# PaddlePaddle/Anakin

Measured on AMD Instinct MI355X. Metric: ResNet50 INT8 images/sec + p50 latency @ batch 1/8, 1×MI355X, higher is better.
Workload: dtype int8

## Files before the change

### anakin_amd/csrc/api_chain.hip

```cpp
#include "api_internal.h"

enum : unsigned { CK_1X1 = 1, CK_3X3 = 2, CK_HEAD = 4, CK_PAIR = 8, CK_LED = CK_3X3 | CK_HEAD, CK_ANY = 15 };
static unsigned chain_kind(const saber_hip_chain* ch) { return !ch->c3 ? CK_1X1 : (ch->b2 ? CK_PAIR : (ch->b ? CK_3X3 : CK_HEAD)); }
static const struct { int c1; unsigned kinds; ChainForm f; } chain_forms[] = {
    {64, CK_ANY,            {4, 4, 4, 1, 1, CS_BASE, false}},
    {64, CK_ANY,            {2, 2, 4, 1, 1, CS_BASE, false}},
    {128, CK_1X1 | CK_LED,  {2, 2, 4, 1, 1, CS_BASE, false}},
    {128, CK_1X1 | CK_LED,  {1, 1, 4, 1, 1, CS_BASE, false}},
    {128, CK_1X1 | CK_LED,  {6, 2, 8, 1, 1, CS_W8, false}},
    {128, CK_1X1 | CK_LED,  {5, 1, 8, 1, 1, CS_W8, false}},
    {256, CK_1X1 | CK_LED,  {1, 1, 4, 1, 1, CS_BASE, false}},
    {256, CK_1X1,           {9, 1, 4, 2, 1, CS_SPLIT, false}},
    {256, CK_1X1,           {11, 1, 8, 2, 1, CS_SPLIT8, false}},
    {256, CK_LED,           {3, 1, 8, 1, 1, CS_W8, false}},
    {256, CK_3X3,           {7, 1, 8, 1, 2, CS_COOP2, true}},
    {256, CK_3X3,           {15, 2, 8, 1, 4, CS_COOP4, true}},
    {512, CK_1X1,           {1, 1, 4, 1, 1, CS_BASE, false}},
    {512, CK_1X1,           {9, 1, 4, 2, 1, CS_SPLIT, false}},
};
static void for_each_chain_form(const saber_hip_chain* ch, const std::function<void(const ChainForm&)>& fn) {
    for (const auto& r : chain_forms)
        if (r.c1 == ch->c1 && (r.kinds & chain_kind(ch))) fn(r.f);
}
static ChainForm chain_form_where(const saber_hip_chain* ch, const std::function<bool(const ChainForm& row, const ChainForm& found)>& take) {
    ChainForm f;
    for_each_chain_form(ch, [&](const ChainForm& c) { if (take(c, f)) f = c; });
    return f;
}
ChainForm chain_form(const saber_hip_chain* ch, int code) { return chain_form_where(ch, [&](const ChainForm& c, const ChainForm&) { return c.code == code; }); }
ChainForm chain_form_default(const saber_hip_chain* ch) { return chain_form_where(ch, [](const ChainForm&, const ChainForm& f) { return !f.code; }); }
ChainForm chain_form_plain(const saber_hip_chain* ch) { return chain_form_where(ch, [](const ChainForm& c, const ChainForm&) { return !c.placement; }); }
bool chain_form_valid(const saber_hip_chain* ch, int code) {
    const ChainForm f = chain_form(ch, code);
    return f.code && ch->d_stream[f.stream].p && (f.coop != 4 || ch->stage1);
}
std::string chain_form_name(const saber_hip_chain* ch) {
    const ChainForm& f = ch->form;
    const std::string c = std::to_string(ch->c1), w8 = f.waves == 8 && f.coop == 1 ? "_w8" : "";
    if (!ch->c3) return "chain1x1_c" + c + "_px" + std::to_string(16 * f.rows) + (f.split == 2 ? "_split2" : "") + w8;
    return std::string("conv3x3+") + (ch->b2 ? "conv1x1+pair1x1_c" : (ch->b ? "chain1x1_c" : "conv1x1_c")) + c + "_" + std::to_string(f.rows) + "x16" + w8 +
           (f.coop == 2 ? "_coop2" : "") + (f.coop == 4 ? "_coop4" : "");
}
void for_each_chain_candidate(const saber_hip_chain* ch, bool shared_device, const std::function<void(const ChainForm&)>& fn) {
    for_each_chain_form(ch, [&](const ChainForm& c) { if (!(shared_device && c.placement) && chain_form_valid(ch, c.code)) fn(c); });
}

static bool chain_1x1(const saber_hip_conv* o, bool sub_res_ok = false) {
    const saber_hip_conv_desc& d = o->d;
    return o->is_i8 && o->weights_set && !o->gpool && o->algo == ALGO_IGEMM_I8 && o->epi == EPI_I8_CONV && d.kh == 1 && d.kw == 1 &&
           d.stride_h == 1 && d.stride_w == 1 && d.pad_h == 0 && d.pad_w == 0 && d.group == 1 && !o->pair_k2 &&
           !o->pool_fused && !o->pool2 && !o->pre_quant && !o->pre_pad && o->c_eff == d.c && d.act_negative_slope == 0.f &&
           d.in_layout == SABER_HIP_NHWC && d.out_layout == SABER_HIP_NHWC && (d.res_stride <= 1 || sub_res_ok);
}
static void pack_chain_params(const saber_hip_conv* o, size_t chunks_pad, std::vector<uint8_t>& out) {
    const int K = o->d.k;
    out.assign(chunks_pad * 16, 0);
    for (int k4 = 0; k4 < K / 4; ++k4) {
        float* f = (float*)(out.data() + (size_t)k4 * 48);
        int* ip = (int*)(out.data() + (size_t)k4 * 48 + 32);
        for (int r = 0; r < 4; ++r) {
            const int k = k4 * 4 + r;
            f[r] = o->scale_host.empty() ? 1.f : o->scale_host[k];
            f[4 + r] = (o->has_bias && !o->bias_p_host.empty()) ? o->bias_p_host[k] : 0.f;
            ip[r] = o->comp_host.empty() ? 0 : o->comp_host[k];
        }
    }
}
static void pack_chain_weights(const int8_t* w, int K, int C, int mfg, int wave, std::vector<uint8_t>& out, int kbase = 0,
                               int nw = 4, int ks0 = 0) {
    const int kw = K / nw, groups = kw / (16 * mfg), ksn = C / 64;
    for (int g = 0; g < groups; ++g)
        for (int ksi = 0; ksi < ksn; ++ksi)
            for (int mf = 0; mf < mfg; ++mf) {
                const int ks = (ks0 + ksi) % ksn;
                for (int lane = 0; lane < 64; ++lane) {
                    const int rho = lane & 15, kq = lane >> 4;
                    const int ch = kbase + wave * kw + g * 16 * mfg + (rho >> 2) * 4 * mfg + mf * 4 + (rho & 3);
                    const int8_t* src = w + (size_t)ch * C + ks * 64 + kq * 16;
                    out.insert(out.end(), (const uint8_t*)src, (const uint8_t*)src + 16);
                }
            }
}
static void pack_chain_weights3(const int8_t* w, int C, int wave, std::vector<uint8_t>& out, int nw = 4, int kbase = 0, int kcount = 0) {
    const int kw = (kcount ? kcount : C) / nw, mf0 = kw / 16, ksn = C / 64;
    for (int tap = 0; tap < 9; ++tap)
        for (int ks = 0; ks < ksn; ++ks)
            for (int mf = 0; mf < mf0; ++mf)
                for (int lane = 0; lane < 64; ++lane) {
                    const int rho = lane & 15, kq = lane >> 4;
                    const int ch = kbase + wave * kw + (rho >> 2) * 4 * mf0 + mf * 4 + (rho & 3);
                    for (int t = 0; t < 16; ++t) {
                        const int c = ks * 64 + kq * 16 + t;
// ... 279 lines not shown
    if (!xcd_round_robin()) return fail(SABER_HIP_UNIMPL, "stage: this device does not place workgroup b on XCD b % 8");
    return stage_build(chains, n, true, nullptr, out);
}
int saber_hip_conv2d_stage_create_tail(saber_hip_chain_t* const* chains, int n, saber_hip_chain_t* tail, saber_hip_chain_stage_t** out) {
    if (!tail) return fail(SABER_HIP_INVALID_VALUE, "null argument");
    if (!xcd_round_robin()) return fail(SABER_HIP_UNIMPL, "stage: this device does not place workgroup b on XCD b % 8");
    return stage_build(chains, n, true, tail, out);
}
int saber_hip_conv2d_stage_create_head(saber_hip_chain_t* const* chains, int n, saber_hip_chain_t* tail, const saber_hip_conv_t* head_a,
                                       const saber_hip_conv_t* head_b, saber_hip_chain_stage_t** out) {
    if (!head_a || !head_b) return fail(SABER_HIP_INVALID_VALUE, "null argument");
    if (!xcd_round_robin()) return fail(SABER_HIP_UNIMPL, "stage: this device does not place workgroup b on XCD b % 8");
    return stage_build(chains, n, true, tail, out, head_a, head_b);
}
void saber_hip_conv2d_stage_destroy(saber_hip_chain_stage_t* st) { delete st; }
int saber_hip_conv2d_stage_run(saber_hip_chain_stage_t* st, const void* x, const void* res, void* const* y1, void* const* y2, saber_hip_stream_t stream) {
    if (g_capture) return capture_unsupported("saber_hip_conv2d_stage_run (saber_hip_net_optimize forms stages itself)");
    if (!st || !x || !res || !y1 || !y2) return fail(SABER_HIP_INVALID_VALUE, "null argument");
    for (size_t i = 0; i < st->chains.size(); ++i)
        if ((!y1[i] && !(st->c1 == 64 && i + 1 < st->chains.size())) || !y2[i]) return fail(SABER_HIP_INVALID_VALUE, "stage: an output pointer per block");
    return stage_run(st, x, res, y1, y2, (hipStream_t)stream);
}
int saber_hip_conv2d_stage_run_tail(saber_hip_chain_stage_t* st, const void* x, const void* res, void* const* y1, void* const* y2, void* y_tail,
                                    saber_hip_stream_t stream) {
    if (g_capture) return capture_unsupported("saber_hip_conv2d_stage_run_tail (saber_hip_net_optimize forms stages itself)");
    if (!st || !x || !res || !y1 || !y2 || !y_tail) return fail(SABER_HIP_INVALID_VALUE, "null argument");
    for (size_t i = 0; i < st->chains.size(); ++i)
        if (!y1[i] || !y2[i]) return fail(SABER_HIP_INVALID_VALUE, "stage: an output pointer per block");
    return stage_run(st, x, res, y1, y2, (hipStream_t)stream, y_tail);
}
int saber_hip_conv2d_stage_run_head(saber_hip_chain_stage_t* st, const void* x_head, void* y_head_b, void* const* y1, void* const* y2, void* y_tail,
                                    saber_hip_stream_t stream) {
    if (g_capture) return capture_unsupported("saber_hip_conv2d_stage_run_head (saber_hip_net_optimize forms stages itself)");
    if (!st || !x_head || !y_head_b || !y1 || !y2) return fail(SABER_HIP_INVALID_VALUE, "null argument");
    for (size_t i = 0; i < st->chains.size(); ++i)
        if (!y1[i] || !y2[i]) return fail(SABER_HIP_INVALID_VALUE, "stage: an output pointer per block");
    return stage_run(st, x_head, nullptr, y1, y2, (hipStream_t)stream, y_tail, y_head_b);
}
static void pack_chain_stream(const saber_hip_chain* ch, ChainStream layout, std::vector<uint8_t>& out) {
    const saber_hip_conv *c3 = ch->c3, *a = ch->a, *b = ch->b;
    const int c = ch->c1, k1 = ch->k1, k2 = ch->k2, c2 = b ? b->d.c : 0, k2w = k2 / 2;
    const int nw = layout == CS_BASE || layout == CS_SPLIT ? 4 : 8;
    const int8_t *w3 = c3 ? c3->wq_oihw.data() : nullptr, *wa = a->wq_oihw.data(), *wb = b ? b->wq_oihw.data() : nullptr;
    std::vector<int8_t> wcat;
    if (ch->b2) {
        wcat.assign(b->wq_oihw.begin(), b->wq_oihw.end());
        wcat.insert(wcat.end(), ch->b2->wq_oihw.begin(), ch->b2->wq_oihw.end());
        wb = wcat.data();
    }
    auto mfg = [&](int k) { return ch->b2 ? 2 : std::min(4, k / nw / 16); };
    switch (layout) {
    case CS_BASE: case CS_W8:
        for (int w = 0; w < nw; ++w) {
            if (c3) pack_chain_weights3(w3, c, w, out, nw);
            pack_chain_weights(wa, k1, c, 4, w, out, 0, nw);
            if (b) pack_chain_weights(wb, k2, c2, mfg(k2), w, out, 0, nw);
        }
        break;
    case CS_SPLIT: case CS_SPLIT8:
        for (int half = 0; half < 2; ++half)
            for (int w = 0; w < nw; ++w) {
                pack_chain_weights(wa, k1, c, 4, w, out, 0, nw);
                pack_chain_weights(wb, k2w, c2, mfg(k2w), w, out, half * k2w, nw);
            }
        break;
    case CS_COOP2:
        for (int half = 0; half < 2; ++half)
            for (int w = 0; w < nw; ++w) {
                pack_chain_weights3(w3, c, w, out, nw, half * (c / 2), c / 2);
                pack_chain_weights(wa, k1 / 2, c, 4, w, out, half * (k1 / 2), nw, half * (c / 128));
                pack_chain_weights(wb, k2w, c2, 1, w, out, half * k2w, nw, half * (c2 / 128));
            }
        break;
    default: pack_coop4_stream(w3, wa, wb, out);
    }
}
static int chain_build(saber_hip_conv* c3, saber_hip_conv* a, saber_hip_conv* b, saber_hip_chain_t** out, saber_hip_conv* b2 = nullptr) {
    if (!a || !out || (!b && !c3) || (b2 && (!b || !c3))) return fail(SABER_HIP_INVALID_VALUE, "null argument");
    const bool pair2 = b2 != nullptr;
    const bool strided = c3 && (!b || pair2) && c3->d.stride_h == 2 && c3->d.stride_w == 2;
    if (pair2 && !strided) return fail(SABER_HIP_INVALID_VALUE, "chain: a sibling pair follows the strided head (conv3x3 / stride 2 + conv1x1 + eltwise) only");
    if (!chain_1x1(a, strided) || (b && !chain_1x1(b)) || (b2 && !chain_1x1(b2)))
        return fail(SABER_HIP_INVALID_VALUE, "chain: both ops must be plain 1x1 stride-1 INT8 NHWC convs with weights set");
    if (strided != (a->d.res_stride > 1) || (strided && a->d.res_stride != 2))
        return fail(SABER_HIP_INVALID_VALUE, "chain: a stride-2 head goes with a shortcut sub-sampled by 2 (and only with one)");
    const saber_hip_conv_desc& da = a->d;
    if (da.res_mode != SABER_HIP_RES_ELTWISE || da.out_dtype != SABER_HIP_S8 || (da.res_has_dtype && da.res_dtype != SABER_HIP_S8))
        return fail(SABER_HIP_INVALID_VALUE, "chain: the first conv must carry the fused eltwise epilogue with s8 residual and output");
    if (b) {
        const saber_hip_conv_desc& db = b->d;
        if (db.res_mode != SABER_HIP_RES_NONE || b->x_dtype != DT_S8 || (db.out_dtype != SABER_HIP_S8 && db.out_dtype != SABER_HIP_U8))
            return fail(SABER_HIP_INVALID_VALUE, "chain: the second conv must be a plain s8-input conv with an 8-bit output");
        if (db.n != da.n || db.h != a->oh || db.w != a->ow || db.c != da.k || (!pair2 && db.k != da.c))
            return fail(SABER_HIP_INVALID_VALUE, "chain: shapes must be C -> 4C -> C with C in {64,128,256,512} on the same pixels");
    }
    if (pair2) {
        const saber_hip_conv_desc &db = b->d, &d2 = b2->d;
        if (d2.res_mode != SABER_HIP_RES_NONE || b2->x_dtype != DT_S8 || (d2.out_dtype != SABER_HIP_S8 && d2.out_dtype != SABER_HIP_U8) || d2.n != da.n ||
            d2.h != a->oh || d2.w != a->ow || d2.c != da.k || da.c != 64 || db.k % 32 || db.k + d2.k != 640 || d2.k <= 0)
            return fail(SABER_HIP_INVALID_VALUE, "chain: the sibling pair after a strided head: 64 -> 256 (+ eltwise) -> k_b | k_b2 with k_b + k_b2 = 640, k_b % 32 == 0, 8-bit outputs");
    }
    if (!conv1x1_chain_ok(da.c, da.k, da.c))
        return fail(SABER_HIP_INVALID_VALUE, "chain: shapes must be C -> 4C -> C with C in {64,128,256,512} on the same pixels");
    if (c3) {
        const saber_hip_conv_desc& d3 = c3->d;
        const bool ok = c3->is_i8 && c3->weights_set && c3->algo == ALGO_IGEMM_I8 && c3->epi == EPI_I8_CONV && d3.kh == 3 && d3.kw == 3 &&
                        d3.stride_h == (strided ? 2 : 1) && d3.stride_w == d3.stride_h && d3.pad_h == 1 && d3.pad_w == 1 && d3.dil_h == 1 && d3.dil_w == 1 &&
                        d3.group == 1 && !c3->pair_k2 && !c3->pool_fused && !c3->pool2 && !c3->pre_quant && !c3->pre_pad &&
                        c3->c_eff == d3.c && d3.act_negative_slope == 0.f && d3.in_layout == SABER_HIP_NHWC &&
                        d3.out_layout == SABER_HIP_NHWC && d3.res_mode == SABER_HIP_RES_NONE && d3.c == da.c && d3.k == da.c &&
                        d3.n == da.n && c3->oh == da.h && c3->ow == da.w && da.c <= 256 &&
                        (d3.out_dtype == SABER_HIP_S8 || d3.out_dtype == SABER_HIP_U8) &&
                        (d3.out_dtype == SABER_HIP_U8) == (a->x_dtype == DT_U8);
        if (!ok) return fail(SABER_HIP_INVALID_VALUE, "chain: the head must be the 3x3 pad-1 INT8 conv (C -> C, C <= 256; stride 1, or 2 in front of a lone 1x1 conv) whose 8-bit output the first 1x1 conv reads");
    }
    saber_hip_chain* ch = new saber_hip_chain();
    const int k2 = b ? b->d.k + (pair2 ? b2->d.k : 0) : 0;
    ch->c3 = c3; ch->a = a; ch->b = b; ch->b2 = b2; ch->c1 = da.c; ch->k1 = da.k; ch->k2 = k2;
    ch->scale_conv = a->out_scale;
    if (c3 && !b && da.c == 256 && strided) {
        ch->tail_w3 = c3->wq_oihw;
        ch->tail_wa = a->wq_oihw;
    }
    ch->form = chain_form_default(ch);
    std::vector<uint8_t> p0, p1, p2;
    hipError_t e = hipSuccess;
    for (int l = 0; l < CS_COUNT && e == hipSuccess; ++l) {
        bool needed = false;
        for_each_chain_form(ch, [&](const ChainForm& f) { needed = needed || (f.stream == l && (!f.placement || xcd_round_robin())); });
        if (!needed) continue;
        std::vector<uint8_t> stream;
        pack_chain_stream(ch, (ChainStream)l, stream);
        e = ch->d_stream[l].upload(stream);
    }
    pack_chain_params(a, (size_t)da.k / 4 * 3, p1);
    if (b) pack_chain_params(b, ((size_t)k2 / 4 * 3 + 63) / 64 * 64 + 64, p2);
    if (pair2) {
        std::vector<uint8_t> pb2;
        pack_chain_params(b2, (size_t)b2->d.k / 4 * 3, pb2);
        std::memcpy(p2.data() + (size_t)b->d.k / 4 * 48, pb2.data(), pb2.size());
    }
    if (e == hipSuccess && ch->d_stream[CS_COOP2].p) {
        ch->coop_tiles = da.n * da.h * ((da.w + 15) / 16);
        e = ch->d_coop_ctr.alloc_zero((size_t)ch->coop_tiles * 32);
        if (e == hipSuccess) e = ch->d_coop_xcc.alloc_zero((size_t)ch->coop_tiles * 32);
        if (e == hipSuccess) e = ch->d_coop_xch.alloc_zero((size_t)ch->coop_tiles * 16 * da.c);
        if (e == hipSuccess) e = hipHostMalloc((void**)&ch->h_coop_err, sizeof(unsigned), hipHostMallocMapped);
        if (e == hipSuccess) *ch->h_coop_err = 0u;
    }
    if (e == hipSuccess && (da.c == 128 || da.c == 64) && c3 && b && !pair2 && c3->d.stride_h == 1 && xcd_round_robin()) {
        std::vector<uint8_t> s1;
        if (da.c == 128) pack_stage1_c128_stream(c3, a, b, s1);
        else pack_stage1_c64_stream(c3->wq_oihw.data(), a->wq_oihw.data(), b->wq_oihw.data(), s1);
        e = ch->d_stream_stage1.upload(s1);
    }
    if (e == hipSuccess) e = ch->d_prm1.upload(p1);
    if (e == hipSuccess && b) e = ch->d_prm2.upload(p2);
    if (e == hipSuccess && c3) {
        pack_chain_params(c3, ((size_t)da.c / 4 * 3 + 63) / 64 * 64 + 64, p0);
        e = ch->d_prm0.upload(p0);
    }
    if (e != hipSuccess) {
        delete ch;
        return hip_fail(e, "chain: device copies");
    }
    if (ch->d_stream[CS_COOP4].p) {
        const int rc = stage_build(&ch, 1, false, nullptr, &ch->stage1);
        if (rc != SABER_HIP_OK) {
            delete ch;
            return rc;
        }
    }
    *out = ch;
    return SABER_HIP_OK;
}
int saber_hip_conv2d_chain_create(saber_hip_conv_t* a, saber_hip_conv_t* b, saber_hip_chain_t** out) {
    if (!b) return fail(SABER_HIP_INVALID_VALUE, "null argument");
    return chain_build(nullptr, a, b, out);
}
int saber_hip_conv2d_chain_create3(saber_hip_conv_t* conv3x3, saber_hip_conv_t* a, saber_hip_conv_t* b, saber_hip_chain_t** out) {
    if (!conv3x3) return fail(SABER_HIP_INVALID_VALUE, "null argument");
    return chain_build(conv3x3, a, b, out);
}
int saber_hip_conv2d_chain_create3_pair(saber_hip_conv_t* conv3x3, saber_hip_conv_t* a, saber_hip_conv_t* pair_a, saber_hip_conv_t* pair_b,
                                        saber_hip_chain_t** out) {
    if (!conv3x3 || !pair_a || !pair_b) return fail(SABER_HIP_INVALID_VALUE, "null argument");
    return chain_build(conv3x3, a, pair_a, out, pair_b);
}
void saber_hip_conv2d_chain_destroy(saber_hip_chain_t* ch) { delete ch; }
int saber_hip_conv2d_chain_set_tile(saber_hip_chain_t* ch, int tn) {
    if (!ch) return fail(SABER_HIP_INVALID_VALUE, "null argument");
    if (!chain_form_valid(ch, tn)) return fail(SABER_HIP_INVALID_VALUE, "chain: no kernel form with that code for this chain");
    ch->form = chain_form(ch, tn);
    return SABER_HIP_OK;
}
int saber_hip_conv2d_chain_get_tile(const saber_hip_chain_t* ch) { return ch ? ch->form.code : 0; }
int saber_hip_conv2d_chain_run(saber_hip_chain_t* ch, const void* x, const void* res, void* y_a, void* y_b,
                               saber_hip_stream_t stream) {
    return saber_hip_conv2d_chain_run3(ch, x, res, y_a, y_b, nullptr, stream);
}
int saber_hip_conv2d_chain_run3(saber_hip_chain_t* ch, const void* x, const void* res, void* y_a, void* y_b, void* y_c,
                                saber_hip_stream_t stream) {
    if (g_capture) return capture_unsupported("saber_hip_conv2d_chain_run (saber_hip_net_optimize forms chains itself)");
    if (!ch || !x || !res || !y_a || (ch->b && !y_b) || (ch->b2 && !y_c)) return fail(SABER_HIP_INVALID_VALUE, "null argument");
    const saber_hip_conv *a = ch->a, *b = ch->b;
    ChainKArgs k;
    std::memset(&k, 0, sizeof k);
    k.x = x; k.res = res;
    const ChainForm f = ch->form;
    k.wstream = ch->d_stream[f.stream].p;
    k.prm1 = ch->d_prm1.p;
    k.prm2 = ch->d_prm2.p;
    k.y1 = y_a; k.y2 = y_b;
    k.M = a->d.n * a->oh * a->ow;
    k.in_u8 = a->x_dtype == DT_U8;
    k.relu1 = a->d.act == SABER_HIP_ACT_RELU;
    k.res_relu = a->d.res_act == SABER_HIP_ACT_RELU;
    k.coeff_conv = a->d.coeff_conv; k.scale_conv = ch->scale_conv; k.coeff_res = a->d.coeff_res; k.scale_res = a->d.scale_res;
    if (b) {
        k.relu2 = b->d.act == SABER_HIP_ACT_RELU;
        k.out_u8_2 = b->d.out_dtype == SABER_HIP_U8;
    }
    if (ch->b2) {
        k.y2b = y_c;
        k.k2_split = b->d.k;
        k.relu2b = ch->b2->d.act == SABER_HIP_ACT_RELU;
        k.out_u8_2b = ch->b2->d.out_dtype == SABER_HIP_U8;
    }
    if (ch->c3) {
        k.prm0 = ch->d_prm0.p;
        k.zero = zero_page();
        if (!k.zero) return fail(SABER_HIP_RUNTIME_ERROR, "chain: zero page");
        k.N = a->d.n; k.H = a->d.h; k.W = a->d.w;
        k.tiles_x = (k.W + 15) / 16;
        k.tiles_per_img = k.tiles_x * ((k.H + f.rows - 1) / f.rows);
        k.mg_tiles_x = div_magic(k.tiles_x);
        k.mg_tpi = div_magic(k.tiles_per_img);
        k.in0_u8 = ch->c3->x_dtype == DT_U8;
        k.relu0 = ch->c3->d.act == SABER_HIP_ACT_RELU;
        k.s0 = ch->c3->d.stride_h;
        k.H0 = ch->c3->d.h; k.W0 = ch->c3->d.w;
        if (a->d.res_stride > 1) { k.res_sub = a->d.res_stride; k.res_H = a->d.res_h; k.res_W = a->d.res_w; }
    }
    if (f.coop == 4) {
        const int rc = stage_run(ch->stage1, x, res, &y_a, &y_b, (hipStream_t)stream);
        if (rc != SABER_HIP_OK) ch->form = chain_form_plain(ch);
        return rc;
    }
    if (f.coop == 2) {
        if (*(volatile unsigned*)ch->h_coop_err) {
            *(volatile unsigned*)ch->h_coop_err = 0u;
            ch->form = chain_form_plain(ch);
            return fail(SABER_HIP_RUNTIME_ERROR, "cooperative chain: an earlier launch's workgroup pairs did not share an XCD or timed out at their "
                        "barrier (its outputs are not valid); the chain now runs the single-workgroup form");
        }
        const CoopKArgs ck{k, ch->d_coop_ctr.p, ch->d_coop_xch.p, ch->d_coop_xcc.p, ch->h_coop_err, ch->coop_tiles};
        HIP_TRY(launch_conv_chain_coop(ck, (hipStream_t)stream));
        return SABER_HIP_OK;
    }
    HIP_TRY(launch_conv1x1_chain(k, ch->c1, ch->k1, ch->k2, f.rows, f.waves, f.split, ch->c3 ? 1 : 0, (hipStream_t)stream));
    return SABER_HIP_OK;
}
```

### anakin_amd/csrc/api_internal.h

```cpp
#pragma once
#include "../../include/saber_hip.h"
#include "kernels.h"

#include <cmath>
#include <cstdio>
#include <algorithm>
#include <cstdlib>
#include <cstring>
#include <functional>
#include <memory>
#include <mutex>
#include <string>
#include <utility>
#include <type_traits>
#include <vector>

using namespace saber_mi355x;

namespace saber_api {

extern thread_local std::string g_err;
inline int fail(int code, const std::string& msg) {
    g_err = msg;
    return code;
// ... 124 lines not shown
    bool is_i8 = false;
    int x_dtype = DT_S8;
    int c_eff = 0;
    bool pre_quant = false;
    bool pre_pad = false;
    bool pre_transpose = false;
    size_t ws_bytes = 0;
    int Kg = 0, Kg_pad = 0, kw_pad = 0;
    float in_scale = 1.f, out_scale = 1.f;
    bool weights_set = false;
    std::vector<int8_t> wq_oihw;
    std::vector<float> w_scale;
    std::vector<float> bias_host;
    std::vector<float> bias_p_host, scale_host;
    std::vector<int> comp_host;
    DevBuf<uint8_t> d_w;
    DevBuf<float> d_part;
    DevBuf<unsigned> d_part_ctr;
    unsigned* h_part_err = nullptr;
    DevBuf<uint8_t> d_w3;
    DevBuf<float> d_bias, d_scale;
    DevBuf<int> d_comp;
    DevBuf<unsigned> d_sm_ctr;
    bool has_bias = false, has_comp = false;
    std::string algo_name;
    int pair_k1 = 0, pair_k2 = 0, pair_relu2 = 0, pair_dtype2 = 0;
    const saber_hip_conv* pair_src_a = nullptr;
    const saber_hip_conv* pair_src_b = nullptr;
};

struct saber_hip_stem_pair {
    saber_hip_conv* stem = nullptr;
    const saber_hip_conv* a = nullptr;
    const saber_hip_conv* b = nullptr;
    DevBuf<uint8_t> d_w, d_prm;
};

enum ChainStream { CS_BASE, CS_SPLIT, CS_SPLIT8, CS_W8, CS_COOP2, CS_COOP4, CS_COUNT };
struct ChainForm {
    int code = 0;
    int rows = 0;
    int waves = 4;
    int split = 1;
    int coop = 1;
    ChainStream stream = CS_BASE;
    bool placement = false;
};

struct saber_hip_chain {
    saber_hip_conv* c3 = nullptr;
    saber_hip_conv* a = nullptr;
    saber_hip_conv* b = nullptr;
    saber_hip_conv* b2 = nullptr;
    int c1 = 0, k1 = 0, k2 = 0;
    float scale_conv = 1.f;
    std::vector<int8_t> tail_w3, tail_wa;
    ChainForm form;
    DevBuf<uint8_t> d_stream[CS_COUNT];
    DevBuf<uint8_t> d_prm0, d_prm1, d_prm2;
    DevBuf<uint8_t> d_coop_xch;
    DevBuf<uint8_t> d_stream_stage1;
    DevBuf<unsigned long long> d_coop_ctr;
    DevBuf<unsigned> d_coop_xcc;
    unsigned* h_coop_err = nullptr;
    int coop_tiles = 0;
    struct saber_hip_chain_stage* stage1 = nullptr;
    ~saber_hip_chain();
};

struct saber_hip_chain_stage {
    std::vector<saber_hip_chain*> chains;
    saber_hip_chain* tail = nullptr;
    DevBuf<uint8_t> d_tail_stream;
    const saber_hip_conv* head_a = nullptr;
    const saber_hip_conv* head_b = nullptr;
    DevBuf<uint8_t> d_head_stream, d_head_prm1, d_head_prm2;
    DevBuf<saber_mi355x::StageBlk> d_blk;
    DevBuf<unsigned long long> d_grp_ctr, d_img_ctr;
    DevBuf<uint8_t> d_xch;
    DevBuf<unsigned> d_xcc;
    unsigned* h_err = nullptr;
    int c1 = 0, n = 0, h = 0, w = 0, tiles_x = 0, tiles_per_img = 0;
    bool per_image = false;
    ~saber_hip_chain_stage() {
        if (h_err) (void)hipHostFree(h_err);
    }
};

struct saber_hip_sep {
    saber_hip_conv* dw = nullptr;
    saber_hip_conv* pw = nullptr;
    int form = 0;
    DevBuf<uint8_t> d_wdw, d_wpw, d_prm;
    DevBuf<float> d_dw_bias, d_dw_scale;
    std::string name;
};

struct saber_hip_ir {
    saber_hip_conv* expand = nullptr;
    saber_hip_conv* dw = nullptr;
    saber_hip_conv* project = nullptr;
    int form = 0;
    float scale_conv = 1.f;
    DevBuf<uint8_t> d_we, d_eprm, d_wdw, d_wp, d_pprm;
    DevBuf<float> d_dw_bias, d_dw_scale;
    std::string name;
// ... 54 lines not shown
        ev.assign(2 * (size_t)reps, nullptr);
        for (hipEvent_t& x : ev)
            if ((e = hipEventCreate(&x)) != hipSuccess) return e;
        return hipStreamSynchronize(nullptr);
    }
    ~ColdBench() {
        for (hipEvent_t x : ev)
            if (x) (void)hipEventDestroy(x);
        if (buf) (void)hipFree(buf);
    }
    float run(hipStream_t s, const std::function<int()>& fn) {
        if (fn() != 0) return -1.f;
        for (int r = 0; r < reps; ++r) {
            if (launch_l2_flush(buf, kBytes, (unsigned*)((char*)buf + kBytes), s) != hipSuccess) return -1.f;
            if (hipEventRecord(ev[2 * r], s) != hipSuccess) return -1.f;
            if (fn() != 0) return -1.f;
            if (hipEventRecord(ev[2 * r + 1], s) != hipSuccess) return -1.f;
        }
        if (hipEventSynchronize(ev[2 * reps - 1]) != hipSuccess) return -1.f;
        std::vector<float> t(reps);
        for (int r = 0; r < reps; ++r)
            if (hipEventElapsedTime(&t[r], ev[2 * r], ev[2 * r + 1]) != hipSuccess) return -1.f;
        std::sort(t.begin(), t.end());
        return t[reps / 2] * 1000.f;
    }
};

extern thread_local ColdBench* g_cold;
int time_enqueued(hipStream_t s, const std::function<int()>& fn, int warm_iters, float* t);
extern thread_local std::vector<unsigned long long>* g_used_kernels;
constexpr float g_reuse_tol = 0.03f;
struct ColdScope {
    ColdBench local;
    bool owner = false;
    hipError_t enter(int reps, size_t flush_bytes = 0) {
        const char* w = std::getenv("SABER_HIP_AUTOTUNE_WARM");
        if (w && w[0] == '1') return hipSuccess;
        if (g_cold) return hipSuccess;
        hipError_t e = local.init(reps, flush_bytes);
        if (e != hipSuccess) return e;
        g_cold = &local;
        owner = true;
        return hipSuccess;
    }
    ~ColdScope() {
        if (owner) g_cold = nullptr;
    }
};

}

namespace saber_api {
enum OpKind { OP_CONV, OP_CONV_PAIR, OP_FC, OP_QUANT, OP_DEQUANT, OP_TRANSPOSE_IN, OP_ELT_I8, OP_ELT_F32, OP_POOL_I8, OP_POOL_F32, OP_POOL_F32_I8, OP_FC_Q, OP_SOFTMAX, OP_RELU_F32, OP_ACT_F32, OP_CONCAT, OP_DECONV };
enum Launch { LAUNCH_NONE, LAUNCH_OWN, LAUNCH_CHAIN, LAUNCH_CHAIN3, LAUNCH_STAGE, LAUNCH_STEM_PAIR, LAUNCH_SEP, LAUNCH_IR, LAUNCH_FIRE };
struct NetOp {
    OpKind kind;
    std::string name;
    saber_hip_conv* conv = nullptr;
    saber_hip_fc* fc = nullptr;
    saber_hip_deconv* deconv = nullptr;
    int in = -1, in2 = -1, out = -1, out2 = -1;
    std::vector<int> ins, cat_c;
    std::vector<float> cat_m;
    Launch launch = LAUNCH_OWN;
    int absorbed_by = -1;
    bool skip = false;
    std::string res_note;
    saber_hip_chain* chain = nullptr;
    int chain_out = -1;
    bool chain_on = false;
    saber_hip_chain* chain3 = nullptr;
    int chain3_res = -1, chain3_y1 = -1, chain3_y2 = -1;
    int chain3_y3 = -1;
    bool led_on = false;
    saber_hip_chain_stage* stage = nullptr;
    int stage_n = 0;
    bool stage_on = false;
    bool stage_name_kept = false;
    bool tail_on = false;
    int tail_of = -1;
    bool head_on = false;
    int head_of = -1;
    bool stage_y1_private = false;
    saber_hip_stem_pair* stem_pair = nullptr;
    int stem_y1 = -1, stem_y2 = -1;
    saber_hip_sep* sep = nullptr;
    int sep_out = -1;
    bool sep_on = false;
    saber_hip_ir* ir = nullptr;
    int ir_out = -1;
    bool ir_on = false;
    saber_hip_fire* fire = nullptr;
    int fire_out = -1;
    bool fire_on = false;
    int lane = 0;
    bool record = false;
    int p[16] = {0};
    float f[6] = {0};
    size_t count = 0;
};
template <typename F>
inline void op_for_each_input(const NetOp& o, F&& f) {
    if (o.kind == OP_CONCAT) {
        for (int t : o.ins) f(t);
        return;
    }
    if (o.in >= 0) f(o.in);
    if (o.in2 >= 0) f(o.in2);
}
inline int op_reads(const NetOp& o, int t) {
    int n = 0;
    op_for_each_input(o, [&](int u) { n += u == t; });
    return n;
}
inline bool op_touches(const NetOp& o, int t) { return op_reads(o, t) || o.out == t || o.out2 == t; }
}

struct saber_hip_net {
    std::vector<size_t> tensor_bytes;
    std::vector<size_t> tensor_off;
    std::vector<void*> tensor_ext;
    std::vector<std::pair<const void*, int>> captured_ptr;
    void* ptr(int id) const {
        if (id < 0) return nullptr;
        if ((size_t)id < tensor_ext.size() && tensor_ext[id]) return tensor_ext[id];
        return (void*)(arena + tensor_off[id]);
    }
    std::vector<NetOp> ops;
    char* arena = nullptr;
    size_t arena_bytes = 0, ws_off = 0, ws_bytes = 0;
    hipGraph_t graph = nullptr;
    hipGraphExec_t exec = nullptr;
    bool finalized = false;
    bool compacted = false;
    bool shared_device = false;
    bool reproducible_fp32 = false;
    bool inplace_external = false;
    int coop_fallbacks = 0;
    hipStream_t side = nullptr;
    hipEvent_t ev_start = nullptr, ev_join = nullptr;
    std::vector<hipEvent_t> ev_op;
    std::vector<int> writer;
    bool lanes_ready = false, has_side = false;
    std::vector<saber_hip_conv*> owned;
    std::vector<saber_hip_chain*> owned_chains;
    std::vector<saber_hip_chain_stage*> owned_stages;
    std::vector<saber_hip_stem_pair*> owned_stem_pairs;
    std::vector<saber_hip_sep*> owned_seps;
    std::vector<saber_hip_ir*> owned_irs;
    std::vector<saber_hip_fire*> owned_fires;
};

namespace saber_api {
struct Capture;
extern thread_local Capture* g_capture;
int capture_conv(saber_hip_conv* op, const void* x, void* y, const void* res);
int capture_fc(saber_hip_fc* fc, const void* x, float* y, bool quantised_input);
int capture_unsupported(const char* what);
int capture_deconv(saber_hip_deconv* op, const void* x, void* y);
int capture_concat(size_t pixels, int n_inputs, const void* const* xs, const int* channels, const float* mult, int dtype, void* y);
int capture_stream_op(OpKind kind, const char* name, const int* p, int np, const float* f, int nf, size_t count, const void* in,
                      size_t in_bytes, const void* in2, size_t in2_bytes, void* out, size_t out_bytes, void* out2, size_t out2_bytes);
}

bool sel_valid(const saber_hip_conv* op, const saber_api::ConvSel& s);
int sel_set(saber_hip_conv* op, const saber_api::ConvSel& s);
void sel_release_unused(saber_hip_conv* op);
void sel_name(saber_hip_conv* op);
unsigned long long sel_kernel_key(const saber_hip_conv* op, const saber_api::ConvSel& s);
int sel_launch(saber_hip_conv* op, saber_mi355x::ConvKArgs& a, hipStream_t s);
void for_each_candidate(const saber_hip_conv* op, const saber_api::ConvSel* best, const std::function<void(const saber_api::ConvSel&)>& fn);
bool dw_ok(const saber_hip_conv* op);
bool group_ok(const saber_hip_conv* op);
bool stem_ok(const saber_hip_conv* op);
bool fc_small_ok(const saber_hip_conv* op);
bool b3_tile_ok(const saber_hip_conv* op, int tile, int ks);
int dw_static_form(const saber_hip_conv* op);
int group_static_form(const saber_hip_conv* op);
constexpr long DW_STRIP_MIN_LANES = 150000;
void conv_fill_args(const saber_hip_conv* op, saber_mi355x::ConvKArgs& a, const void* x, void* y, const void* res);
int stem_pool_args(const saber_hip_conv* op, const void* x, void* y, void* workspace, hipStream_t s, saber_mi355x::ConvKArgs* a);
bool xcd_round_robin();
int split_prepare(saber_hip_conv* op);
bool img_conv_ok(const saber_hip_conv* op);
int img_conv_prepare(saber_hip_conv* op);
int pw_prepare(saber_hip_conv* op);
bool pw_eligible(const saber_hip_conv* op);
int img_conv_run(saber_hip_conv* op, const void* x, void* y, const void* res, void* y_pool, hipStream_t stream);
void img_conv_release(saber_hip_conv* op);
int net_launch(saber_hip_net* net, const NetOp& o, hipStream_t s);
bool fc_softmax_ok(const saber_hip_fc* fc, bool quantised_input = false);
int fc_run_softmax(saber_hip_fc* fc, const void* x, float* y, float* prob, void* workspace, hipStream_t s, bool quantised_input);
int fc_softmax_prepare(saber_hip_fc* fc);
int concat_check(int n_inputs, const int* channels, const float* mult, int dtype, int* row_bytes);
void net_resolve(saber_hip_net* net);
void net_drop_graph(saber_hip_net* net);
void net_set_chain_mode(saber_hip_net* net, int ia, int mode);
int net_chain_mode(const saber_hip_net* net, int ia);
void net_set_stage(saber_hip_net* net, int i0, bool on);
void net_set_head(saber_hip_net* net, int i0, bool on);
void net_set_tail(saber_hip_net* net, int i0, bool on);
ChainForm chain_form(const saber_hip_chain* ch, int code);
bool chain_form_valid(const saber_hip_chain* ch, int code);
ChainForm chain_form_default(const saber_hip_chain* ch);
ChainForm chain_form_plain(const saber_hip_chain* ch);
std::string chain_form_name(const saber_hip_chain* ch);
void for_each_chain_candidate(const saber_hip_chain* ch, bool shared_device, const std::function<void(const ChainForm&)>& fn);
bool conv_sep_ok(const saber_hip_conv* dw, const saber_hip_conv* pw, std::string* why);
bool sep_form_valid(const saber_hip_sep* sp, int code);
void for_each_sep_form(const saber_hip_sep* sp, const std::function<void(int code)>& fn);
int sep_static_form(const saber_hip_sep* sp);
void net_set_sep(saber_hip_net* net, int i, int code);
bool conv_ir_ok(const saber_hip_conv* expand, const saber_hip_conv* dw, const saber_hip_conv* project, std::string* why);
bool ir_form_valid(const saber_hip_ir* ir, int code);
void for_each_ir_form(const saber_hip_ir* ir, const std::function<void(int code)>& fn);
int ir_static_form(const saber_hip_ir* ir);
void net_set_ir(saber_hip_net* net, int i, int code);
bool conv_fire_ok(const saber_hip_conv* squeeze, const saber_hip_conv* e1, const saber_hip_conv* e3, std::string* why);
bool fire_form_valid(const saber_hip_fire* fr, int code);
void for_each_fire_form(const saber_hip_fire* fr, const std::function<void(int code)>& fn);
int fire_static_form(const saber_hip_fire* fr);
void net_set_fire(saber_hip_net* net, int i, int code);
bool deconv_form_valid(const saber_hip_deconv* op, int form);
int deconv_static_form(const saber_hip_deconv* op);
void for_each_deconv_form(const saber_hip_deconv* op, const std::function<void(int form)>& fn);
int stage_run(saber_hip_chain_stage* st, const void* x, const void* res, void* const* y1, void* const* y2, hipStream_t s, void* y_tail = nullptr,
              void* y_head = nullptr);
```

### anakin_amd/csrc/api_net.hip

```cpp
#include "api_internal.h"

#include <atomic>
static std::atomic<int> g_coop_fallbacks_total{0};

void net_drop_graph(saber_hip_net* net) {
    if (net->exec) (void)hipGraphExecDestroy(net->exec);
    if (net->graph) (void)hipGraphDestroy(net->graph);
    net->exec = nullptr;
    net->graph = nullptr;
}
int net_launch(saber_hip_net* net, const NetOp& o, hipStream_t s) {
    auto T = [&](int id) -> void* { return net->ptr(id); };
    void* ws = net->arena + net->ws_off;
    switch (o.kind) {
    case OP_CONV:
        switch (o.launch) {
        case LAUNCH_NONE: return SABER_HIP_OK;
        case LAUNCH_STAGE: {
            void* y1[saber_mi355x::STAGE4_LONG];
            void* y2[saber_mi355x::STAGE4_LONG];
            const NetOp* ops = &o;
            for (int k = 0; k < o.stage_n; ++k) {
                y1[k] = ops[3 * k].stage_y1_private ? nullptr : T(ops[3 * k].chain3_y1);
                y2[k] = T(ops[3 * k].chain3_y2);
            }
            void* const y_tail = o.tail_on ? T(ops[3 * o.stage_n].chain3_y1) : nullptr;
            const int rc = o.head_on ? stage_run(o.stage, T(ops[-1].in), nullptr, y1, y2, s, y_tail, T(o.in))
                                     : stage_run(o.stage, T(o.in), T(o.chain3_res), y1, y2, s, y_tail);
            if (rc == SABER_HIP_RUNTIME_ERROR) {
                ++net->coop_fallbacks;
                ++g_coop_fallbacks_total;
                net_set_stage(net, (int)(&o - net->ops.data()), false);
                net_drop_graph(net);
            }
            return rc;
        }
        case LAUNCH_STEM_PAIR: return saber_hip_conv2d_stem_pair_run(o.stem_pair, T(o.in), nullptr, T(o.stem_y1), T(o.stem_y2), ws, s);
        case LAUNCH_CHAIN3: {
            const int rc = saber_hip_conv2d_chain_run3(o.chain3, T(o.in), T(o.chain3_res), T(o.chain3_y1), T(o.chain3_y2), T(o.chain3_y3), s);
            if (rc == SABER_HIP_RUNTIME_ERROR) {
                ++net->coop_fallbacks;
                ++g_coop_fallbacks_total;
            }
            return rc;
        }
        case LAUNCH_CHAIN: return saber_hip_conv2d_chain_run(o.chain, T(o.in), T(o.in2), T(o.out), T(o.chain_out), s);
        case LAUNCH_SEP: return saber_hip_conv2d_sep_run(o.sep, T(o.in), nullptr, T(o.sep_out), s);
        case LAUNCH_IR: return saber_hip_conv2d_ir_run(o.ir, T(o.in), nullptr, nullptr, T(o.ir_out), s);
        case LAUNCH_FIRE: return saber_hip_conv2d_fire_run(o.fire, T(o.in), nullptr, T(o.fire_out), s);
        case LAUNCH_OWN: break;
        }
        if (o.conv->gpool) return saber_hip_conv2d_run_gpool(o.conv, T(o.in), T(o.out), T(o.in2), T(o.out2), s);
        return saber_hip_conv2d_run(o.conv, T(o.in), T(o.out), T(o.in2), ws, s);
    case OP_CONV_PAIR:
        if (o.skip) return SABER_HIP_OK;
        return saber_hip_conv2d_run_pair(o.conv, T(o.in), T(o.out), T(o.out2), s);
    case OP_FC:
        if (o.out2 >= 0) return fc_run_softmax(o.fc, T(o.in), (float*)T(o.out), (float*)T(o.out2), ws, s, false);
        return saber_hip_fc_run(o.fc, T(o.in), (float*)T(o.out), ws, s);
    case OP_QUANT:
        return saber_hip_quantize_nchw_to_nhwc(o.p[0], o.p[1], o.p[2], o.p[3], o.p[4], o.p[5], o.f[0],
                                               (const float*)T(o.in), T(o.out), s);
    case OP_DEQUANT:
        return saber_hip_dequantize_nhwc_to_nchw(o.p[0], o.p[1], o.p[2], o.p[3], o.p[4], o.f[0], T(o.in),
                                                 (float*)T(o.out), s);
    case OP_TRANSPOSE_IN:
        return saber_hip_transpose_nchw_to_nhwc_f32(o.p[0], o.p[1], o.p[2], o.p[3], o.p[4], (const float*)T(o.in),
                                                    (float*)T(o.out), s);
    case OP_ELT_I8:
        return saber_hip_eltwise_sum_i8(o.count, (const int8_t*)T(o.in), (const int8_t*)T(o.in2), o.f[0], o.f[1],
                                        o.f[2], o.f[3], o.p[0], (int8_t*)T(o.out), s);
    case OP_ELT_F32:
        return saber_hip_eltwise_sum_f32(o.count, (const float*)T(o.in), (const float*)T(o.in2), o.f[0], o.f[1],
                                         o.p[0], (float*)T(o.out), s);
    case OP_POOL_I8:
        return saber_hip_pool2d_i8_nhwc(o.p[0], o.p[1], o.p[2], o.p[3], o.p[4], o.p[5], o.p[6], o.p[7], o.p[8],
                                        o.p[9], o.p[10], o.p[11], o.p[12], o.p[13], o.p[14], T(o.in), T(o.out), s);
    case OP_POOL_F32:
        return saber_hip_pool2d_f32(o.p[0], o.p[1], o.p[2], o.p[3], o.p[4], o.p[5], o.p[6], o.p[7], o.p[8], o.p[9],
                                    o.p[10], o.p[11], o.p[12], o.p[13], (const float*)T(o.in), (float*)T(o.out), s);
    case OP_POOL_F32_I8:
        return saber_hip_pool2d_f32_from_i8_q(o.p[0], o.p[1], o.p[2], o.p[3], o.p[4], o.p[5], o.p[6], o.p[7], o.p[8],
                                              o.p[9], o.p[10], o.p[11], o.p[12], o.p[13], o.f[0], T(o.in),
                                              (float*)T(o.out), o.f[1], (int8_t*)T(o.out2), s);
    case OP_FC_Q:
        if (o.out2 >= 0) return fc_run_softmax(o.fc, T(o.in), (float*)T(o.out), (float*)T(o.out2), ws, s, true);
        return saber_hip_fc_run_q(o.fc, (const int8_t*)T(o.in), (float*)T(o.out), s);
    case OP_SOFTMAX:
        if (o.skip) return SABER_HIP_OK;
        return saber_hip_softmax_f32(o.p[0], o.p[1], (const float*)T(o.in), (float*)T(o.out), s);
    case OP_RELU_F32: return saber_hip_relu_f32(o.count, (const float*)T(o.in), (float*)T(o.out), s);
    case OP_ACT_F32: return saber_hip_activation_f32(o.p[0], o.count, o.f[0], o.f[1], (const float*)T(o.in), (float*)T(o.out), s);
    case OP_CONCAT: {
        if (o.skip) return SABER_HIP_OK;
        const void* xs[CONCAT_MAX_INPUTS];
        for (size_t k = 0; k < o.ins.size(); ++k) xs[k] = T(o.ins[k]);
        return saber_hip_concat_nhwc(o.count, (int)o.ins.size(), xs, o.cat_c.data(), o.cat_m.empty() ? nullptr : o.cat_m.data(), o.p[0], T(o.out), s);
    }
// ... 184 lines not shown
    o.kind = OP_DECONV; o.deconv = op; o.in = in_id; o.out = out_id;
    o.name = std::string("deconv:") + op->algo_name;
    return push(net, std::move(o));
}
int saber_hip_net_add_softmax(saber_hip_net_t* net, int rows, int cols, int in_id, int out_id) {
    NetOp o;
    o.kind = OP_SOFTMAX; o.in = in_id; o.out = out_id; o.name = "softmax_f32";
    o.p[0] = rows; o.p[1] = cols;
    return push(net, std::move(o));
}

int saber_hip_net_finalize(saber_hip_net_t* net) {
    if (net->finalized) return SABER_HIP_OK;
    size_t off = 0;
    net->tensor_off.resize(net->tensor_bytes.size());
    for (size_t i = 0; i < net->tensor_bytes.size(); ++i) {
        net->tensor_off[i] = off;
        if (net->tensor_ext[i]) continue;
        off += (net->tensor_bytes[i] + 255) / 256 * 256;
    }
    net->ws_off = off;
    off += (net->ws_bytes + 255) / 256 * 256;
    net->arena_bytes = off ? off : 256;
    HIP_TRY(hipMalloc((void**)&net->arena, net->arena_bytes));
    HIP_TRY(hipMemset(net->arena, 0, net->arena_bytes));
    HIP_TRY(hipStreamSynchronize(nullptr));
    net->finalized = true;
    return SABER_HIP_OK;
}
int saber_hip_net_compact_arena(saber_hip_net_t* net, const int* keep, int n_keep) {
    if (!net || !net->finalized) return fail(SABER_HIP_INVALID_VALUE, "compact_arena: net not finalized");
    const int nt = (int)net->tensor_bytes.size(), nops = (int)net->ops.size();
    for (const NetOp& o : net->ops)
        if (o.lane) return SABER_HIP_OK;
    std::vector<int> first(nt, nops), last(nt, -1), writes(nt, 0), reads(nt, 0);
    std::vector<char> pinned(nt, 0);
    for (int i = 0; i < n_keep; ++i)
        if (keep && keep[i] >= 0 && keep[i] < nt) pinned[keep[i]] = 1;
    std::vector<int> g_lo(nops), g_hi(nops);
    for (int i = 0; i < nops; ++i) g_lo[i] = g_hi[i] = i;
    auto span = [&](int i, int n) {
        const int hi = std::min(nops - 1, i + n - 1);
        int lo = i;
        for (int j = i; j <= hi; ++j) lo = std::min(lo, g_lo[j]);
        int h2 = hi;
        for (int j = i; j <= hi; ++j) h2 = std::max(h2, g_hi[j]);
        for (int j = lo; j <= h2; ++j) { g_lo[j] = std::min(g_lo[j], lo); g_hi[j] = std::max(g_hi[j], h2); }
    };
    for (int i = 0; i < nops; ++i) {
        const NetOp& o = net->ops[i];
        if (o.stage) span(i, 3 * o.stage_n + (o.stage->tail ? 2 : 0));
        if (o.stage && o.stage->head_a && i > 0) span(i - 1, 2);
        if (o.chain3) span(i, 3);
        if (o.chain) span(i, 2);
        if (o.stem_pair) span(i, 2);
        if (o.sep) span(i, 2);
        if (o.fire) span(i, 4);
        if (o.ir) span(i, 3);
        if ((o.kind == OP_FC || o.kind == OP_FC_Q) && o.out2 >= 0) span(i, 2);
    }
    for (int i = 0; i < nops; ++i) {
        const NetOp& o = net->ops[i];
        const int rd[] = {o.in, o.in2, o.chain3_res};
        const int wr[] = {o.out, o.out2, o.chain_out, o.chain3_y1, o.chain3_y2, o.chain3_y3, o.stem_y1, o.stem_y2, o.sep_out, o.ir_out, o.fire_out};
        auto touch = [&](int t) {
            if (t < 0 || t >= nt) return;
            first[t] = std::min(first[t], g_lo[i]);
            last[t] = std::max(last[t], g_hi[i]);
        };
        for (int t : rd) { touch(t); if (t >= 0 && t < nt) ++reads[t]; }
        for (size_t k = 1; k < o.ins.size(); ++k) { touch(o.ins[k]); if (o.ins[k] >= 0 && o.ins[k] < nt) ++reads[o.ins[k]]; }
        for (int t : wr) { touch(t); if (t >= 0 && t < nt) ++writes[t]; }
    }
    for (int t = 0; t < nt; ++t)
        if (net->tensor_ext[t] || !writes[t] || !reads[t] || last[t] < 0) pinned[t] = 1;
    for (int t = 0; t < nt; ++t)
        if (pinned[t]) { first[t] = -1; last[t] = nops; }
    std::vector<int> order;
    for (int t = 0; t < nt; ++t)
        if (!net->tensor_ext[t]) order.push_back(t);
    auto slot = [&](int t) { return (net->tensor_bytes[t] + 255) / 256 * 256; };
    std::stable_sort(order.begin(), order.end(), [&](int a, int b) { return slot(a) > slot(b); });
    std::vector<size_t> off(nt, 0);
    std::vector<int> placed;
    size_t top = 0;
    for (int t : order) {
        const size_t sz = slot(t);
        if (!sz) { off[t] = 0; continue; }
        std::vector<std::pair<size_t, size_t>> busy;
        for (int u : placed)
            if (first[u] <= last[t] && first[t] <= last[u]) busy.push_back({off[u], off[u] + slot(u)});
        std::sort(busy.begin(), busy.end());
        size_t at = 0;
        for (const auto& b : busy) {
            if (at + sz <= b.first) break;
            at = std::max(at, b.second);
        }
        off[t] = at;
        top = std::max(top, at + sz);
        placed.push_back(t);
    }
    const size_t ws_off = top, total = std::max<size_t>(256, top + (net->ws_bytes + 255) / 256 * 256);
    if (total >= net->arena_bytes) return SABER_HIP_OK;
    char* fresh = nullptr;
    HIP_TRY(hipMalloc((void**)&fresh, total));
    HIP_TRY(hipMemset(fresh, 0, total));
    HIP_TRY(hipDeviceSynchronize());
    for (int t = 0; t < nt; ++t)
        if (!net->tensor_ext[t] && !writes[t] && net->tensor_bytes[t])
            HIP_TRY(hipMemcpy(fresh + off[t], net->arena + net->tensor_off[t], net->tensor_bytes[t], hipMemcpyDeviceToDevice));
    HIP_TRY(hipDeviceSynchronize());
    (void)hipFree(net->arena);
    net->arena = fresh;
    net->arena_bytes = total;
    net->ws_off = ws_off;
    for (int t = 0; t < nt; ++t)
        if (!net->tensor_ext[t]) net->tensor_off[t] = off[t];
// ... 52 lines not shown
int saber_hip_net_run(saber_hip_net_t* net, saber_hip_stream_t stream) {
    if (!net->finalized) return fail(SABER_HIP_INVALID_VALUE, "net not finalized");
    int rc = net_prepare_lanes(net);
    if (rc) return rc;
    hipStream_t main_s = (hipStream_t)stream;
    if (!net->has_side) {
        for (const NetOp& o : net->ops) {
            rc = net_launch(net, o, main_s);
            if (rc) return rc;
        }
        return SABER_HIP_OK;
    }
    HIP_TRY(hipEventRecord(net->ev_start, main_s));
    HIP_TRY(hipStreamWaitEvent(net->side, net->ev_start, 0));
    std::fill(net->writer.begin(), net->writer.end(), -1);
    std::vector<std::vector<int>> readers(net->tensor_bytes.size());
    bool side_dirty = false;
    for (size_t i = 0; i < net->ops.size(); ++i) {
        const NetOp& o = net->ops[i];
        hipStream_t s = o.lane ? net->side : main_s;
        int ins[1 + CONCAT_MAX_INPUTS] = {o.out}, n_ins = 1;
        op_for_each_input(o, [&](int t) { ins[n_ins++] = t; });
        for (int k = 0; k < n_ins; ++k) {
            const int t = ins[k];
            if (t < 0) continue;
            const int wi = net->writer[t];
            if (wi >= 0 && net->ops[wi].lane != o.lane) HIP_TRY(hipStreamWaitEvent(s, net->ev_op[wi], 0));
        }
        const int outs[2] = {o.out, o.out2};
        for (int t : outs) {
            if (t < 0) continue;
            for (int r : readers[t])
                if (net->ops[r].lane != o.lane) HIP_TRY(hipStreamWaitEvent(s, net->ev_op[r], 0));
            readers[t].clear();
        }
        rc = net_launch(net, o, s);
        if (rc) return rc;
        if (o.record) HIP_TRY(hipEventRecord(net->ev_op[i], s));
        if (o.lane) side_dirty = true;
        net->writer[o.out] = (int)i;
        if (o.out2 >= 0) net->writer[o.out2] = (int)i;
        op_for_each_input(o, [&](int t) { readers[t].push_back((int)i); });
    }
    if (side_dirty) {
        HIP_TRY(hipEventRecord(net->ev_join, net->side));
        HIP_TRY(hipStreamWaitEvent(main_s, net->ev_join, 0));
    }
    return SABER_HIP_OK;
}
int saber_hip_net_set_lane(saber_hip_net_t* net, int index, int lane) {
    if (index < 0 || index >= (int)net->ops.size() || lane < 0 || lane > 1) return fail(SABER_HIP_INVALID_VALUE, "bad op index / lane");
    if (net->lanes_ready) return fail(SABER_HIP_INVALID_VALUE, "lanes are fixed after the first run");
    for (const NetOp& o : net->ops)
        if (lane && (o.chain || o.chain3 || o.stem_pair || o.sep || o.ir || o.fire))
            return fail(SABER_HIP_INVALID_VALUE, "the net has launches that span several ops' tensors (conv1x1 chains, the stem pair, separable sites): lanes must be assigned before saber_hip_net_optimize");
    if (lane) {
        const NetOp& o = net->ops[index];
        const size_t ws = o.kind == OP_CONV && o.conv ? o.conv->ws_bytes : (o.kind == OP_FC && o.fc ? saber_hip_fc_workspace_bytes(o.fc) : 0);
        if (ws) return fail(SABER_HIP_INVALID_VALUE, "an op that needs the shared workspace cannot run on the side lane");
    }
    net->ops[index].lane = lane;
    return SABER_HIP_OK;
}
int saber_hip_net_run_op(saber_hip_net_t* net, int index, saber_hip_stream_t stream) {
    if (!net->finalized || index < 0 || index >= (int)net->ops.size()) return fail(SABER_HIP_INVALID_VALUE, "bad op index");
    return net_launch(net, net->ops[index], (hipStream_t)stream);
}
static bool net_coop_error_pending(const saber_hip_net* net) {
    for (const NetOp& o : net->ops) {
        if (o.stage && o.stage->h_err && *(volatile unsigned*)o.stage->h_err) return true;
        if (const saber_hip_chain* ch = o.chain3)
            if ((ch->h_coop_err && *(volatile unsigned*)ch->h_coop_err) || (ch->stage1 && ch->stage1->h_err && *(volatile unsigned*)ch->stage1->h_err))
                return true;
    }
    return false;
}
int saber_hip_net_capture(saber_hip_net_t* net, saber_hip_stream_t stream) {
    hipStream_t s = (hipStream_t)stream;
    net_drop_graph(net);
    if (net_coop_error_pending(net)) return saber_hip_net_status(net);
    HIP_TRY(hipStreamBeginCapture(s, hipStreamCaptureModeThreadLocal));
    int rc = saber_hip_net_run(net, stream);
    hipError_t e = hipStreamEndCapture(s, &net->graph);
    if (rc == SABER_HIP_OK && e != hipSuccess) rc = hip_fail(e, "hipStreamEndCapture");
    if (rc == SABER_HIP_OK && (e = hipGraphInstantiate(&net->exec, net->graph, nullptr, nullptr, 0)) != hipSuccess) rc = hip_fail(e, "hipGraphInstantiate");
    if (rc != SABER_HIP_OK) net_drop_graph(net);
    return rc;
}
int saber_hip_net_replay(saber_hip_net_t* net, saber_hip_stream_t stream) {
    if (!net->exec) return fail(SABER_HIP_INVALID_VALUE, "net not captured");
    if (net_coop_error_pending(net)) return saber_hip_net_status(net);
    HIP_TRY(hipGraphLaunch(net->exec, (hipStream_t)stream));
    return SABER_HIP_OK;
}
int saber_hip_net_coop_fallbacks(const saber_hip_net_t* net) { return net ? net->coop_fallbacks : 0; }
int saber_hip_coop_fallbacks_total(void) { return g_coop_fallbacks_total.load(); }
static void conv_work(const saber_hip_conv* c, double& bytes, double& flops) {
    const saber_hip_conv_desc& d = c->d;
    const double esz_in = d.in_dtype == SABER_HIP_F32 ? 4 : 1, esz_out = d.out_dtype == SABER_HIP_F32 ? 4 : 1;
    const double esz_w = c->is_i8 ? 1 : 4;
    const double in_el = (double)d.n * d.h * d.w * d.c;
    const int oh = c->oh, ow = c->ow;
    const double out_el = (double)d.n * ((c->pool_fused || c->pool2) ? c->pool_oh * c->pool_ow : oh * ow) * d.k;
    bytes += in_el * esz_in + out_el * esz_out + (double)d.k * (d.c / d.group) * d.kh * d.kw * esz_w;
    if (d.res_mode != SABER_HIP_RES_NONE) bytes += (double)d.n * oh * ow * d.k * esz_out;
    flops += 2.0 * d.n * oh * ow * (double)d.k * (d.c / d.group) * d.kh * d.kw;
}
// ... 71 lines not shown
            float ms = 0;
            HIP_TRY(hipEventElapsedTime(&ms, ev[prev[i]], ev[i + 1]));
            acc[i] += ms;
        }
    }
    for (size_t i = 0; i < n; ++i) out_us[i] = (float)(acc[i] * 1000.0 / iters);
    return SABER_HIP_OK;
}
int saber_hip_net_time_op_in_pass(saber_hip_net_t* net, saber_hip_stream_t stream, int index, int iters, float* out_us) {
    if (!net || !net->finalized || iters <= 0 || !out_us || index < 0 || index >= (int)net->ops.size())
        return fail(SABER_HIP_INVALID_VALUE, "bad argument");
    hipStream_t s = (hipStream_t)stream;
    EventPair evp;
    HIP_TRY(evp.init());
    double acc = 0.0;
    for (int it = 0; it < iters + 1; ++it) {
        for (size_t i = 0; i < net->ops.size(); ++i) {
            if ((int)i == index) HIP_TRY(hipEventRecord(evp.e0, s));
            int rc = net_launch(net, net->ops[i], s);
            if (rc) return rc;
            if ((int)i == index) HIP_TRY(hipEventRecord(evp.e1, s));
        }
        HIP_TRY(hipStreamSynchronize(s));
        float ms = 0;
        HIP_TRY(hipEventElapsedTime(&ms, evp.e0, evp.e1));
        if (it) acc += ms;
    }
    *out_us = (float)(acc * 1000.0 / iters);
    return SABER_HIP_OK;
}
int saber_hip_net_time_ops(saber_hip_net_t* net, saber_hip_stream_t stream, int iters, float* out_us) {
    hipStream_t s = (hipStream_t)stream;
    EventPair evp;
    HIP_TRY(evp.init());
    hipEvent_t e0 = evp.e0, e1 = evp.e1;
    for (size_t i = 0; i < net->ops.size(); ++i) {
        int rc = net_launch(net, net->ops[i], s);
        if (rc) return rc;
        HIP_TRY(hipEventRecord(e0, s));
        for (int it = 0; it < iters; ++it) net_launch(net, net->ops[i], s);
        HIP_TRY(hipEventRecord(e1, s));
        HIP_TRY(hipEventSynchronize(e1));
        float ms = 0;
        HIP_TRY(hipEventElapsedTime(&ms, e0, e1));
        out_us[i] = ms * 1000.f / iters;
    }
    return SABER_HIP_OK;
}
int saber_hip_net_tensor_unwritten(const saber_hip_net_t* net, int id) {
    if (id < 0 || id >= (int)net->tensor_bytes.size()) return 0;
    if (net->tensor_bytes[id] == 0) return 1;
    for (const NetOp& o : net->ops) {
        const Launch by = o.skip ? net->ops[o.absorbed_by].launch : o.launch;
        if (o.out == id && (o.launch == LAUNCH_CHAIN3 || o.launch == LAUNCH_STEM_PAIR || o.launch == LAUNCH_SEP || (o.chain3 && by == LAUNCH_STAGE))) return 1;
        if (o.out == id && (o.launch == LAUNCH_IR || (o.skip && by == LAUNCH_IR && (int)(&o - net->ops.data()) == o.absorbed_by + 1))) return 1;
        if (o.out == id && o.kind == OP_CONV && (o.launch == LAUNCH_FIRE || (o.skip && by == LAUNCH_FIRE))) return 1;
        if (o.launch == LAUNCH_STAGE && o.head_on && o.chain3_res == id) return 1;
        if (o.chain3 && o.stage_y1_private && o.chain3_y1 == id && (o.launch == LAUNCH_STAGE || (o.skip && by == LAUNCH_STAGE))) return 1;
    }
    return 0;
}
int saber_hip_net_status(saber_hip_net_t* net) {
    if (!net || !net->finalized) return fail(SABER_HIP_INVALID_VALUE, "net not finalized");
    int bad = 0;
    for (size_t i = 0; i < net->ops.size(); ++i) {
        NetOp& o = net->ops[i];
        if (o.stage && o.stage->h_err && *(volatile unsigned*)o.stage->h_err) {
            *(volatile unsigned*)o.stage->h_err = 0u;
            if (o.stage_on) net_set_stage(net, (int)i, false);
            ++bad;
        }
        saber_hip_chain* ch = o.chain3;
        if (ch) {
            unsigned* words[2] = {ch->h_coop_err, ch->stage1 ? ch->stage1->h_err : nullptr};
            for (unsigned* w : words)
                if (w && *(volatile unsigned*)w) {
                    *(volatile unsigned*)w = 0u;
                    if (ch->form.placement) ch->form = chain_form_plain(ch);
                    ++bad;
                }
        }
    }
    if (!bad) return SABER_HIP_OK;
    net->coop_fallbacks += bad;
    g_coop_fallbacks_total += bad;
    net_resolve(net);
    net_drop_graph(net);
    return fail(SABER_HIP_RUNTIME_ERROR, "a cooperative launch of the last pass did not complete (workgroups on different XCDs, or a hand-off "
                "timed out: another kernel held the CUs); its outputs are not valid - those sites now launch block by block: run the pass again");
}
int saber_hip_net_inject_coop_error(saber_hip_net_t* net) {
    if (!net) return fail(SABER_HIP_INVALID_VALUE, "null argument");
    auto res2 = [](const NetOp& o) { return o.stage && o.stage->c1 == 64; };
    for (NetOp& o : net->ops)
        if (o.stage && !res2(o) && o.stage_on && o.stage->h_err) { *(volatile unsigned*)o.stage->h_err = 1u; return SABER_HIP_OK; }
    for (NetOp& o : net->ops)
        if (res2(o) && o.stage_on && o.stage->h_err) { *(volatile unsigned*)o.stage->h_err = 1u; return SABER_HIP_OK; }
    for (NetOp& o : net->ops) {
        if (o.stage && !res2(o) && o.stage->h_err) { *(volatile unsigned*)o.stage->h_err = 1u; return SABER_HIP_OK; }
        if (o.chain3 && o.chain3->h_coop_err) { *(volatile unsigned*)o.chain3->h_coop_err = 1u; return SABER_HIP_OK; }
    }
    for (NetOp& o : net->ops)
        if (res2(o) && o.stage->h_err) { *(volatile unsigned*)o.stage->h_err = 1u; return SABER_HIP_OK; }
    return fail(SABER_HIP_INVALID_VALUE, "the net has no cooperative launch site");
}
int saber_hip_net_num_launches(const saber_hip_net_t* net) {
    int n = 0;
// ... 23 lines not shown
```

### anakin_amd/csrc/api_net_autotune.hip

```cpp
#include "api_internal.h"

static saber_hip_conv* net_op_conv(saber_hip_net* net, int index) {
    if (index < 0 || index >= (int)net->ops.size()) return nullptr;
    NetOp& o = net->ops[index];
    if (o.kind == OP_CONV || o.kind == OP_CONV_PAIR) return o.conv;
    if (o.kind == OP_FC || o.kind == OP_FC_Q) return o.fc ? o.fc->conv : nullptr;
    return nullptr;
}
int saber_hip_net_get_choice(saber_hip_net_t* net, int index) {
    if (net && index >= 0 && index < (int)net->ops.size() && net->ops[index].kind == OP_DECONV)
        return (18 << 16) | saber_hip_deconv2d_get_tile(net->ops[index].deconv);
    saber_hip_conv* c = net_op_conv(net, index);
    int choice = (c && !c->pool_fused && (c->algo <= ALGO_IGEMM_F32 || dw_ok(c) || group_ok(c))) ? saber_hip_conv2d_get_tile(c) : 0;
    if (!c) return choice;
    const NetOp& o = net->ops[index];
    if (o.chain) choice |= (1 << 28) | ((o.chain_on ? o.chain->form.code : 0) << 24);
    if (o.chain3) choice |= (1 << 29) | ((o.led_on ? o.chain3->form.code : 0) << 24);
    if (o.sep) choice |= (3 << 28) | ((o.sep_on ? o.sep->form : 0) << 24);
    if (o.ir) choice |= (int)0x80000000u | ((o.ir_on ? o.ir->form : 0) << 24);
    if (o.fire) choice |= (int)0x80000000u | ((o.fire_on ? o.fire->form : 0) << 24);
    if (o.stage && o.stage_on) choice |= 1 << 30;
    if (o.stage && o.stage_on && o.tail_on) choice |= (int)0x80000000u;
    if (o.head_of >= 0 && net->ops[o.head_of].stage_on && net->ops[o.head_of].head_on) choice |= 1 << 29;
    return choice;
}
int saber_hip_net_stage_blocks(const saber_hip_net_t* net, int index) {
    if (!net || index < 0 || index >= (int)net->ops.size()) return 0;
    const NetOp& o = net->ops[index];
    return o.stage ? (o.stage->c1 == 64 ? -o.stage_n : o.stage_n) : 0;
}
int saber_hip_net_stage_head(const saber_hip_net_t* net, int index) {
    if (!net || index < 1 || index >= (int)net->ops.size() || !net->ops[index].stage) return -1;
    return net->ops[index - 1].head_of == index ? index - 1 : -1;
}
int saber_hip_net_set_choice(saber_hip_net_t* net, int index, int choice) {
    if (net && index >= 0 && index < (int)net->ops.size() && net->ops[index].kind == OP_DECONV) {
        if (net->reproducible_fp32 || ((choice >> 16) & 0xff) != 18) return SABER_HIP_OK;
        const int rc = saber_hip_deconv2d_set_tile(net->ops[index].deconv, choice & 0xffff);
        if (rc) return rc;
        net_resolve(net);
        net_drop_graph(net);
        return SABER_HIP_OK;
    }
    saber_hip_conv* c = net_op_conv(net, index);
    const bool ir_bits = c && net->ops[index].ir && ((unsigned)choice >> 30) == 2u;
    const int ir_tn = (choice >> 24) & 15;
    if (ir_bits && ir_tn && !ir_form_valid(net->ops[index].ir, ir_tn)) return saber_hip_conv2d_ir_set_tile(net->ops[index].ir, ir_tn);
    const bool fire_bits = c && net->ops[index].fire && ((unsigned)choice >> 30) == 2u;
    if (fire_bits && ir_tn && !fire_form_valid(net->ops[index].fire, ir_tn)) return saber_hip_conv2d_fire_set_tile(net->ops[index].fire, ir_tn);
    if (fire_bits && !(choice & 0xffffff)) {
        net_set_fire(net, index, ir_tn);
        net_drop_graph(net);
        return SABER_HIP_OK;
    }
    if (ir_bits && !(choice & 0xffffff)) {
        net_set_ir(net, index, ir_tn);
        net_drop_graph(net);
        return SABER_HIP_OK;
    }
    if (!c || !choice || c->pool_fused || (c->algo > ALGO_IGEMM_F32 && !dw_ok(c) && !group_ok(c))) return SABER_HIP_OK;
    if (net->reproducible_fp32 && !c->is_i8) return SABER_HIP_OK;
    if (net->ops[index].kind == OP_CONV_PAIR && index > 0 && net->ops[index - 1].stem_pair) return SABER_HIP_OK;
    const int chain_bits = (choice >> 24) & 63;
    const bool stage_on = ((choice >> 30) & 1) && !net->shared_device;
    const bool tail_on = stage_on && (((unsigned)choice >> 31) & 1u);
    choice &= 0xffffff;
    if (net->shared_device && ((choice >> 16) & 0xff) == 11) choice &= ~(0xf << 12);
    NetOp& o = net->ops[index];
    saber_hip_chain* ch = index + 1 >= (int)net->ops.size() ? nullptr : ((o.chain3 && (chain_bits & 32)) ? o.chain3 : ((o.chain && (chain_bits & 16)) ? o.chain : nullptr));
    int tn = chain_bits & 15;
    if (ch && net->shared_device && chain_form(ch, tn).placement) tn = chain_form_plain(ch).code;
    if (ch && tn && !chain_form_valid(ch, tn)) return saber_hip_conv2d_chain_set_tile(ch, tn);
    const bool sep_bits = o.sep && (chain_bits & 48) == 48;
    if (sep_bits && tn && !sep_form_valid(o.sep, tn)) return saber_hip_conv2d_sep_set_tile(o.sep, tn);
    int rc = choice ? saber_hip_conv2d_set_tile(c, choice) : SABER_HIP_OK;
    if (rc) return rc;
    o.res_note.clear();
    o.stage_name_kept = false;
    if (ch && tn) (void)saber_hip_conv2d_chain_set_tile(ch, tn);
    const bool in_stage = o.chain3 && o.skip && !o.stage && o.tail_of < 0;
    const int mode = ch ? net_chain_mode(net, ch == o.chain3 ? index + 1 : index) : 0;
    if (ch && ch == o.chain3) net_set_chain_mode(net, index + 1, (tn || in_stage) ? 2 : std::min(mode, 1));
    else if (ch) net_set_chain_mode(net, index, mode == 2 ? 2 : (tn ? 1 : 0));
    if (o.stage) net_set_stage(net, index, stage_on);
    if (o.stage) net_set_tail(net, index, tail_on);
    if (o.head_of >= 0) net_set_head(net, o.head_of, (chain_bits & 32) && !net->shared_device);
    if (sep_bits) net_set_sep(net, index, tn);
    if (ir_bits) net_set_ir(net, index, ir_tn);
    if (fire_bits) net_set_fire(net, index, ir_tn);
    net_resolve(net);
    net_drop_graph(net);
    return SABER_HIP_OK;
}

static int net_consolidate_kernels(saber_hip_net* net, hipStream_t s) {
    if (net->has_side) return SABER_HIP_OK;
    if (const char* e = std::getenv("SABER_HIP_NO_CONSOLIDATE"))
        if (e[0] == '1') return SABER_HIP_OK;
    struct Site { int op; unsigned long long key; ConvSel choice; };
    auto conv_of = [&](const NetOp& o) -> saber_hip_conv* {
        if (o.launch != LAUNCH_OWN) return nullptr;
        if (o.kind != OP_CONV && o.kind != OP_CONV_PAIR) return nullptr;
        if (net->reproducible_fp32 && o.conv && !o.conv->is_i8) return nullptr;
        return (o.conv && !o.conv->pool_fused && o.conv->algo <= ALGO_IGEMM_F32) ? o.conv : nullptr;
    };
    auto collect = [&]() {
        std::vector<Site> v;
        for (int i = 0; i < (int)net->ops.size(); ++i)
            if (saber_hip_conv* c = conv_of(net->ops[i])) v.push_back({i, sel_kernel_key(c, c->sel), c->sel});
        return v;
    };
    EventPair ev;
    HIP_TRY(ev.init());
    auto forward_ms = [&](float* ms) -> int {
        int rc = 0;
        for (int i = 0; i < 3 && !rc; ++i) rc = saber_hip_net_run(net, s);
        if (rc) return rc;
        HIP_TRY(hipEventRecord(ev.e0, s));
        for (int i = 0; i < 30 && !rc; ++i) rc = saber_hip_net_run(net, s);
        HIP_TRY(hipEventRecord(ev.e1, s));
        HIP_TRY(hipEventSynchronize(ev.e1));
        HIP_TRY(hipEventElapsedTime(ms, ev.e0, ev.e1));
        return rc;
    };
    std::vector<Site> sites = collect();
    for (size_t si = 0; si < sites.size(); ++si) {
        const Site cur = sites[si];
        if ((cur.key >> 8 & 0xff) != 5) continue;
        int uses = 0;
        for (const Site& t : sites) uses += t.key == cur.key;
        if (uses != 1) continue;
        saber_hip_conv* c = conv_of(net->ops[cur.op]);
        std::vector<Site> alts;
        for (const Site& t : sites) {
            if (t.op == cur.op || (t.key & 0xff) != (cur.key & 0xff) || (t.key >> 8 & 0xff) != 5 || t.key == cur.key) continue;
            if ((net->ops[t.op].kind == OP_CONV_PAIR) != (net->ops[cur.op].kind == OP_CONV_PAIR)) continue;
            bool dup = false;
            for (const Site& a : alts) dup |= a.key == t.key;
            if (!dup) alts.push_back(t);
// ... 34 lines not shown
    ColdScope scope;
    HIP_TRY(scope.enter(iters < 7 ? 7 : (iters > 15 ? 15 : iters), net->arena_bytes > ((size_t)256 << 20) ? net->arena_bytes : 0));
    std::vector<unsigned long long> used_kernels;
    struct UsedScope {
        UsedScope(std::vector<unsigned long long>* v) { g_used_kernels = g_cold ? v : nullptr; }
        ~UsedScope() { g_used_kernels = nullptr; }
    } used_scope(&used_kernels);
    for (NetOp& o : net->ops) {
        if (o.kind == OP_CONV_PAIR && o.skip && &o != net->ops.data() && (&o)[-1].stem_pair) continue;
        if (net->reproducible_fp32 && o.conv && !o.conv->is_i8) continue;
        if (net->reproducible_fp32 && o.fc && o.fc->conv && !o.fc->conv->is_i8) continue;
        if (o.kind == OP_CONV_PAIR) {
            int rc = saber_hip_conv2d_autotune_pair(o.conv, T(o.in), T(o.out), T(o.out2), stream, iters);
            if (rc) return rc;
            continue;
        }
        saber_hip_conv* c = o.kind == OP_CONV ? o.conv : ((o.kind == OP_FC || o.kind == OP_FC_Q) ? o.fc->conv : nullptr);
        if (!c) continue;
        const void* xin = T(o.in);
        if (o.kind == OP_FC && o.fc->pre_quant) {
            int rq = net_launch(net, o, (hipStream_t)stream);
            if (rq) return rq;
            xin = net->arena + net->ws_off;
        }
        int rc = saber_hip_conv2d_autotune(c, xin, T(o.out), T(o.in2), net->arena + net->ws_off, stream, iters);
        if (rc) return rc;
        o.res_note.clear();
    }
    for (NetOp& o : net->ops) {
        if (o.kind != OP_DECONV || net->reproducible_fp32) continue;
        hipStream_t s = (hipStream_t)stream;
        auto run = [&]() -> int { return net_launch(net, o, s); };
        float best = 0.f;
        int best_form = -1;
        for_each_deconv_form(o.deconv, [&](int form) {
            float us = -1.f;
            if (saber_hip_deconv2d_set_tile(o.deconv, form) != SABER_HIP_OK) return;
            if (time_enqueued(s, run, 20, &us) != SABER_HIP_OK) return;
            if (best_form < 0 || us < best) { best = us; best_form = form; }
        });
        if (best_form < 0) return fail(SABER_HIP_RUNTIME_ERROR, "autotune: no form of a deconv op could be timed");
        int rc = saber_hip_deconv2d_set_tile(o.deconv, best_form);
        if (!rc) rc = run();
        if (rc) return rc;
    }
    net_resolve(net);
    const char* log_env = std::getenv("SABER_HIP_AUTOTUNE_LOG");
    const bool log_cands = g_cold && log_env && log_env[0] == '1';
    auto log_cand = [&](const saber_hip_conv* c, const std::string& name, float t) {
        if (log_cands) std::fprintf(stderr, "autotune [%dx%dx%d c%d k%d %dx%d] %-40s %8.2f us\n", c->d.n, c->d.h, c->d.w, c->d.c, c->d.k, c->d.kh, c->d.kw, name.c_str(), t);
    };
    for (size_t i = 0; i < net->ops.size(); ++i)
        if (net->ops[i].stage) net_set_stage(net, (int)i, false);
    for (size_t i = 0; i < net->ops.size(); ++i) {
        NetOp& A = net->ops[i];
        const int ia = (int)i;
        NetOp* H = (ia > 0 && net->ops[ia - 1].chain3) ? &net->ops[ia - 1] : nullptr;
        if (!A.chain && !H) continue;
        const int first = H ? ia - 1 : ia;
        const int last = (A.chain || (H && H->chain3->b2)) ? ia + 1 : ia;
        hipStream_t s = (hipStream_t)stream;
        auto run_all = [&]() -> int {
            int rc = 0;
            for (int k = first; k <= last; ++k) rc |= net_launch(net, net->ops[k], s);
            return rc;
        };
        auto timed = [&](float* t) { return time_enqueued(s, run_all, 20, t); };
        float best = 0.f;
        int best_mode = 0, best_tn = 0;
        net_set_chain_mode(net, ia, 0);
        int rc = timed(&best);
        if (rc) return rc;
        log_cand(A.conv, "separate", best);
        for (int mode = A.chain ? 1 : 2; mode <= (H ? 2 : 1); ++mode) {
            saber_hip_chain* ch = mode == 2 ? H->chain3 : A.chain;
            for_each_chain_candidate(ch, net->shared_device, [&](const ChainForm& f) {
                float ms = -1.f;
                if (saber_hip_conv2d_chain_set_tile(ch, f.code) != SABER_HIP_OK) return;
                net_set_chain_mode(net, ia, mode);
                const int rt = timed(&ms);
                log_cand(A.conv, (mode == 2 ? H->name : A.name).substr(5), ms);
                if (rt == SABER_HIP_OK && ms < best) { best = ms; best_mode = mode; best_tn = f.code; }
            });
        }
        if (best_mode) (void)saber_hip_conv2d_chain_set_tile(best_mode == 2 ? H->chain3 : A.chain, best_tn);
        net_set_chain_mode(net, ia, best_mode);
        rc = run_all();
        if (rc) return rc;
    }
    for (size_t i = 0; i < net->ops.size(); ++i) {
        NetOp& H0 = net->ops[i];
        if (!H0.stage || net->shared_device) continue;
        const bool has_tail = H0.stage->tail != nullptr;
        const bool has_head = saber_hip_net_stage_head(net, (int)i) >= 0;
        const int first = (int)i, last = first + 3 * H0.stage_n - 1 + (has_tail ? 2 : 0);
        hipStream_t s = (hipStream_t)stream;
        auto run_all = [&]() -> int {
            int rc = 0;
            for (int k = first - (has_head ? 1 : 0); k <= last; ++k) rc |= net_launch(net, net->ops[k], s);
            return rc;
        };
        auto timed = [&](float* t) { return time_enqueued(s, run_all, 20, t); };
        std::vector<int> modes(H0.stage_n), tns(H0.stage_n);
        for (int k = 0; k < H0.stage_n; ++k) {
            modes[k] = net_chain_mode(net, first + 3 * k + 1);
            tns[k] = net->ops[first + 3 * k].chain3->form.code;
        }
        float sep = 0.f, one = 0.f;
        int rc = timed(&sep);
        if (rc) return rc;
        log_cand(H0.conv, "separate", sep);
        net_set_stage(net, first, true);
        net_set_tail(net, first, false);
        bool ok = timed(&one) == SABER_HIP_OK && hipStreamSynchronize(s) == hipSuccess && !*(volatile unsigned*)H0.stage->h_err;
        log_cand(H0.conv, H0.name.substr(5), ok ? one : -1.f);
        if (ok && has_tail) {
            float wt = 0.f;
            net_set_tail(net, first, true);
            const bool ok_t = timed(&wt) == SABER_HIP_OK && hipStreamSynchronize(s) == hipSuccess && !*(volatile unsigned*)H0.stage->h_err;
            log_cand(H0.conv, H0.name.substr(5), ok_t ? wt : -1.f);
            if (*(volatile unsigned*)H0.stage->h_err) ok = false;
            else if (ok_t && wt < one) one = wt;
            else net_set_tail(net, first, false);
        }
        if (ok && one < sep && has_head) {
            float wh = 0.f;
            net_set_head(net, first, true);
            const bool ok_h = timed(&wh) == SABER_HIP_OK && hipStreamSynchronize(s) == hipSuccess && !*(volatile unsigned*)H0.stage->h_err;
            log_cand(H0.conv, H0.name.substr(5), ok_h ? wh : -1.f);
            if (*(volatile unsigned*)H0.stage->h_err) ok = false;
            else if (ok_h && wh < one * 0.99f) one = wh;
            else net_set_head(net, first, false);
        }
        if (!ok || one >= sep * (H0.stage->c1 == 64 ? 0.99f : 1.f)) {
            *(volatile unsigned*)H0.stage->h_err = 0u;
            net_set_stage(net, first, false);
            for (int k = 0; k < H0.stage_n; ++k) {
                (void)saber_hip_conv2d_chain_set_tile(net->ops[first + 3 * k].chain3, tns[k]);
                net_set_chain_mode(net, first + 3 * k + 1, modes[k]);
            }
        }
        rc = run_all();
        if (rc) return rc;
    }
    for (size_t i = 0; i + 1 < net->ops.size(); ++i) {
        NetOp& D = net->ops[i];
        if (!D.sep) continue;
        hipStream_t s = (hipStream_t)stream;
        auto run_all = [&]() -> int { return net_launch(net, net->ops[i], s) | net_launch(net, net->ops[i + 1], s); };
        auto timed = [&](float* t) { return time_enqueued(s, run_all, 20, t); };
        float best = 0.f;
        int best_code = 0;
        net_set_sep(net, (int)i, 0);
        int rc = timed(&best);
        if (rc) return rc;
        log_cand(D.conv, "separate", best);
        for_each_sep_form(D.sep, [&](int code) {
            float us = -1.f;
            net_set_sep(net, (int)i, code);
            const int rt = timed(&us);
            log_cand(D.conv, D.name.substr(5), us);
            if (rt == SABER_HIP_OK && us < best) { best = us; best_code = code; }
        });
        net_set_sep(net, (int)i, best_code);
        rc = run_all();
        if (rc) return rc;
    }
    for (size_t i = 0; i + 2 < net->ops.size(); ++i) {
        NetOp& E = net->ops[i];
        if (!E.ir) continue;
        hipStream_t s = (hipStream_t)stream;
        auto run_all = [&]() -> int { return net_launch(net, net->ops[i], s) | net_launch(net, net->ops[i + 1], s) | net_launch(net, net->ops[i + 2], s); };
        auto timed = [&](float* t) { return time_enqueued(s, run_all, 20, t); };
        float best = 0.f;
        int best_code = 0;
        net_set_ir(net, (int)i, 0);
        int rc = timed(&best);
        if (rc) return rc;
        log_cand(E.conv, "separate", best);
        for_each_ir_form(E.ir, [&](int code) {
            float us = -1.f;
            net_set_ir(net, (int)i, code);
            const int rt = timed(&us);
            log_cand(E.conv, E.name.substr(5), us);
            if (rt == SABER_HIP_OK && us < best) { best = us; best_code = code; }
        });
        net_set_ir(net, (int)i, best_code);
        rc = run_all();
        if (rc) return rc;
    }
    for (size_t i = 0; i + 3 < net->ops.size(); ++i) {
        NetOp& Q = net->ops[i];
        if (!Q.fire) continue;
        hipStream_t s = (hipStream_t)stream;
        auto run_all = [&]() -> int {
            int r = 0;
            for (size_t j = i; j <= i + 3; ++j) r |= net_launch(net, net->ops[j], s);
// ... 23 lines not shown
```

### anakin_amd/csrc/api_net_optimize.hip

```cpp
#include "api_internal.h"

void net_resolve(saber_hip_net* net) {
    std::vector<NetOp>& ops = net->ops;
    const int n = (int)ops.size();
    enum { IN_CHAIN, IN_STAGE, IN_STEM, IN_SEP, IN_IR, IN_FIRE };
    static const char* const covered[] = {"conv:(in the chain launch)", "conv:(in the stage launch)", "conv:(in the stem launch)", "conv:(in the separable launch)",
                                          "conv:(in the inverted-residual launch)", "conv:(in the fire launch)"};
    std::vector<int> in(n, IN_CHAIN);
    for (NetOp& o : ops) {
        o.launch = LAUNCH_OWN;
        o.absorbed_by = -1;
    }
    auto absorb = [&](int j, int by, int what) {
        ops[j].launch = LAUNCH_NONE;
        ops[j].absorbed_by = by;
        in[j] = what;
    };
    for (int i = 0; i < n; ++i) {
        NetOp& o = ops[i];
        if (o.launch == LAUNCH_NONE) continue;
        if ((o.kind == OP_FC || o.kind == OP_FC_Q) && o.out2 >= 0) {
            for (int j = i + 1; j < n; ++j)
                if (ops[j].kind == OP_SOFTMAX && ops[j].out == o.out2) { absorb(j, i, IN_CHAIN); break; }
        }
        if (o.kind != OP_CONV || i + 1 >= n) continue;
        if (o.stage && o.stage_on) {
            o.launch = LAUNCH_STAGE;
            for (int k = 0; k < o.stage_n; ++k) {
                if (k) absorb(i + 3 * k, i, IN_STAGE);
                absorb(i + 3 * k + 1, i, IN_CHAIN);
                absorb(i + 3 * k + 2, i, IN_CHAIN);
            }
            if (o.tail_on)
                for (int j = i + 3 * o.stage_n; j < i + 3 * o.stage_n + 2; ++j) absorb(j, i, IN_STAGE);
            if (o.head_on) absorb(i - 1, i, IN_STAGE);
        } else if (o.stem_pair) {
            o.launch = LAUNCH_STEM_PAIR;
            absorb(i + 1, i, IN_STEM);
        } else if (o.chain3 && o.led_on) {
            o.launch = LAUNCH_CHAIN3;
            absorb(i + 1, i, IN_CHAIN);
            if (o.chain3->b || o.chain3->b2) absorb(i + 2, i, IN_CHAIN);
        } else if (o.chain && o.chain_on) {
            o.launch = LAUNCH_CHAIN;
            absorb(i + 1, i, IN_CHAIN);
        } else if (o.sep && o.sep_on) {
            o.launch = LAUNCH_SEP;
            absorb(i + 1, i, IN_SEP);
        } else if (o.ir && o.ir_on && i + 2 < n) {
            o.launch = LAUNCH_IR;
            absorb(i + 1, i, IN_IR);
            absorb(i + 2, i, IN_IR);
        } else if (o.fire && o.fire_on && i + 3 < n) {
            o.launch = LAUNCH_FIRE;
            for (int j = i + 1; j <= i + 3; ++j) absorb(j, i, IN_FIRE);
        }
    }
    for (int i = 0; i < n; ++i) {
        NetOp& o = ops[i];
        o.skip = o.launch == LAUNCH_NONE;
        if (o.kind == OP_CONCAT) {
            o.name = "concat" + std::to_string(o.ins.size()) + (o.skip ? " (in the fire launch)" : "");
        } else if (o.kind == OP_DECONV) {
            o.name = std::string("deconv:") + o.deconv->algo_name;
        } else if (o.kind == OP_SOFTMAX) {
            o.name = o.skip ? "softmax_f32 (in the fc launch)" : "softmax_f32";
        } else if (o.kind == OP_FC || o.kind == OP_FC_Q) {
            o.name = std::string("fc:") + o.fc->conv->algo_name;
            if (o.out2 >= 0) o.name += fc_softmax_ok(o.fc, o.kind == OP_FC_Q) ? "+softmax" : " | softmax_f32";
        } else if (o.kind == OP_CONV || o.kind == OP_CONV_PAIR) {
            const std::string own = o.conv->algo_name;
            const bool kept = o.stage_name_kept && !o.skip;
            switch (kept ? (o.stage ? LAUNCH_STAGE : LAUNCH_NONE) : o.launch) {
            case LAUNCH_NONE: o.name = covered[kept ? IN_STAGE : in[i]]; break;
            case LAUNCH_OWN: o.name = "conv:" + own + o.res_note; break;
            case LAUNCH_CHAIN: o.name = "conv:" + chain_form_name(o.chain); break;
            case LAUNCH_CHAIN3: o.name = "conv:" + chain_form_name(o.chain3); break;
            case LAUNCH_SEP: o.name = std::string("conv:") + saber_hip_conv2d_sep_algo(o.sep); break;
            case LAUNCH_IR: o.name = std::string("conv:") + saber_hip_conv2d_ir_algo(o.ir); break;
            case LAUNCH_FIRE: o.name = std::string("conv:") + saber_hip_conv2d_fire_algo(o.fire); break;
            case LAUNCH_STEM_PAIR: o.name = "conv:" + own + "+pair1x1_" + std::to_string(o.stem_pair->a->d.k) + "+" + std::to_string(o.stem_pair->b->d.k); break;
            case LAUNCH_STAGE:
                o.name = std::string(o.head_on && !kept ? "conv:[pair1x1]+stage_c" : "conv:stage_c") + std::to_string(o.stage->c1) + "_" + std::to_string(o.stage_n) + "x[conv3x3+chain1x1]_2x16" +
                         (o.stage->c1 == 256 ? "_coop4" : "") + (o.tail_on && !kept ? "+[conv3x3/2+conv1x1]" : "");
                break;
            }
        }
    }
}
void net_set_chain_mode(saber_hip_net* net, int ia, int mode) {
    NetOp& A = net->ops[ia];
    NetOp* H = (ia > 0 && net->ops[ia - 1].chain3) ? &net->ops[ia - 1] : nullptr;
    if (H) H->led_on = mode == 2;
    if (H) H->stage_name_kept = false;
    A.chain_on = A.chain && mode >= 1;
    A.res_note.clear();
    net_resolve(net);
}
int net_chain_mode(const saber_hip_net* net, int ia) {
    const NetOp& A = net->ops[ia];
    return (ia > 0 && net->ops[ia - 1].chain3 && net->ops[ia - 1].led_on) ? 2 : (A.chain_on ? 1 : 0);
}
void net_set_tail(saber_hip_net* net, int i0, bool on) {
    NetOp& H0 = net->ops[i0];
    if (!H0.stage || !H0.stage->tail) return;
    H0.tail_on = on;
    net_resolve(net);
}
void net_set_head(saber_hip_net* net, int i0, bool on) {
    NetOp& H0 = net->ops[i0];
    if (!H0.stage || !H0.stage->head_a || i0 < 1 || net->ops[i0 - 1].head_of != i0) return;
    H0.head_on = on;
    net_resolve(net);
}
void net_set_stage(saber_hip_net* net, int i0, bool on) {
    NetOp& H0 = net->ops[i0];
    if (!H0.stage) return;
    if (on || H0.stage_on)
        for (int k = 0; k < H0.stage_n; ++k) {
            net->ops[i0 + 3 * k].led_on = true;
            net->ops[i0 + 3 * k].stage_name_kept = !on;
            net->ops[i0 + 3 * k + 1].chain_on = net->ops[i0 + 3 * k + 1].chain != nullptr;
        }
    if (on) H0.tail_on = H0.stage->tail != nullptr;
    if (!on) H0.tail_on = H0.head_on = false;
    H0.stage_on = on;
    net_resolve(net);
}
void net_set_sep(saber_hip_net* net, int i, int code) {
    NetOp& D = net->ops[i];
    if (!D.sep || i + 1 >= (int)net->ops.size()) return;
    if (code && saber_hip_conv2d_sep_set_tile(D.sep, code) != SABER_HIP_OK) code = 0;
    D.sep_on = code != 0;
    net_resolve(net);
}
void net_set_ir(saber_hip_net* net, int i, int code) {
    NetOp& E = net->ops[i];
    if (!E.ir || i + 2 >= (int)net->ops.size()) return;
    if (code && saber_hip_conv2d_ir_set_tile(E.ir, code) != SABER_HIP_OK) code = 0;
    E.ir_on = code != 0;
    net_resolve(net);
}
void net_set_fire(saber_hip_net* net, int i, int code) {
    NetOp& Q = net->ops[i];
    if (!Q.fire || i + 3 >= (int)net->ops.size()) return;
    if (code && saber_hip_conv2d_fire_set_tile(Q.fire, code) != SABER_HIP_OK) code = 0;
    Q.fire_on = code != 0;
    net_resolve(net);
}
static int clone_conv_i8(const saber_hip_conv* src, const saber_hip_conv_desc& d, saber_hip_conv** out) {
    int rc = saber_hip_conv2d_create(&d, out);
    if (rc) return rc;
    rc = saber_hip_conv2d_set_weights(*out, src->wq_oihw.data(), SABER_HIP_S8, src->w_scale.data(),
                                      src->has_bias ? src->bias_host.data() : nullptr, src->in_scale, src->out_scale);
    if (rc) {
        saber_hip_conv2d_destroy(*out);
        *out = nullptr;
    }
    return rc;
}

int saber_hip_net_optimize(saber_hip_net_t* net, int flags) {
    if (!net) return fail(SABER_HIP_INVALID_VALUE, "null argument");
    if (net->finalized) return fail(SABER_HIP_INVALID_VALUE, "optimize must run before finalize");
    if (flags & 2048) {
        net->shared_device = true;
        flags &= ~256;
    }
    if (net->shared_device) flags &= ~256;
    if (flags & SABER_HIP_NET_REPRODUCIBLE_FP32) net->reproducible_fp32 = true;
    std::vector<NetOp>& ops = net->ops;
    const int nt = (int)net->tensor_bytes.size();
    std::vector<char> dead(ops.size(), 0);
    int removed = 0;
    auto consumers = [&](int t) {
        int c = 0;
        for (size_t i = 0; i < ops.size(); ++i)
            if (!dead[i]) c += op_reads(ops[i], t);
// ... 314 lines not shown
                A.chain3 || B.chain3 || in_ir(A) || in_ir(B))
                continue;
            if (A.conv->d.res_mode != SABER_HIP_RES_ELTWISE || B.in != A.out || A.in2 < 0 || B.in2 >= 0) continue;
            saber_hip_chain* ch = nullptr;
            if (saber_hip_conv2d_chain_create(A.conv, B.conv, &ch) != SABER_HIP_OK) continue;
            net->owned_chains.push_back(ch);
            A.chain = ch;
            A.chain_out = B.out;
            net_set_chain_mode(net, (int)i, ch->c1 <= 256 ? 1 : 0);
            if (A.chain_on) ++removed;
        }
    }
    if (flags & 32) {
        for (size_t i = 0; i + 2 < ops.size(); ++i) {
            NetOp& Hd = ops[i];
            NetOp& A = ops[i + 1];
            NetOp& B = ops[i + 2];
            if (!A.chain || Hd.kind != OP_CONV || !Hd.conv || Hd.chain3 || Hd.chain || Hd.skip || Hd.lane || Hd.in2 >= 0 ||
                A.in != Hd.out)
                continue;
            if (readers(Hd.out) != 1) continue;
            saber_hip_chain* ch = nullptr;
            if (saber_hip_conv2d_chain_create3(Hd.conv, A.conv, B.conv, &ch) != SABER_HIP_OK) continue;
            net->owned_chains.push_back(ch);
            Hd.chain3 = ch;
            Hd.chain3_res = A.in2; Hd.chain3_y1 = A.out; Hd.chain3_y2 = B.out;
            const bool was = A.chain_on;
            net_set_chain_mode(net, (int)i + 1, ch->c1 <= 128 ? 2 : (was ? 1 : 0));
            if (Hd.led_on) removed += was ? 1 : 2;
        }
        for (size_t i = 0; i + 1 < ops.size(); ++i) {
            NetOp& Hd = ops[i];
            NetOp& A = ops[i + 1];
            if (A.chain || A.skip || A.kind != OP_CONV || !A.conv || A.conv->d.res_mode != SABER_HIP_RES_ELTWISE || A.in2 < 0 || A.lane ||
                Hd.kind != OP_CONV || !Hd.conv || Hd.chain3 || Hd.chain || Hd.skip || Hd.lane || Hd.in2 >= 0 || A.in != Hd.out || in_ir(Hd) || in_ir(A))
                continue;
            if (readers(Hd.out) != 1) continue;
            saber_hip_chain* ch = nullptr;
            NetOp* P = (flags & 1024) && i + 2 < ops.size() ? &ops[i + 2] : nullptr;
            if (P && (P->kind != OP_CONV_PAIR || P->lane || P->skip || P->in != A.out || !P->conv || !P->conv->pair_src_a || !P->conv->pair_src_b)) P = nullptr;
            if (P) {
                if (readers(A.out) != 1 || saber_hip_conv2d_chain_create3_pair(Hd.conv, A.conv, const_cast<saber_hip_conv*>(P->conv->pair_src_a),
                                                                   const_cast<saber_hip_conv*>(P->conv->pair_src_b), &ch) != SABER_HIP_OK)
                    P = nullptr;
            }
            if (!P && saber_hip_conv2d_chain_create3(Hd.conv, A.conv, nullptr, &ch) != SABER_HIP_OK) continue;
            net->owned_chains.push_back(ch);
            Hd.chain3 = ch;
            Hd.chain3_res = A.in2; Hd.chain3_y1 = A.out; Hd.chain3_y2 = P ? P->out : -1; Hd.chain3_y3 = P ? P->out2 : -1;
            net_set_chain_mode(net, (int)i + 1, ch->c1 <= 128 ? 2 : 0);
            if (Hd.led_on) removed += P ? 2 : 1;
        }
    }
    if ((flags & 256) && (flags & 32) && !two_lanes) {
        for (size_t i = 0; i + 2 < ops.size();) {
            auto block_ok = [&](size_t j) {
                return j + 2 < ops.size() && ops[j].chain3 && ops[j].chain3->b && !ops[j].stage && ops[j].chain3_y2 >= 0 &&
                       ((ops[j].chain3->c1 == 256 && ops[j].chain3->stage1) || ((ops[j].chain3->c1 == 128 || ops[j].chain3->c1 == 64) && ops[j].chain3->d_stream_stage1.p));
            };
            if (!block_ok(i)) { ++i; continue; }
            std::vector<saber_hip_chain*> run{ops[i].chain3};
            while ((int)run.size() < saber_mi355x::STAGE4_LONG) {
                const size_t p = i + 3 * (run.size() - 1), j = p + 3;
                if (!block_ok(j) || ops[j].chain3->c1 != run[0]->c1 || ops[j].in != ops[p].chain3_y2 || ops[j].chain3_res != ops[p].chain3_y1) break;
                run.push_back(ops[j].chain3);
            }
            if (run.size() >= 2) {
                saber_hip_chain_stage* st = nullptr;
                const size_t pl = i + 3 * (run.size() - 1), jt = pl + 3;
                saber_hip_chain* tail = nullptr;
                if (jt + 1 < ops.size() && run[0]->c1 == 256 && ops[jt].chain3 && !ops[jt].chain3->b && !ops[jt].chain3->b2 && !ops[jt].stage &&
                    ops[jt].chain3->c1 == 256 && ops[jt].chain3->c3->d.stride_h == 2 && ops[jt].in == ops[pl].chain3_y2 &&
                    ops[jt].chain3_res == ops[pl].chain3_y1 && ops[jt].chain3_y1 >= 0)
                    tail = ops[jt].chain3;
                const saber_hip_conv *head_a = nullptr, *head_b = nullptr;
                if (i >= 1 && run[0]->c1 == 256 && ops[i - 1].kind == OP_CONV_PAIR && !ops[i - 1].skip && !ops[i - 1].lane && ops[i - 1].conv &&
                    ops[i - 1].conv->pair_src_a && ops[i - 1].conv->pair_src_b && !(i >= 3 && ops[i - 3].chain3 && ops[i - 3].chain3->b2)) {
                    const NetOp& P = ops[i - 1];
                    const int t_res = ops[i].chain3_res, t_x = ops[i].in;
                    const bool fwd = P.out == t_res && P.out2 == t_x, rev = P.out == t_x && P.out2 == t_res;
                    if ((fwd || rev) && t_res != t_x && readers(t_res) == 1 && readers(t_x) == 1) {
                        head_a = fwd ? P.conv->pair_src_a : P.conv->pair_src_b;
                        head_b = fwd ? P.conv->pair_src_b : P.conv->pair_src_a;
                    }
                }
                if (head_a && saber_hip_conv2d_stage_create_head(run.data(), (int)run.size(), tail, head_a, head_b, &st) != SABER_HIP_OK) head_a = head_b = nullptr;
                if (!head_a && tail && saber_hip_conv2d_stage_create_tail(run.data(), (int)run.size(), tail, &st) != SABER_HIP_OK) tail = nullptr;
                if (head_a || tail || saber_hip_conv2d_stage_create(run.data(), (int)run.size(), &st) == SABER_HIP_OK) {
                    net->owned_stages.push_back(st);
                    ops[i].stage = st;
                    ops[i].stage_n = (int)run.size();
                    if (tail) ops[jt].tail_of = (int)i;
                    if (head_a) ops[i - 1].head_of = (int)i;
                    int before = 0;
                    for (size_t k = 0; k < run.size(); ++k) before += 3 - (ops[i + 3 * k].skip + ops[i + 3 * k + 1].skip + ops[i + 3 * k + 2].skip);
                    if (tail) before += 2 - (ops[jt].skip + ops[jt + 1].skip);
                    if (run[0]->c1 == 64)
                        for (size_t k = 0; k + 1 < run.size(); ++k) ops[i + 3 * k].stage_y1_private = readers(ops[i + 3 * k].chain3_y1) == 2;
                    const bool on = run[0]->a->d.n >= 4 && run[0]->c1 == 256;
                    net_set_stage(net, (int)i, on);
                    if (on) removed += before - 1;
                }
            }
            i += 3 * run.size();
        }
    }
// ... 38 lines not shown
```

### anakin_amd/csrc/conv1x1_chain.hip

```cpp
#include "epilogue_pack.h"

namespace saber_mi355x {


template <int KS1, int G1, int MFG2, int G2, int TN, int R, bool C3, int SP, bool HAS2 = true, int NW = 4, int S0 = 1>
__global__ __launch_bounds__(64 * NW) void conv1x1_chain_kernel(const ChainKArgs a) {
    static_assert(NW == 4 || NW == 8, "4 or 8 waves");
    static_assert(S0 == 1 || (C3 && S0 == 2), "a strided head is led by its 3x3 conv");
    constexpr int KS2 = NW * G1;
    constexpr int K1 = 64 * NW * G1, C1 = 64 * KS1, K2W = NW * G2 * 16 * MFG2, K2 = K2W * SP;
    constexpr int NPX = 16 * TN;
    constexpr int MF0 = C3 ? C1 / (16 * NW) : 1;
    static_assert(!C3 || C1 % (16 * NW) == 0, "3x3 conv: at least 16 channels per wave");
    constexpr int T0 = C3 ? MF0 * 9 * KS1 : 0;
    constexpr int SG1 = KS1 * 4, SG2 = KS2 * MFG2;
    constexpr int T1 = G1 * SG1, T2 = HAS2 ? G2 * SG2 : 0;
    constexpr int OFF = T0 % R;
    constexpr int CPR = K1 / 16;
    constexpr int CH1 = C1 / 16;
    constexpr int PCH = CH1 + 1;
    constexpr int HW = 16 * S0 + 3 - S0, HP = ((TN - 1) * S0 + 3) * HW;
    constexpr int HCH = C3 ? (HP * PCH + 63) / 64 * 64 : 1;
    constexpr int P0C = C3 ? (C1 / 4 * 3 + 63) / 64 * 64 : 1;
    constexpr int P1C = K1 / 4 * 3, P2C = (K2 / 4 * 3 + 63) / 64 * 64;
    static_assert(SG1 % R == 0 && SG2 % R == 0, "ring depth must divide the group lengths");
    static_assert(CPR >= 16 && P1C % 64 == 0, "tile rows are swizzled on 16 chunks");
    static_assert(SP == 1 || (!C3 && (NPX * CPR / (64 * NW)) % SP == 0), "split second conv: 1x1 chains only");

    __shared__ v4i tile[NPX * CPR];
    __shared__ v4i prm1[P1C];
    __shared__ v4i prm2[P2C];
    __shared__ v4i halo[HCH];
    __shared__ v4i mid[C3 ? NPX * PCH : 1];
    __shared__ v4i prm0[P0C];
    SABER_TL_DECL;
    SABER_TL(0);
    asm volatile("" ::"s"(a.x), "s"(a.wstream), "s"(a.res), "s"(a.prm1), "s"(a.prm2), "s"(a.M), "s"(a.in_u8));
    const int tid = threadIdx.x, lane = tid & 63;
    const int wave = __builtin_amdgcn_readfirstlane(tid >> 6);
    const int frow = lane & 15, fq = lane >> 4;
    const int half = SP == 1 ? 0 : (int)(blockIdx.x % SP);
    const int p0 = (SP == 1 ? blockIdx.x : blockIdx.x / SP) * NPX;
    const int plast = a.M - 1;
    int n = 0, y0 = 0, x0 = 0;
    if constexpr (C3) {
        asm volatile("" ::"s"(a.prm0), "s"(a.zero), "s"(a.H), "s"(a.W), "s"(a.tiles_x), "s"(a.tiles_per_img), "s"(a.mg_tiles_x),
                     "s"(a.mg_tpi));
        const int t = blockIdx.x;
        n = a.mg_tpi ? (int)__umulhi((unsigned)t, a.mg_tpi) : t;
        const int rem = t - n * a.tiles_per_img;
        const int ty = a.mg_tiles_x ? (int)__umulhi((unsigned)rem, a.mg_tiles_x) : rem;
        y0 = ty * TN;
        x0 = (rem - ty * a.tiles_x) * 16;
    }
    auto pix = [&](int px, bool& ok) -> int {
        if constexpr (!C3) {
            const int p = p0 + px;
            ok = p < a.M;
            return p < plast ? p : plast;
        } else {
            int y = y0 + (px >> 4), x = x0 + (px & 15);
            ok = y < a.H && x < a.W;
            y = y < a.H ? y : a.H - 1;
            x = x < a.W ? x : a.W - 1;
            return (n * a.H + y) * a.W + x;
        }
    };

    v4i bx[KS1][TN];
    if constexpr (!C3) {
#pragma unroll
        for (int j = 0; j < TN; ++j) {
            bool ok;
            const int p = pix(j * 16 + frow, ok);
            const char* xp = (const char*)a.x + (size_t)p * C1 + fq * 16;
#pragma unroll
            for (int ks = 0; ks < KS1; ++ks) bx[ks][j] = *(const v4i*)(xp + ks * 64);
        }
    }

    {
        if constexpr (C3) {
            const char* xg = (const char*)a.x;
            for (int i = wave; i < HCH / 64; i += NW) {
                const int L = i * 64 + lane;
                const int hp = L / PCH, cc = L - hp * PCH;
                const int hy = hp / HW, hx = hp - hy * HW;
                const int gy = y0 * S0 - 1 + hy, gx = x0 * S0 - 1 + hx;
                const int H0 = S0 == 1 ? a.H : a.H0, W0 = S0 == 1 ? a.W : a.W0;
                const bool in = hp < HP && cc < CH1 && (unsigned)gy < (unsigned)H0 && (unsigned)gx < (unsigned)W0;
                const char* src = in ? xg + ((size_t)((n * H0 + gy) * W0 + gx) * C1 + cc * 16) : (const char*)a.zero;
                lds_dma16(src, halo + i * 64);
            }
            for (int i = wave; i < P0C / 64; i += NW) lds_dma16((const v4i*)a.prm0 + i * 64 + lane, prm0 + i * 64);
        }
        const char* rg = (const char*)a.res;
        constexpr int NI = NPX * CPR / 64;
#pragma unroll
        for (int i0 = 0; i0 < NI; i0 += NW) {
            const int i = i0 + wave;
            const int L = i * 64 + lane;
            const int px = L / CPR, c = (L % CPR) ^ (px & 15);
            bool ok;
            int p = pix(px, ok);
            if constexpr (S0 > 1) {
                const int yy = min(y0 + (px >> 4), a.H - 1), xx = min(x0 + (px & 15), a.W - 1);
                p = (n * a.res_H + yy * a.res_sub) * a.res_W + xx * a.res_sub;
            }
            lds_dma16(rg + (size_t)p * K1 + c * 16, tile + i * 64);
        }
        for (int i = wave; i < P1C / 64; i += NW) lds_dma16((const v4i*)a.prm1 + i * 64 + lane, prm1 + i * 64);
        if constexpr (HAS2)
            for (int i = wave; i < P2C / 64; i += NW) lds_dma16((const v4i*)a.prm2 + i * 64 + lane, prm2 + i * 64);
    }
    asm volatile("" ::: "memory");

    const v4i* wsb = (const v4i*)a.wstream + (size_t)(half * NW + wave) * ((T0 + T1 + T2) * 64);
    v4i ring[R];
#pragma unroll
    for (int r = 0; r < R; ++r) ring[r] = wsb[r * 64 + lane];
    wsb += R * 64;

    if constexpr (C3) {
        asm volatile("s_waitcnt vmcnt(%0)" ::"n"(R) : "memory");
        __builtin_amdgcn_s_barrier();
        SABER_TL(1);
        const int xm0 = a.in0_u8 ? (int)0x80808080u : 0;
        const int c0 = wave * (C1 / NW) + fq * (4 * MF0);
        const v4i* pp = prm0 + (c0 / 4) * 3;
        v4i acc[MF0][TN];
#pragma unroll
        for (int mf = 0; mf < MF0; ++mf)
#pragma unroll
            for (int j = 0; j < TN; ++j) acc[mf][j] = pp[mf * 3 + 2];
        const v4i* hb = halo + (frow * S0) * PCH + fq;
#pragma unroll
        for (int s = 0; s < T0; ++s) {
            const int mf = s % MF0, ks = (s / MF0) % KS1, tap = s / (MF0 * KS1);
            const int dy = tap / 3, dx = tap % 3;
#pragma unroll
            for (int j = 0; j < TN; ++j) {
                v4i b = hb[((j * S0 + dy) * HW + dx) * PCH + ks * 4];
                b.x ^= xm0; b.y ^= xm0; b.z ^= xm0; b.w ^= xm0;
                acc[mf][j] = mma_step(ring[s % R], b, acc[mf][j]);
            }
            ring[s % R] = wsb[s * 64 + lane];
        }
        wsb += T0 * 64;
        const float lo0 = a.relu0 ? 0.f : -3.0e38f;
        const float off0 = a.in_u8 ? 0.f : 128.f;
        const unsigned xo0 = a.in_u8 ? 0u : 0x80808080u;
#pragma unroll
        for (int j = 0; j < TN; ++j) {
            unsigned o[MF0];
#pragma unroll
            for (int mf = 0; mf < MF0; ++mf)
                o[mf] = chain_out_pack(acc[mf][j], v4i{0, 0, 0, 0}, __builtin_bit_cast(v4f, pp[mf * 3 + 1]),
                                       __builtin_bit_cast(v4f, pp[mf * 3]), lo0, off0, xo0);
            char* mp = (char*)mid + (j * 16 + frow) * (PCH * 16) + c0;
            if constexpr (MF0 == 1) *(unsigned*)mp = o[0];
            else if constexpr (MF0 == 2) *(uint2*)mp = make_uint2(o[0], o[1]);
            else *(uint4*)mp = make_uint4(o[0], o[1], o[2], o[3]);
        }
        asm volatile("s_waitcnt lgkmcnt(0)" ::: "memory");
        __builtin_amdgcn_s_barrier();
#pragma unroll
        for (int j = 0; j < TN; ++j)
#pragma unroll
            for (int ks = 0; ks < KS1; ++ks) bx[ks][j] = mid[(j * 16 + frow) * PCH + ks * 4 + fq];
    }

    const int xmask = a.in_u8 ? (int)0x80808080u : 0;
#pragma unroll
    for (int ks = 0; ks < KS1; ++ks)
// ... 74 lines not shown
    }
    v4i b2[KS2][TN];
#pragma unroll
    for (int j = 0; j < TN; ++j)
#pragma unroll
        for (int ks = 0; ks < KS2; ++ks) b2[ks][j] = tile[(j * 16 + frow) * CPR + ((ks * 4 + fq) ^ frow)];
    SABER_TL(4);

#pragma unroll 1
    for (int g = 0; g < G2; ++g) {
        v4i acc[MFG2][TN];
        const int cg = half * K2W + wave * (K2W / NW) + g * (16 * MFG2) + fq * (4 * MFG2);
        const bool side_b = a.k2_split > 0 && wave * (K2W / NW) + g * (16 * MFG2) >= a.k2_split;
        const float lo2 = (side_b ? a.relu2b : a.relu2) ? 0.f : -3.0e38f;
        const float off2 = (side_b ? a.out_u8_2b : a.out_u8_2) ? 0.f : 128.f;
        const unsigned xm2 = (side_b ? a.out_u8_2b : a.out_u8_2) ? 0u : 0x80808080u;
        const int kout = a.k2_split > 0 ? (side_b ? K2 - a.k2_split : a.k2_split) : K2;
        char* yout = side_b ? (char*)a.y2b - a.k2_split : (char*)a.y2;
        const v4i* pp = prm2 + (cg / 4) * 3;
#pragma unroll
        for (int mf = 0; mf < MFG2; ++mf)
#pragma unroll
            for (int j = 0; j < TN; ++j) acc[mf][j] = pp[mf * 3 + 2];
#pragma unroll
        for (int s = 0; s < SG2; ++s) {
            const int ri = (OFF + s) % R;
            const int ks = s / MFG2, mf = s % MFG2;
#pragma unroll
            for (int j = 0; j < TN; ++j) acc[mf][j] = mma_step(ring[ri], b2[ks][j], acc[mf][j]);
            if (s + R < SG2 || g + 1 < G2) ring[ri] = wsb[s * 64 + lane];
        }
        wsb += SG2 * 64;
        unsigned o[MFG2];
#pragma unroll
        for (int j = 0; j < TN; ++j) {
#pragma unroll
            for (int mf = 0; mf < MFG2; ++mf)
                o[mf] = chain_out_pack(acc[mf][j], v4i{0, 0, 0, 0}, __builtin_bit_cast(v4f, pp[mf * 3 + 1]),
                                       __builtin_bit_cast(v4f, pp[mf * 3]), lo2, off2, xm2);
            bool ok;
            const int p = pix(j * 16 + frow, ok);
            if (ok) {
                char* y = yout + (size_t)p * kout + cg;
                if constexpr (MFG2 == 1) *(unsigned*)y = o[0];
                else if constexpr (MFG2 == 2) *(uint2*)y = make_uint2(o[0], o[1]);
                else *(uint4*)y = make_uint4(o[0], o[1], o[2], o[3]);
            }
        }
    }
    SABER_TL(5);
    SABER_TL_FLUSH();
}

bool conv1x1_chain_ok(int c1, int k1, int k2) {
    return (c1 == 64 || c1 == 128 || c1 == 256 || c1 == 512) && k1 == 4 * c1 && k2 == c1;
}

hipError_t launch_conv1x1_chain(const ChainKArgs& a, int c1, int k1, int k2, int rows, int waves, int split, int with3x3, hipStream_t s) {
    const bool has2 = k2 != 0;
    const bool pair2 = has2 && a.k2_split > 0;
    if (pair2 && !(a.s0 == 2 && with3x3 && c1 == 64 && k1 == 256 && k2 == 640 && a.k2_split % 32 == 0 && a.k2_split < 640)) return hipErrorInvalidValue;
    if (!conv1x1_chain_ok(c1, k1, (has2 && !pair2) ? k2 : c1) || a.M <= 0 || (!has2 && !with3x3)) return hipErrorInvalidValue;
    const dim3 block(64 * waves);
    const dim3 grid((with3x3 ? a.tiles_per_img * a.N : (a.M + 16 * rows - 1) / (16 * rows)) * split);
    enum { PLAIN, LED, HEAD, SHEAD, PAIR };
    const int kind = pair2 ? PAIR : (!has2 ? (a.s0 == 2 ? SHEAD : HEAD) : (with3x3 ? LED : PLAIN));
#define SABER_CHAIN(KIND, C1, ROWS, NW, SP, KS1, G1, MFG2, G2, R)                                                                   \
    case (((KIND * 1024 + C1) * 8 + ROWS) * 16 + NW) * 4 + SP:                                                                      \
        hipLaunchKernelGGL((conv1x1_chain_kernel<KS1, G1, MFG2, G2, ROWS, R, KIND != PLAIN, SP, KIND == PLAIN || KIND == LED || KIND == PAIR, NW, \
                                                 KIND == SHEAD || KIND == PAIR ? 2 : 1>), grid, block, 0, s, a);                   \
        break;
#define SABER_CHAIN_W4(KIND)                          \
    SABER_CHAIN(KIND, 64, 4, 4, 1, 1, 1, 1, 1, 4)     \
    SABER_CHAIN(KIND, 64, 2, 4, 1, 1, 1, 1, 1, 4)     \
    SABER_CHAIN(KIND, 128, 2, 4, 1, 2, 2, 2, 1, 8)    \
    SABER_CHAIN(KIND, 128, 1, 4, 1, 2, 2, 2, 1, 8)    \
    SABER_CHAIN(KIND, 256, 1, 4, 1, 4, 4, 4, 1, 16)
#define SABER_CHAIN_C128_W8(KIND)                     \
    SABER_CHAIN(KIND, 128, 2, 8, 1, 2, 1, 1, 1, 8)    \
    SABER_CHAIN(KIND, 128, 1, 8, 1, 2, 1, 1, 1, 8)
    switch ((((kind * 1024 + c1) * 8 + rows) * 16 + waves) * 4 + split) {
    SABER_CHAIN(PAIR, 64, 4, 4, 1, 1, 1, 2, 5, 4)
    SABER_CHAIN(PAIR, 64, 2, 4, 1, 1, 1, 2, 5, 4)
    SABER_CHAIN_W4(SHEAD)
    SABER_CHAIN(SHEAD, 256, 1, 8, 1, 4, 2, 2, 1, 16)
    SABER_CHAIN_C128_W8(SHEAD)
    SABER_CHAIN_W4(HEAD)
    SABER_CHAIN(HEAD, 256, 1, 8, 1, 4, 2, 2, 1, 16)
    SABER_CHAIN_C128_W8(HEAD)
    SABER_CHAIN_W4(PLAIN)
    SABER_CHAIN(PLAIN, 256, 1, 4, 2, 4, 4, 2, 1, 16)
    SABER_CHAIN(PLAIN, 256, 1, 8, 2, 4, 2, 1, 1, 16)
    SABER_CHAIN(PLAIN, 512, 1, 4, 1, 8, 8, 4, 2, 16)
    SABER_CHAIN(PLAIN, 512, 1, 4, 2, 8, 8, 4, 1, 16)
    SABER_CHAIN_W4(LED)
    SABER_CHAIN(LED, 256, 1, 8, 1, 4, 2, 2, 1, 16)
    SABER_CHAIN_C128_W8(PLAIN)
    SABER_CHAIN_C128_W8(LED)
    default: return hipErrorInvalidValue;
    }
#undef SABER_CHAIN_C128_W8
#undef SABER_CHAIN_W4
#undef SABER_CHAIN
    return hipGetLastError();
}

}
```

### anakin_amd/csrc/kernels.h

```cpp
#pragma once
#include <hip/hip_runtime.h>
#include <stddef.h>
#include <stdint.h>

#ifdef SABER_TIMELINE
extern __device__ unsigned long long* saber_tl_buf;
#define SABER_TL_DECL unsigned long long tl_[16] = {0, 0, 0, 0, 0, 0, 0, 0, 0, 0, 0, 0, 0, 0, 0, 0}
#define SABER_TL(i) tl_[i] = wall_clock64()
#define SABER_TL_FLUSH()                                                                   \
    do {                                                                                   \
        if (threadIdx.x == 0 && saber_tl_buf)                                              \
            for (int i_ = 0; i_ < 16; ++i_) saber_tl_buf[(size_t)blockIdx.x * 16 + i_] = tl_[i_]; \
    } while (0)
#else
#define SABER_TL_DECL do { } while (0)
#define SABER_TL(i) do { } while (0)
#define SABER_TL_FLUSH() do { } while (0)
#endif

namespace saber_mi355x {

enum { DT_F32 = 0, DT_S8 = 1, DT_U8 = 2 };

enum {
// ... 42 lines not shown
    int K1, K2, relu2, out_dtype2;
    int pool_oh, pool_ow;
    int res_sub, res_H, res_W;
    int w_plane_chunks;
    int ksplit_sh;
    float* part;
    unsigned* part_ctr;
    unsigned* part_err;
};

struct ImgKArgs {
    ConvKArgs c;
    int ib, rb, nw, nrs;
    unsigned mg[6];
};
static_assert(offsetof(ConvKArgs, y) == 128, "hot kernel arguments fill exactly the first two 64-byte lines");

struct StemPairTail {
    const void* w;
    const void* prm;
    void* y1;
    void* y2;
    int K1, K2;
    int relu1, relu2, u8_1, u8_2;
};
struct StemPairKArgs {
    ConvKArgs c;
    StemPairTail t;
};

constexpr int STAGE_MAX_TENSORS = 24;
struct ChainKArgs {
    const void* x;
    const void* wstream;
    const void* res;
    const void* prm1;
    const void* prm2;
    void* y1;
    void* y2;
    int M, in_u8;
    int relu1, res_relu;
    float coeff_conv, scale_conv, coeff_res, scale_res;
    int relu2, out_u8_2;
    const void* prm0;
    const void* zero;
    int N, H, W;
    int tiles_x, tiles_per_img;
    unsigned mg_tiles_x, mg_tpi;
    int in0_u8, relu0;
    int s0, H0, W0;
    int res_sub, res_H, res_W;
    void* y2b;
    int k2_split, relu2b, out_u8_2b;
};
struct CoopKArgs {
    ChainKArgs c;
    unsigned long long* coop_ctr;
    void* coop_xch;
    unsigned* coop_xcc;
    unsigned* coop_err;
    int n_tiles;
};
bool conv1x1_chain_ok(int c1, int k1, int k2);
hipError_t launch_conv1x1_chain(const ChainKArgs& a, int c1, int k1, int k2, int rows, int waves, int split, int with3x3, hipStream_t s);
hipError_t launch_conv_chain_coop(const CoopKArgs& a, hipStream_t s);

struct StageBlk {
    const void* wstream;
    const void* prm0;
    const void* prm1;
    const void* prm2;
    float coeff_conv, scale_conv, coeff_res, scale_res;
    int in0_u8, relu0, in_u8, relu1, res_relu, relu2, out_u8_2, pad_;
};
template <int MAXB>
struct Stage4KArgs {
    const void* x;
    const void* res;
    const void* zero;
    const StageBlk* blk;
    unsigned long long* grp_ctr;
    unsigned long long* img_ctr;
    void* xch;
    unsigned* xcc;
    unsigned* err;
    int nblk, N, H, W;
    int tiles_x, tiles_per_img;
    unsigned mg_tiles_x, mg_tpi, mg_wpi;
    int per_image;
    void* y1[MAXB];
    void* y2[MAXB];
    void* head_y;
};
constexpr int STAGE4_SHORT = 8, STAGE4_LONG = 24;
hipError_t launch_conv_stage4(const Stage4KArgs<STAGE4_SHORT>& a, bool tail, bool head, hipStream_t s);
hipError_t launch_conv_stage4(const Stage4KArgs<STAGE4_LONG>& a, bool tail, bool head, hipStream_t s);
hipError_t launch_conv_stage1_c128(const Stage4KArgs<STAGE4_SHORT>& a, hipStream_t s);
hipError_t launch_conv_stage1_c128(const Stage4KArgs<STAGE4_LONG>& a, hipStream_t s);
hipError_t launch_conv_stage1_c64(const Stage4KArgs<STAGE4_SHORT>& a, hipStream_t s);
hipError_t launch_conv_stage1_c64(const Stage4KArgs<STAGE4_LONG>& a, hipStream_t s);
int conv_stage1_c64_blocks_per_cu();

struct StagePhase {
    int type;
    int cin, cout;
    int in_t, out_t, res_t;
    int in_u8, relu, out_u8;
    int elt, res_relu;
    float coeff_conv, scale_conv, coeff_res, scale_res;
    unsigned w_chunk, prm_chunk;
    int barrier;
    int reload;
    unsigned pch, mg_pch;
    int red_chunk;
    int pool_t;
    float pool_idiv;
// ... 231 lines not shown
```

### anakin_amd/lib.py

```python
import ctypes as C
import os

HERE = os.path.dirname(os.path.abspath(__file__))
LIB_PATH = os.environ.get("SABER_MI355X_LIB") or os.path.join(HERE, "libsaber_mi355x.so")

F32, S8, U8, S32 = 0, 1, 2, 3
NHWC, NCHW = 0, 1
ACT_NONE, ACT_RELU = 0, 1
POOL_MAX, POOL_AVG_INCL, POOL_AVG_EXCL = 0, 1, 2
RES_NONE, RES_SUM_INPLACE, RES_ELTWISE = 0, 1, 2
TILES = ["32x32", "64x32", "64x64", "128x64", "64x128", "128x128"]

SYMBOLS = [
    "saber_hip_last_error", "saber_hip_device_ok",
    "saber_hip_conv2d_create", "saber_hip_conv2d_set_weights", "saber_hip_conv2d_workspace_bytes",
    "saber_hip_conv2d_out_shape", "saber_hip_conv2d_run", "saber_hip_conv2d_destroy",
    "saber_hip_conv2d_get_quantized_weights", "saber_hip_conv2d_algo", "saber_hip_conv2d_set_tile",
    "saber_hip_conv2d_get_tile", "saber_hip_conv2d_autotune", "saber_hip_conv2d_set_pooling",
    "saber_hip_conv2d_create_pair", "saber_hip_conv2d_run_pair", "saber_hip_conv2d_autotune_pair",
    "saber_hip_net_add_conv_pair",
    "saber_hip_conv2d_chain_create", "saber_hip_conv2d_chain_create3", "saber_hip_conv2d_chain_create3_pair", "saber_hip_conv2d_chain_destroy", "saber_hip_conv2d_chain_run",
    "saber_hip_conv2d_chain_run3",
    "saber_hip_conv2d_chain_set_tile", "saber_hip_conv2d_chain_get_tile",
    "saber_hip_conv2d_stage_create", "saber_hip_conv2d_stage_destroy", "saber_hip_conv2d_stage_run", "saber_hip_conv2d_stage_create_tail", "saber_hip_conv2d_stage_run_tail",
    "saber_hip_conv2d_stage_create_head", "saber_hip_conv2d_stage_run_head",
    "saber_hip_conv2d_stem_pair_create", "saber_hip_conv2d_stem_pair_destroy", "saber_hip_conv2d_stem_pair_run",
    "saber_hip_conv2d_sep_create", "saber_hip_conv2d_sep_run", "saber_hip_conv2d_sep_set_tile", "saber_hip_conv2d_sep_get_tile",
    "saber_hip_conv2d_sep_algo", "saber_hip_conv2d_sep_destroy",
    "saber_hip_conv2d_ir_create", "saber_hip_conv2d_ir_run", "saber_hip_conv2d_ir_set_tile", "saber_hip_conv2d_ir_get_tile",
    "saber_hip_conv2d_ir_algo", "saber_hip_conv2d_ir_destroy",
    "saber_hip_conv2d_set_global_pooling", "saber_hip_conv2d_run_gpool",
    "saber_hip_stage_create", "saber_hip_stage_num_tensors", "saber_hip_stage_run", "saber_hip_stage_status", "saber_hip_stage_trace", "saber_hip_stage_destroy",
    "saber_hip_fc_create", "saber_hip_fc_set_weights", "saber_hip_fc_workspace_bytes", "saber_hip_fc_run",
    "saber_hip_fc_destroy", "saber_hip_fc_algo", "saber_hip_fc_set_tile", "saber_hip_gemm_f32", "saber_hip_gemm_f32_release_plans",
    "saber_hip_gemm_i8_create", "saber_hip_gemm_i8_workspace_bytes", "saber_hip_gemm_i8_run", "saber_hip_gemm_i8_destroy",
    "saber_hip_quantize_nchw_to_nhwc", "saber_hip_dequantize_nhwc_to_nchw",
    "saber_hip_transpose_nchw_to_nhwc_f32", "saber_hip_transpose_nhwc_to_nchw_f32",
    "saber_hip_quantize_flat_s8", "saber_hip_eltwise_sum_i8", "saber_hip_eltwise_sum_f32", "saber_hip_relu_f32", "saber_hip_activation_f32", "saber_hip_prelu_f32",
    "saber_hip_pool_out_dim", "saber_hip_pool_out_dim2", "saber_hip_pool2d_i8_nhwc", "saber_hip_pool2d_f32", "saber_hip_pool2d_f32_from_i8", "saber_hip_pool2d_f32_from_i8_q", "saber_hip_fc_run_q", "saber_hip_fc_run_softmax", "saber_hip_softmax_f32",
    "saber_hip_net_add_pool_f32_from_i8_q", "saber_hip_net_add_fc_q", "saber_hip_net_optimize", "saber_hip_net_num_launches", "saber_hip_net_tensor_unwritten", "saber_hip_net_get_choice", "saber_hip_net_set_choice", "saber_hip_net_stage_blocks", "saber_hip_net_stage_head", "saber_hip_net_time_op_in_pass", "saber_hip_net_status", "saber_hip_net_inject_coop_error", "saber_hip_net_coop_fallbacks", "saber_hip_coop_fallbacks_total",
    "saber_hip_net_create", "saber_hip_net_add_tensor", "saber_hip_net_add_conv", "saber_hip_net_add_fc",
    "saber_hip_net_add_quantize", "saber_hip_net_add_dequantize", "saber_hip_net_add_transpose_in_f32", "saber_hip_net_add_eltwise_i8",
    "saber_hip_net_add_eltwise_f32", "saber_hip_net_add_pool_i8", "saber_hip_net_add_pool_f32",
    "saber_hip_net_add_pool_f32_from_i8", "saber_hip_net_add_softmax", "saber_hip_net_set_lane", "saber_hip_net_finalize", "saber_hip_net_tensor_ptr",
    "saber_hip_net_arena_bytes", "saber_hip_net_num_ops", "saber_hip_net_run", "saber_hip_net_run_op",
    "saber_hip_net_capture", "saber_hip_net_replay", "saber_hip_net_time_ops", "saber_hip_net_time_pass", "saber_hip_net_op_work", "saber_hip_net_op_name",
    "saber_hip_net_autotune", "saber_hip_net_destroy",
    "saber_hip_net_add_relu_f32", "saber_hip_net_add_activation_f32", "saber_hip_net_bind_tensor", "saber_hip_net_num_tensors", "saber_hip_net_tensor_bytes",
    "saber_hip_capture_begin", "saber_hip_capture_end", "saber_hip_capture_active", "saber_hip_net_tensor_of_ptr",
    "saber_hip_net_compact_arena", "saber_hip_net_arena_compacted", "saber_hip_serving_streams",
    "saber_hip_concat_nhwc", "saber_hip_net_add_concat",
    "saber_hip_conv2d_fire_create", "saber_hip_conv2d_fire_run", "saber_hip_conv2d_fire_set_tile", "saber_hip_conv2d_fire_get_tile",
    "saber_hip_conv2d_fire_algo", "saber_hip_conv2d_fire_destroy",
    "saber_hip_deconv2d_create", "saber_hip_deconv2d_set_weights", "saber_hip_deconv2d_out_shape", "saber_hip_deconv2d_run",
    "saber_hip_deconv2d_algo", "saber_hip_deconv2d_set_tile", "saber_hip_deconv2d_get_tile", "saber_hip_deconv2d_destroy",
    "saber_hip_net_add_deconv",
]


class StagePhase(C.Structure):
    _fields_ = [("conv", C.c_void_p), ("in_", C.c_int), ("out", C.c_int), ("res", C.c_int)]


class ConvDesc(C.Structure):
    _fields_ = [(n, C.c_int) for n in
                ("n", "h", "w", "c", "k", "kh", "kw", "pad_h", "pad_w", "stride_h", "stride_w", "dil_h", "dil_w",
                 "group", "in_dtype", "out_dtype", "in_layout", "out_layout", "act", "res_mode", "res_act")] + \
               [("sum_scale", C.c_float), ("coeff_conv", C.c_float), ("coeff_res", C.c_float),
                ("scale_res", C.c_float), ("int8_weights", C.c_int), ("act_negative_slope", C.c_float),
                ("res_has_dtype", C.c_int), ("res_dtype", C.c_int), ("res_stride", C.c_int), ("res_h", C.c_int),
                ("res_w", C.c_int)]


class FcDesc(C.Structure):
    _fields_ = [(n, C.c_int) for n in ("m", "n", "k", "in_dtype", "int8_weights", "w_is_kn")]


class SaberHipError(RuntimeError):
    pass


_lib = None


def load():
    global _lib
    if _lib is not None:
        return _lib
    try:
        import torch
    except ImportError:
        pass
    if not os.path.exists(LIB_PATH):
        raise SaberHipError(
            "anakin_amd/libsaber_mi355x.so is missing - build it with `python anakin_amd/build.py` "
            "(there is no CPU fallback for the MI355X Saber target)")
    lib = C.CDLL(LIB_PATH)
    P, I, F, Z = C.c_void_p, C.c_int, C.c_float, C.c_size_t
    lib.saber_hip_last_error.restype = C.c_char_p
    lib.saber_hip_conv2d_create.argtypes = [C.POINTER(ConvDesc), C.POINTER(P)]
    lib.saber_hip_conv2d_set_weights.argtypes = [P, P, I, P, P, F, F]
    lib.saber_hip_conv2d_workspace_bytes.argtypes = [P]
    lib.saber_hip_conv2d_workspace_bytes.restype = Z
    lib.saber_hip_conv2d_out_shape.argtypes = [P, C.POINTER(I), C.POINTER(I)]
    lib.saber_hip_conv2d_out_shape.restype = None
    lib.saber_hip_conv2d_run.argtypes = [P, P, P, P, P, P]
    lib.saber_hip_conv2d_destroy.argtypes = [P]
    lib.saber_hip_conv2d_destroy.restype = None
    lib.saber_hip_conv2d_get_quantized_weights.argtypes = [P, P, P]
    lib.saber_hip_conv2d_algo.argtypes = [P]
    lib.saber_hip_conv2d_algo.restype = C.c_char_p
    lib.saber_hip_conv2d_set_tile.argtypes = [P, I]
    lib.saber_hip_conv2d_get_tile.argtypes = [P]
    lib.saber_hip_conv2d_set_pooling.argtypes = [P] + [I] * 8
    lib.saber_hip_conv2d_autotune.argtypes = [P, P, P, P, P, P, I]
    lib.saber_hip_conv2d_create_pair.argtypes = [P, P, C.POINTER(P)]
    lib.saber_hip_conv2d_run_pair.argtypes = [P, P, P, P, P]
    lib.saber_hip_conv2d_autotune_pair.argtypes = [P, P, P, P, P, I]
    lib.saber_hip_net_add_conv_pair.argtypes = [P, P, I, I, I]
    lib.saber_hip_conv2d_chain_create.argtypes = [P, P, C.POINTER(P)]
    lib.saber_hip_conv2d_chain_create3.argtypes = [P, P, P, C.POINTER(P)]
    lib.saber_hip_net_tensor_unwritten.argtypes = [P, I]
    lib.saber_hip_net_num_launches.argtypes = [P]
    lib.saber_hip_conv2d_chain_destroy.argtypes = [P]
    lib.saber_hip_conv2d_chain_destroy.restype = None
    lib.saber_hip_conv2d_chain_run.argtypes = [P, P, P, P, P, P]
    lib.saber_hip_conv2d_chain_create3_pair.argtypes = [P, P, P, P, C.POINTER(P)]
    lib.saber_hip_conv2d_chain_run3.argtypes = [P, P, P, P, P, P, P]
    lib.saber_hip_conv2d_chain_set_tile.argtypes = [P, I]
    lib.saber_hip_conv2d_chain_get_tile.argtypes = [P]
    lib.saber_hip_conv2d_stage_create.argtypes = [C.POINTER(P), I, C.POINTER(P)]
    lib.saber_hip_conv2d_stage_destroy.argtypes = [P]
    lib.saber_hip_conv2d_stage_destroy.restype = None
    lib.saber_hip_conv2d_stage_run.argtypes = [P, P, P, C.POINTER(P), C.POINTER(P), P]
    lib.saber_hip_conv2d_stage_create_tail.argtypes = [C.POINTER(P), I, P, C.POINTER(P)]
    lib.saber_hip_conv2d_stage_run_tail.argtypes = [P, P, P, C.POINTER(P), C.POINTER(P), P, P]
    lib.saber_hip_conv2d_stage_create_head.argtypes = [C.POINTER(P), I, P, P, P, C.POINTER(P)]
    lib.saber_hip_conv2d_stage_run_head.argtypes = [P, P, P, C.POINTER(P), C.POINTER(P), P, P]
    lib.saber_hip_conv2d_stem_pair_create.argtypes = [P, P, P, C.POINTER(P)]
    lib.saber_hip_conv2d_stem_pair_destroy.argtypes = [P]
    lib.saber_hip_conv2d_stem_pair_destroy.restype = None
    lib.saber_hip_conv2d_stem_pair_run.argtypes = [P, P, P, P, P, P, P]
    lib.saber_hip_conv2d_sep_create.argtypes = [P, P, C.POINTER(P)]
    lib.saber_hip_conv2d_sep_run.argtypes = [P, P, P, P, P]
    lib.saber_hip_conv2d_sep_set_tile.argtypes = [P, I]
    lib.saber_hip_conv2d_sep_get_tile.argtypes = [P]
    lib.saber_hip_conv2d_sep_algo.argtypes = [P]
    lib.saber_hip_conv2d_sep_algo.restype = C.c_char_p
    lib.saber_hip_conv2d_sep_destroy.argtypes = [P]
    lib.saber_hip_conv2d_sep_destroy.restype = None
    lib.saber_hip_conv2d_ir_create.argtypes = [P, P, P, C.POINTER(P)]
    lib.saber_hip_conv2d_ir_run.argtypes = [P, P, P, P, P, P]
    lib.saber_hip_conv2d_ir_set_tile.argtypes = [P, I]
    lib.saber_hip_conv2d_ir_get_tile.argtypes = [P]
    lib.saber_hip_conv2d_ir_algo.argtypes = [P]
    lib.saber_hip_conv2d_ir_algo.restype = C.c_char_p
    lib.saber_hip_conv2d_ir_destroy.argtypes = [P]
    lib.saber_hip_conv2d_ir_destroy.restype = None
    lib.saber_hip_conv2d_set_global_pooling.argtypes = [P]
    lib.saber_hip_conv2d_run_gpool.argtypes = [P, P, P, P, P, P]
    lib.saber_hip_stage_create.argtypes = [C.POINTER(StagePhase), I, C.POINTER(P)]
    lib.saber_hip_stage_num_tensors.argtypes = [P]
    lib.saber_hip_stage_run.argtypes = [P, C.POINTER(P), I, P]
    lib.saber_hip_stage_status.argtypes = [P]
    lib.saber_hip_stage_trace.argtypes = [P, P, C.c_size_t]
    lib.saber_hip_stage_destroy.argtypes = [P]
    lib.saber_hip_stage_destroy.restype = None
    lib.saber_hip_fc_create.argtypes = [C.POINTER(FcDesc), C.POINTER(P)]
    lib.saber_hip_fc_set_weights.argtypes = [P, P, I, P, P, F, F]
    lib.saber_hip_fc_workspace_bytes.argtypes = [P]
    lib.saber_hip_fc_workspace_bytes.restype = Z
    lib.saber_hip_fc_run.argtypes = [P, P, P, P, P]
    lib.saber_hip_fc_destroy.argtypes = [P]
    lib.saber_hip_net_optimize.argtypes = [P, I]
    lib.saber_hip_net_stage_blocks.argtypes = [P, I]
    lib.saber_hip_net_stage_head.argtypes = [P, I]
    lib.saber_hip_net_status.argtypes = [P]
    lib.saber_hip_net_inject_coop_error.argtypes = [P]
    lib.saber_hip_net_coop_fallbacks.argtypes = [P]
    lib.saber_hip_coop_fallbacks_total.argtypes = []
# ... 138 lines not shown
```

### anakin_amd/saber.py

```python
import ctypes as C

import numpy as np
import torch

from . import lib as L

_TORCH_DT = {L.F32: torch.float32, L.S8: torch.int8, L.U8: torch.uint8}


def _stream():
    return C.c_void_p(torch.cuda.current_stream().cuda_stream)


def _p(t):
    return None if t is None else C.c_void_p(t.data_ptr())


def _np_ptr(a):
    return None if a is None else a.ctypes.data_as(C.c_void_p)


def dtype_code(t):
    return {torch.float32: L.F32, torch.int8: L.S8, torch.uint8: L.U8}[t.dtype]

# ... 263 lines not shown
        return y


class SaberConvPair:

    def __init__(self, a, b):
        self.a, self.b = a, b
        self.h = C.c_void_p()
        L.check(L.load().saber_hip_conv2d_create_pair(a.h, b.h, C.byref(self.h)))

    def dispatch(self, x, ya, yb):
        L.check(L.load().saber_hip_conv2d_run_pair(self.h, _p(x), _p(ya), _p(yb), _stream()))
        return ya, yb

    def algo(self):
        return L.load().saber_hip_conv2d_algo(self.h).decode()

    def set_tile(self, tile):
        L.check(L.load().saber_hip_conv2d_set_tile(self.h, tile))

    def autotune(self, x, ya, yb, iters=5):
        L.check(L.load().saber_hip_conv2d_autotune_pair(self.h, _p(x), _p(ya), _p(yb), _stream(), iters))

    def __del__(self):
        try:
            if self.h:
                L.load().saber_hip_conv2d_destroy(self.h)
        except Exception:
            pass


ACTIVE_SIGMOID, ACTIVE_RELU, ACTIVE_TANH, ACTIVE_CLIPPED_RELU, ACTIVE_ELU, ACTIVE_STANH, ACTIVE_PRELU, ACTIVE_GELU, ACTIVE_SWISH = \
    1, 2, 3, 4, 5, 9, 10, 11, 12


def activation(active, x, y=None, negative_slope=0.0, coef=1.0):
    import torch
    if y is None:
        y = torch.empty_like(x)
    L.check(L.load().saber_hip_activation_f32(int(active), x.numel(), float(negative_slope), float(coef), _p(x), _p(y), _stream()))
    return y


def prelu(x, slope, channels, inner, channel_shared=False, y=None):
    import torch
    if y is None:
        y = torch.empty_like(x)
    L.check(L.load().saber_hip_prelu_f32(x.numel(), int(channels), int(inner), int(bool(channel_shared)), _p(slope), _p(x), _p(y), _stream()))
    return y


class SaberConvChain:

    def __init__(self, a, b, conv3x3=None, pair_b=None):
        self.a, self.b, self.c3, self.b2 = a, b, conv3x3, pair_b
        self.h = C.c_void_p()
        if pair_b is not None:
            L.check(L.load().saber_hip_conv2d_chain_create3_pair(conv3x3.h, a.h, b.h, pair_b.h, C.byref(self.h)))
        elif conv3x3 is None:
            L.check(L.load().saber_hip_conv2d_chain_create(a.h, b.h, C.byref(self.h)))
        else:
            L.check(L.load().saber_hip_conv2d_chain_create3(conv3x3.h, a.h, None if b is None else b.h, C.byref(self.h)))

    def dispatch(self, x, res, ya, yb=None, yc=None):
        L.check(L.load().saber_hip_conv2d_chain_run3(self.h, _p(x), _p(res), _p(ya), _p(yb), _p(yc), _stream()))
        return ya, yb

    def set_tile(self, tn):
        L.check(L.load().saber_hip_conv2d_chain_set_tile(self.h, tn))

    def tile(self):
        return L.load().saber_hip_conv2d_chain_get_tile(self.h)

    def __del__(self):
        try:
            if self.h:
                L.load().saber_hip_conv2d_chain_destroy(self.h)
        except Exception:
            pass


class SaberChainStage:

    def __init__(self, chains, tail=None, head=None):
        self.chains = list(chains)
        self.tail = tail
        self.head = head
        arr = (C.c_void_p * len(chains))(*[c.h for c in chains])
        self.h = C.c_void_p()
        if head is not None:
            L.check(L.load().saber_hip_conv2d_stage_create_head(arr, len(chains), tail.h if tail is not None else None, head[0].h, head[1].h,
                                                                C.byref(self.h)))
        elif tail is None:
            L.check(L.load().saber_hip_conv2d_stage_create(arr, len(chains), C.byref(self.h)))
        else:
            L.check(L.load().saber_hip_conv2d_stage_create_tail(arr, len(chains), tail.h, C.byref(self.h)))

    def dispatch(self, x, res, y1s, y2s, y_tail=None):
        n = len(self.chains)
        a = (C.c_void_p * n)(*[t.data_ptr() if t is not None else None for t in y1s])
        b = (C.c_void_p * n)(*[t.data_ptr() for t in y2s])
        if y_tail is None:
            L.check(L.load().saber_hip_conv2d_stage_run(self.h, _p(x), _p(res), a, b, _stream()))
        else:
            L.check(L.load().saber_hip_conv2d_stage_run_tail(self.h, _p(x), _p(res), a, b, _p(y_tail), _stream()))

    def dispatch_head(self, x_head, y_head_b, y1s, y2s, y_tail=None):
        n = len(self.chains)
        a = (C.c_void_p * n)(*[t.data_ptr() for t in y1s])
        b = (C.c_void_p * n)(*[t.data_ptr() for t in y2s])
# ... 712 lines not shown
```

### anakin_amd/workloads.py

```python
import numpy as np

F32, S8, U8 = 0, 1, 2


def resnet_spec(depth=50):
    return _bottleneck_spec({50: [3, 4, 6, 3], 101: [3, 4, 23, 3]}[depth], 64, 4, 1, False)


def resnext_spec():
    return _bottleneck_spec([3, 4, 6, 3], 128, 2, 32, True)


def _bottleneck_spec(blocks, width, expand, group, stride_3x3):
    L = []
    L.append(dict(kind="conv", name="conv1", src="data", cin=3, cout=64, k=7, stride=2, pad=3, relu=True))
    L.append(dict(kind="pool", name="pool1", src="conv1", win=3, stride=2, pad=0, type=0))
    prev, cin, hw = "pool1", 64, 56
    for si, nb in enumerate(blocks):
        mid = width << si
        cout = mid * expand
        for bi in range(nb):
            stride = 2 if (bi == 0 and si > 0) else 1
            tag = "res%d%s" % (si + 2, chr(ord("a") + bi) if nb <= 6 else ("a" if bi == 0 else "b%d" % bi))
            if bi == 0:
# ... 293 lines not shown
            odt = l.get("odt", U8 if l["relu"] else S8)
            p = S.ConvParam(w, b, l.get("group", 1), (l["pad"],) * 2, (l["stride"],) * 2, (1, 1), l["relu"])
            shape[nm], dtype[nm] = (ho, l["cout"]), odt
            conv = S.SaberConv2D(True).init((B, cin, hin, hin), p, dtype[l["src"]], odt, scales[l["src"]], scales[nm],
                                            in_layout=L.NCHW if dtype[l["src"]] == F32 else L.NHWC)
            net.add_tensor(nm, (B, ho, ho, l["cout"]), odt)
            net.add_conv(conv, l["src"], nm)
        elif kd == "pool":
            hin, c = shape[l["src"]]
            ho = S.pool_out_dim(hin, l["pad"], l["win"], l["stride"], l.get("floor", False))
            shape[nm], dtype[nm] = (ho, c), dtype[l["src"]]
            scales[nm] = scales[l["src"]]
            net.add_tensor(nm, (B, ho, ho, c), dtype[nm])
            net.add_pool_i8(B, hin, hin, c, ho, ho, (l["win"],) * 2, (l["stride"],) * 2, (l["pad"],) * 2, l["type"],
                            dtype[l["src"]], dtype[nm], l["src"], nm)
        elif kd == "eltwise":
            ho, c = shape[l["a"]]
            shape[nm], dtype[nm] = (ho, c), S8
            net.add_tensor(nm, (B, ho, ho, c), S8)
            coeff = 1.0 / scales[nm]
            net.add_eltwise_i8(B * ho * ho * c, scales[l["a"]], scales[l["b"]], coeff, coeff, l["relu"], l["a"], l["b"], nm)
        elif kd == "concat":
            ho, dt = shape[l["srcs"][0]][0], dtype[l["srcs"][0]]
            chans = [shape[s][1] for s in l["srcs"]]
            cat = S.SaberConcat().init(chans, dt, [scales[s] for s in l["srcs"]])
            shape[nm], dtype[nm], scales[nm] = (ho, sum(chans)), dt, cat.out_scale
            net.add_tensor(nm, (B, ho, ho, sum(chans)), dt)
            net.add_concat(l["srcs"], nm, cat)
        elif kd == "gpool" and l.get("int8"):
            hin, c = shape[l["src"]]
            shape[nm], dtype[nm] = (1, c), dtype[l["src"]]
            scales[nm] = scales[l["src"]]
            net.add_tensor(nm, (B, 1, 1, c), dtype[nm])
            net.add_pool_i8(B, hin, hin, c, 1, 1, (hin, hin), (hin, hin), (0, 0), 1, dtype[l["src"]], dtype[nm], l["src"], nm)
        elif kd == "gpool":
            hin, c = shape[l["src"]]
            net.add_tensor(nm, (B, c, 1, 1), F32)
            net.add_pool_f32_from_i8(B, hin, hin, c, 1, 1, (hin, hin), (hin, hin), (0, 0), 1, dtype[l["src"]],
                                     scales[l["src"]], l["src"], nm)
            shape[nm], dtype[nm] = (1, c), F32
        elif kd == "fc":
            w, b = model["params"][nm]
            fc = S.SaberFc(True).init(B, l["cout"], l["cin"], w, b, dtype.get(l["src"], F32), scales[l["src"]])
            net.add_tensor(nm, (B, l["cout"]), F32)
            net.add_fc(fc, l["src"], nm)
        elif kd == "softmax":
            classes = next(e.get("cout", shape.get(l["src"], (0, 0))[1]) for e in model["spec"] if e["name"] == l["src"])
            net.add_tensor(nm, (B, classes), F32)
            net.add_softmax(B, classes, l["src"], nm)
    net.unfused_ops = net.num_ops()
    if shared_device:
        net.optimize(2048)
        stage = False
    net.removed = net.absorbed = net.gpooled = net.stem_paired = net.chained = net.fc_softmaxed = net.separated = net.inverted = net.fired = 0
    if fuse:
        net.removed = net.optimize(15)
    if fire:
        net.fired = net.optimize(65536)
    if inverted:
        net.inverted = net.optimize(32768)
    if separable:
        net.separated = net.optimize(16384)
    if fuse:
        net.absorbed = net.optimize(64) if absorb_pool else 0
        net.gpooled = net.optimize(128) if absorb_pool else 0
        net.stem_paired = net.optimize(512) if stem_pair else 0
        net.chained = net.optimize(16 | (32 if int(chain) >= 2 else 0) | (256 if int(chain) >= 2 and stage else 0) |
                                   (1024 if int(chain) >= 2 and head_pair else 0)) if chain else 0
        net.fc_softmaxed = net.optimize(4096) if fc_softmax else 0
    if before_finalize is not None:
        before_finalize(net)
    net.finalize()
    return net


def build_fp32_net(model, batch, hw=224, pair_siblings=True, fuse_pool=True, shared_device=False, reproducible=False, fuse_stem=True,
                   fc_softmax=True):
    from . import lib as L
    from . import saber as S
    net = S.Net()
    B = batch
    net.add_tensor("data", (B, 3, hw, hw), F32)
    spec = model["spec"]
    shape, alias = {}, {}
    fused_away = set()
    done_convs = set()
    produced = []
    l0, l1 = spec[0], (spec[1] if len(spec) > 1 else None)
    if fuse_stem and l0["kind"] == "conv" and l0["src"] == "data" and l1 is not None and l1["kind"] == "pool" and l1["src"] == l0["name"] \
            and l1["type"] == 0 and l0["relu"] and sum(1 for e in spec for k in ("src", "a", "b") if e.get(k) == l0["name"]) == 1:
        w0, b0 = model["params"][l0["name"]]
        p0 = S.ConvParam(w0, b0, 1, (l0["pad"],) * 2, (l0["stride"],) * 2, (1, 1), True)
        cp0 = S.SaberConv2DPooling(int8=False).init((B, 3, hw, hw), p0, l1["type"], (l1["win"],) * 2, (l1["stride"],) * 2, (l1["pad"],) * 2,
                                                     F32, F32, floor_mode=l1.get("floor", False), in_layout=L.NCHW)
        if cp0.fused and cp0.algo().startswith("stem7x7s2_maxpool3x3s2_f32"):
            po = cp0.out_hw[0]
            net.add_tensor(l1["name"], (B, po, po, l0["cout"]), F32)
            shape[l1["name"]] = (po, l0["cout"])
            net.add_conv(cp0.conv, "data", l1["name"])
            net.keep.append(cp0)
            produced.append((net.num_ops() - 1, l1["name"]))
            fused_away.add(l1["name"])
            done_convs.add(l0["name"])
    if not done_convs:
        net.add_tensor("data_nhwc", (B, hw, hw, 4), F32)
        net.add_transpose_in(B, 3, hw, hw, 4, "data", "data_nhwc")
        shape["data_nhwc"] = (hw, 4)
        alias["data"] = "data_nhwc"

    def T(n):
        return alias.get(n, n)
    sib = {}
    consumers = {}
    for e in spec:
        for src in [e[key] for key in ("src", "a", "b") if key in e] + list(e.get("srcs", ())):
            consumers[src] = consumers.get(src, 0) + 1
    def mark(*names):
        for n_ in names:
            produced.append((net.num_ops() - 1, n_))
    for li, l in enumerate(spec):
        kd, nm = l["kind"], l["name"]
# ... 124 lines not shown
```

### include/saber_hip.h

```cpp
#ifndef SABER_HIP_H
#define SABER_HIP_H

#include <stddef.h>
#include <stdint.h>

#ifdef __cplusplus
extern "C" {
#endif

typedef void* saber_hip_stream_t;

typedef enum {
    SABER_HIP_OK = 0,
    SABER_HIP_INVALID_VALUE = -2,
    SABER_HIP_UNIMPL = -3,
    SABER_HIP_OUT_OF_MEM = -4,
    SABER_HIP_RUNTIME_ERROR = -5
} saber_hip_status;

typedef enum { SABER_HIP_F32 = 0, SABER_HIP_S8 = 1, SABER_HIP_U8 = 2, SABER_HIP_S32 = 3 } saber_hip_dtype;
typedef enum { SABER_HIP_NHWC = 0, SABER_HIP_NCHW = 1 } saber_hip_layout;
typedef enum { SABER_HIP_ACT_NONE = 0, SABER_HIP_ACT_RELU = 1 } saber_hip_act;
typedef enum { SABER_HIP_POOL_MAX = 0, SABER_HIP_POOL_AVG_INCL = 1, SABER_HIP_POOL_AVG_EXCL = 2 } saber_hip_pool_type;

// ... 10 lines not shown
    int n, h, w, c;
    int k;
    int kh, kw;
    int pad_h, pad_w, stride_h, stride_w, dil_h, dil_w, group;
    int in_dtype, out_dtype;
    int in_layout, out_layout;
    int act;
    int res_mode;
    int res_act;
    float sum_scale;
    float coeff_conv, coeff_res;
    float scale_res;
    int int8_weights;
    float act_negative_slope;
    int res_has_dtype;
    int res_dtype;
    int res_stride;
    int res_h, res_w;
} saber_hip_conv_desc;

typedef struct saber_hip_conv saber_hip_conv_t;

int saber_hip_conv2d_create(const saber_hip_conv_desc* desc, saber_hip_conv_t** out);
int saber_hip_conv2d_set_weights(saber_hip_conv_t* op, const void* w, int w_dtype, const float* w_scale,
                                 const float* bias, float in_scale, float out_scale);
size_t saber_hip_conv2d_workspace_bytes(const saber_hip_conv_t* op);
void saber_hip_conv2d_out_shape(const saber_hip_conv_t* op, int* oh, int* ow);
int saber_hip_conv2d_run(saber_hip_conv_t* op, const void* x, void* y, const void* res, void* workspace,
                         saber_hip_stream_t stream);
void saber_hip_conv2d_destroy(saber_hip_conv_t* op);
int saber_hip_conv2d_set_pooling(saber_hip_conv_t* op, int pool_type, int kh, int kw, int stride_h, int stride_w,
                                 int pad_h, int pad_w, int floor_mode);
int saber_hip_conv2d_get_quantized_weights(const saber_hip_conv_t* op, int8_t* wq_oihw, float* w_scale);
const char* saber_hip_conv2d_algo(const saber_hip_conv_t* op);
int saber_hip_conv2d_set_tile(saber_hip_conv_t* op, int tile);
int saber_hip_conv2d_get_tile(const saber_hip_conv_t* op);
int saber_hip_conv2d_autotune(saber_hip_conv_t* op, const void* x, void* y, const void* res, void* workspace,
                              saber_hip_stream_t stream, int iters);

int saber_hip_conv2d_set_global_pooling(saber_hip_conv_t* op);
int saber_hip_conv2d_run_gpool(saber_hip_conv_t* op, const void* x, void* y, const void* res, void* y_pool,
                               saber_hip_stream_t stream);

int saber_hip_conv2d_create_pair(const saber_hip_conv_t* a, const saber_hip_conv_t* b, saber_hip_conv_t** out);
int saber_hip_conv2d_run_pair(saber_hip_conv_t* pair, const void* x, void* y_a, void* y_b, saber_hip_stream_t stream);
int saber_hip_conv2d_autotune_pair(saber_hip_conv_t* pair, const void* x, void* y_a, void* y_b,
                                   saber_hip_stream_t stream, int iters);

typedef struct saber_hip_chain saber_hip_chain_t;
int saber_hip_conv2d_chain_create(saber_hip_conv_t* a, saber_hip_conv_t* b, saber_hip_chain_t** out);
int saber_hip_conv2d_chain_create3(saber_hip_conv_t* conv3x3, saber_hip_conv_t* a, saber_hip_conv_t* b, saber_hip_chain_t** out);
int saber_hip_conv2d_chain_create3_pair(saber_hip_conv_t* conv3x3, saber_hip_conv_t* a, saber_hip_conv_t* pair_a, saber_hip_conv_t* pair_b,
                                        saber_hip_chain_t** out);
void saber_hip_conv2d_chain_destroy(saber_hip_chain_t* chain);
int saber_hip_conv2d_chain_run(saber_hip_chain_t* chain, const void* x, const void* res, void* y_a, void* y_b,
                               saber_hip_stream_t stream);
int saber_hip_conv2d_chain_run3(saber_hip_chain_t* chain, const void* x, const void* res, void* y_a, void* y_b, void* y_c,
                                saber_hip_stream_t stream);
int saber_hip_conv2d_chain_set_tile(saber_hip_chain_t* chain, int tn);
int saber_hip_conv2d_chain_get_tile(const saber_hip_chain_t* chain);

typedef struct saber_hip_chain_stage saber_hip_chain_stage_t;
int saber_hip_conv2d_stage_create(saber_hip_chain_t* const* chains, int n, saber_hip_chain_stage_t** out);
void saber_hip_conv2d_stage_destroy(saber_hip_chain_stage_t* stage);
int saber_hip_conv2d_stage_run(saber_hip_chain_stage_t* stage, const void* x, const void* res, void* const* y1, void* const* y2,
                               saber_hip_stream_t stream);
int saber_hip_conv2d_stage_create_tail(saber_hip_chain_t* const* chains, int n, saber_hip_chain_t* tail, saber_hip_chain_stage_t** out);
int saber_hip_conv2d_stage_run_tail(saber_hip_chain_stage_t* stage, const void* x, const void* res, void* const* y1, void* const* y2,
                                    void* y_tail, saber_hip_stream_t stream);

int saber_hip_conv2d_stage_create_head(saber_hip_chain_t* const* chains, int n, saber_hip_chain_t* tail, const saber_hip_conv_t* head_a,
                                       const saber_hip_conv_t* head_b, saber_hip_chain_stage_t** out);
int saber_hip_conv2d_stage_run_head(saber_hip_chain_stage_t* stage, const void* x_head, void* y_head_b, void* const* y1, void* const* y2,
                                    void* y_tail, saber_hip_stream_t stream);

typedef struct saber_hip_stem_pair saber_hip_stem_pair_t;
int saber_hip_conv2d_stem_pair_create(saber_hip_conv_t* stem, const saber_hip_conv_t* a, const saber_hip_conv_t* b, saber_hip_stem_pair_t** out);
void saber_hip_conv2d_stem_pair_destroy(saber_hip_stem_pair_t* sp);
int saber_hip_conv2d_stem_pair_run(saber_hip_stem_pair_t* sp, const void* x, void* y_pool, void* y_a, void* y_b, void* workspace,
                                   saber_hip_stream_t stream);

typedef struct saber_hip_sep saber_hip_sep_t;
int saber_hip_conv2d_sep_create(saber_hip_conv_t* dw, saber_hip_conv_t* pw, saber_hip_sep_t** out);
int saber_hip_conv2d_sep_run(saber_hip_sep_t* sep, const void* x, void* y_dw , void* y_pw, saber_hip_stream_t stream);
int saber_hip_conv2d_sep_set_tile(saber_hip_sep_t* sep, int code);
int saber_hip_conv2d_sep_get_tile(const saber_hip_sep_t* sep);
const char* saber_hip_conv2d_sep_algo(const saber_hip_sep_t* sep);
void saber_hip_conv2d_sep_destroy(saber_hip_sep_t* sep);

typedef struct saber_hip_ir saber_hip_ir_t;
int saber_hip_conv2d_ir_create(saber_hip_conv_t* expand, saber_hip_conv_t* dw, saber_hip_conv_t* project, saber_hip_ir_t** out);
int saber_hip_conv2d_ir_run(saber_hip_ir_t* ir, const void* x, void* y_expand , void* y_dw , void* y,
                            saber_hip_stream_t stream);
int saber_hip_conv2d_ir_set_tile(saber_hip_ir_t* ir, int code);
int saber_hip_conv2d_ir_get_tile(const saber_hip_ir_t* ir);
const char* saber_hip_conv2d_ir_algo(const saber_hip_ir_t* ir);
void saber_hip_conv2d_ir_destroy(saber_hip_ir_t* ir);

typedef struct saber_hip_fire saber_hip_fire_t;
int saber_hip_conv2d_fire_create(saber_hip_conv_t* squeeze, saber_hip_conv_t* e1, saber_hip_conv_t* e3, saber_hip_fire_t** out);
int saber_hip_conv2d_fire_run(saber_hip_fire_t* fire, const void* x, void* y_squeeze , void* y, saber_hip_stream_t stream);
int saber_hip_conv2d_fire_set_tile(saber_hip_fire_t* fire, int code);
int saber_hip_conv2d_fire_get_tile(const saber_hip_fire_t* fire);
const char* saber_hip_conv2d_fire_algo(const saber_hip_fire_t* fire);
void saber_hip_conv2d_fire_destroy(saber_hip_fire_t* fire);

// ... 69 lines not shown
                        saber_hip_stream_t stream);
int saber_hip_concat_nhwc(size_t pixels, int n_inputs, const void* const* xs, const int* channels, const float* mult, int dtype,
                          void* y, saber_hip_stream_t stream);
int saber_hip_pool_out_dim(int in, int pad, int window, int stride, int floor_mode);
int saber_hip_pool_out_dim2(int in, int pad, int window, int stride, int floor_mode, int any_pad);
int saber_hip_pool2d_i8_nhwc(int n, int h, int w, int c, int oh, int ow, int kh, int kw, int stride_h,
                             int stride_w, int pad_h, int pad_w, int pool_type, int in_dtype, int out_dtype,
                             const void* x, void* y, saber_hip_stream_t stream);
int saber_hip_pool2d_f32(int n, int h, int w, int c, int oh, int ow, int kh, int kw, int stride_h,
                         int stride_w, int pad_h, int pad_w, int pool_type, int layout, const float* x,
                         float* y, saber_hip_stream_t stream);
int saber_hip_pool2d_f32_from_i8(int n, int h, int w, int c, int oh, int ow, int kh, int kw, int stride_h,
                                 int stride_w, int pad_h, int pad_w, int pool_type, int in_dtype, float scale,
                                 const void* x, float* y, saber_hip_stream_t stream);
int saber_hip_pool2d_f32_from_i8_q(int n, int h, int w, int c, int oh, int ow, int kh, int kw, int stride_h,
                                   int stride_w, int pad_h, int pad_w, int pool_type, int in_dtype, float scale,
                                   const void* x, float* y, float q_scale, int8_t* yq, saber_hip_stream_t stream);
int saber_hip_softmax_f32(int rows, int cols, const float* x, float* y, saber_hip_stream_t stream);

typedef struct saber_hip_net saber_hip_net_t;
int saber_hip_net_create(saber_hip_net_t** out);
int saber_hip_net_add_tensor(saber_hip_net_t* net, size_t bytes);
int saber_hip_net_add_conv(saber_hip_net_t* net, saber_hip_conv_t* op, int in_id, int out_id, int res_id);
int saber_hip_net_add_conv_pair(saber_hip_net_t* net, saber_hip_conv_t* pair, int in_id, int out_a_id, int out_b_id);
int saber_hip_net_add_fc(saber_hip_net_t* net, saber_hip_fc_t* op, int in_id, int out_id);
int saber_hip_net_add_quantize(saber_hip_net_t* net, int n, int c, int h, int w, int c_pad, int out_dtype,
                               float scale, int in_id, int out_id);
int saber_hip_net_add_dequantize(saber_hip_net_t* net, int n, int c, int h, int w, int in_dtype, float scale,
                                 int in_id, int out_id);
int saber_hip_net_add_transpose_in_f32(saber_hip_net_t* net, int n, int c, int h, int w, int c_pad, int in_id,
                                       int out_id);
int saber_hip_net_add_eltwise_i8(saber_hip_net_t* net, size_t count, float scale_a, float scale_b,
                                 float coeff_a, float coeff_b, int relu, int a_id, int b_id, int out_id);
int saber_hip_net_add_eltwise_f32(saber_hip_net_t* net, size_t count, float coeff_a, float coeff_b, int relu,
                                  int a_id, int b_id, int out_id);
int saber_hip_net_add_pool_i8(saber_hip_net_t* net, int n, int h, int w, int c, int oh, int ow, int kh, int kw,
                              int stride_h, int stride_w, int pad_h, int pad_w, int pool_type, int in_dtype,
                              int out_dtype, int in_id, int out_id);
int saber_hip_net_add_pool_f32(saber_hip_net_t* net, int n, int h, int w, int c, int oh, int ow, int kh, int kw,
                               int stride_h, int stride_w, int pad_h, int pad_w, int pool_type, int layout,
                               int in_id, int out_id);
int saber_hip_net_add_pool_f32_from_i8(saber_hip_net_t* net, int n, int h, int w, int c, int oh, int ow, int kh,
                                       int kw, int stride_h, int stride_w, int pad_h, int pad_w, int pool_type,
                                       int in_dtype, float scale, int in_id, int out_id);
int saber_hip_net_add_pool_f32_from_i8_q(saber_hip_net_t* net, int n, int h, int w, int c, int oh, int ow, int kh, int kw,
                                         int stride_h, int stride_w, int pad_h, int pad_w, int pool_type, int in_dtype,
                                         float scale, int in_id, int out_id, float q_scale, int q_out_id);
int saber_hip_net_add_fc_q(saber_hip_net_t* net, saber_hip_fc_t* op, int in_q_id, int out_id);
#define SABER_HIP_NET_SHARED_DEVICE 2048
#define SABER_HIP_NET_REPRODUCIBLE_FP32 8192
#define SABER_HIP_NET_SEPARABLE 16384
#define SABER_HIP_NET_INVERTED_RESIDUAL 32768
#define SABER_HIP_NET_FIRE 65536
int saber_hip_net_optimize(saber_hip_net_t* net, int flags);
int saber_hip_net_coop_fallbacks(const saber_hip_net_t* net);
int saber_hip_coop_fallbacks_total(void);
int saber_hip_net_status(saber_hip_net_t* net);
int saber_hip_net_inject_coop_error(saber_hip_net_t* net);
int saber_hip_net_stage_blocks(const saber_hip_net_t* net, int index);
int saber_hip_net_stage_head(const saber_hip_net_t* net, int index);
int saber_hip_net_num_launches(const saber_hip_net_t* net);
int saber_hip_net_tensor_unwritten(const saber_hip_net_t* net, int id);
int saber_hip_net_add_softmax(saber_hip_net_t* net, int rows, int cols, int in_id, int out_id);
int saber_hip_net_set_lane(saber_hip_net_t* net, int op_index, int lane);
int saber_hip_net_finalize(saber_hip_net_t* net);
void* saber_hip_net_tensor_ptr(saber_hip_net_t* net, int id);
size_t saber_hip_net_arena_bytes(const saber_hip_net_t* net);
int saber_hip_net_compact_arena(saber_hip_net_t* net, const int* keep, int n_keep);
int saber_hip_net_arena_compacted(const saber_hip_net_t* net);
int saber_hip_net_num_ops(const saber_hip_net_t* net);
int saber_hip_net_run(saber_hip_net_t* net, saber_hip_stream_t stream);
int saber_hip_net_run_op(saber_hip_net_t* net, int index, saber_hip_stream_t stream);
int saber_hip_net_capture(saber_hip_net_t* net, saber_hip_stream_t stream);
int saber_hip_net_replay(saber_hip_net_t* net, saber_hip_stream_t stream);
int saber_hip_net_time_ops(saber_hip_net_t* net, saber_hip_stream_t stream, int iters, float* out_us);
int saber_hip_net_time_pass(saber_hip_net_t* net, saber_hip_stream_t stream, int iters, float* out_us);
int saber_hip_net_time_op_in_pass(saber_hip_net_t* net, saber_hip_stream_t stream, int index, int iters, float* out_us);
int saber_hip_net_op_work(const saber_hip_net_t* net, int index, double* bytes, double* flops);
const char* saber_hip_net_op_name(const saber_hip_net_t* net, int index);
int saber_hip_net_get_choice(saber_hip_net_t* net, int index);
int saber_hip_net_set_choice(saber_hip_net_t* net, int index, int choice);
int saber_hip_net_autotune(saber_hip_net_t* net, saber_hip_stream_t stream, int iters);
void saber_hip_net_destroy(saber_hip_net_t* net);
int saber_hip_net_add_relu_f32(saber_hip_net_t* net, size_t count, int in_id, int out_id);
int saber_hip_net_add_activation_f32(saber_hip_net_t* net, int active, size_t count, float negative_slope, float coef, int in_id,
                                     int out_id);
int saber_hip_net_add_concat(saber_hip_net_t* net, size_t pixels, int n_inputs, const int* in_ids, const int* channels,
                             const float* mult, int dtype, int out_id);
int saber_hip_net_add_deconv(saber_hip_net_t* net, saber_hip_deconv_t* op, int in_id, int out_id);
int saber_hip_net_bind_tensor(saber_hip_net_t* net, int id, void* ptr);
int saber_hip_net_num_tensors(const saber_hip_net_t* net);
size_t saber_hip_net_tensor_bytes(const saber_hip_net_t* net, int id);

int saber_hip_capture_begin(void);
int saber_hip_capture_end(saber_hip_net_t** out);
int saber_hip_capture_active(void);
int saber_hip_net_tensor_of_ptr(const saber_hip_net_t* net, const void* ptr);

int saber_hip_serving_streams(int n, saber_hip_stream_t* out, int* distinct);

#ifdef __cplusplus
}
#endif
#endif
```

Measured before the change: 39690.

## Split the stage-transition sibling pair into trailing-conv and projection-fused chains

```diff
diff --git a/anakin_amd/csrc/api_chain.hip b/anakin_amd/csrc/api_chain.hip
--- a/anakin_amd/csrc/api_chain.hip
+++ b/anakin_amd/csrc/api_chain.hip
@@ -20,7 +20,7 @@
 };
 static void for_each_chain_form(const saber_hip_chain* ch, const std::function<void(const ChainForm&)>& fn) {
     for (const auto& r : chain_forms)
-        if (r.c1 == ch->c1 && (r.kinds & chain_kind(ch))) fn(r.f);
+        if (r.c1 == ch->c1 && (r.kinds & chain_kind(ch)) && (!ch->proj || (r.f.waves == 8 && r.f.coop == 1))) fn(r.f);
 }
 static ChainForm chain_form_where(const saber_hip_chain* ch, const std::function<bool(const ChainForm& row, const ChainForm& found)>& take) {
     ChainForm f;
@@ -38,6 +38,8 @@
     const ChainForm& f = ch->form;
     const std::string c = std::to_string(ch->c1), w8 = f.waves == 8 && f.coop == 1 ? "_w8" : "";
     if (!ch->c3) return "chain1x1_c" + c + "_px" + std::to_string(16 * f.rows) + (f.split == 2 ? "_split2" : "") + w8;
+    if (ch->proj) return "[proj1x1]+conv3x3+chain1x1_c" + c + "_" + std::to_string(f.rows) + "x16" + w8;
+    if (ch->b && !ch->b2 && ch->c3->d.stride_h == 2) return "conv3x3+conv1x1+next1x1_c" + c + "_" + std::to_string(f.rows) + "x16" + w8;
     return std::string("conv3x3+") + (ch->b2 ? "conv1x1+pair1x1_c" : (ch->b ? "chain1x1_c" : "conv1x1_c")) + c + "_" + std::to_string(f.rows) + "x16" + w8 +
            (f.coop == 2 ? "_coop2" : "") + (f.coop == 4 ? "_coop4" : "");
 }
@@ -423,6 +425,7 @@
     switch (layout) {
     case CS_BASE: case CS_W8:
         for (int w = 0; w < nw; ++w) {
+            if (ch->proj) pack_chain_weights(ch->proj->wq_oihw.data(), ch->proj->d.k, ch->proj->d.c, 4, w, out, 0, nw);
             if (c3) pack_chain_weights3(w3, c, w, out, nw);
             pack_chain_weights(wa, k1, c, 4, w, out, 0, nw);
             if (b) pack_chain_weights(wb, k2, c2, mfg(k2), w, out, 0, nw);
@@ -446,10 +449,12 @@
     default: pack_coop4_stream(w3, wa, wb, out);
     }
 }
-static int chain_build(saber_hip_conv* c3, saber_hip_conv* a, saber_hip_conv* b, saber_hip_chain_t** out, saber_hip_conv* b2 = nullptr) {
-    if (!a || !out || (!b && !c3) || (b2 && (!b || !c3))) return fail(SABER_HIP_INVALID_VALUE, "null argument");
+static int chain_build(saber_hip_conv* c3, saber_hip_conv* a, saber_hip_conv* b, saber_hip_chain_t** out, saber_hip_conv* b2 = nullptr, bool trail = false,
+                       saber_hip_conv* proj = nullptr) {
+    if (!a || !out || (!b && !c3) || (b2 && (!b || !c3)) || (trail && (!b || !c3 || b2)) || (proj && (!b || !c3 || b2 || trail))) return fail(SABER_HIP_INVALID_VALUE, "null argument");
     const bool pair2 = b2 != nullptr;
-    const bool strided = c3 && (!b || pair2) && c3->d.stride_h == 2 && c3->d.stride_w == 2;
+    const bool strided = c3 && (!b || pair2 || trail) && c3->d.stride_h == 2 && c3->d.stride_w == 2;
+    if (trail && !strided) return fail(SABER_HIP_INVALID_VALUE, "chain: a trailing conv follows the strided head (conv3x3 / stride 2 + conv1x1 + eltwise) only");
     if (pair2 && !strided) return fail(SABER_HIP_INVALID_VALUE, "chain: a sibling pair follows the strided head (conv3x3 / stride 2 + conv1x1 + eltwise) only");
     if (!chain_1x1(a, strided) || (b && !chain_1x1(b)) || (b2 && !chain_1x1(b2)))
         return fail(SABER_HIP_INVALID_VALUE, "chain: both ops must be plain 1x1 stride-1 INT8 NHWC convs with weights set");
@@ -462,7 +467,9 @@
         const saber_hip_conv_desc& db = b->d;
         if (db.res_mode != SABER_HIP_RES_NONE || b->x_dtype != DT_S8 || (db.out_dtype != SABER_HIP_S8 && db.out_dtype != SABER_HIP_U8))
             return fail(SABER_HIP_INVALID_VALUE, "chain: the second conv must be a plain s8-input conv with an 8-bit output");
-        if (db.n != da.n || db.h != a->oh || db.w != a->ow || db.c != da.k || (!pair2 && db.k != da.c))
+        if (trail && (da.c != 64 || db.k != 128))
+            return fail(SABER_HIP_INVALID_VALUE, "chain: the trailing conv after a strided head: 64 -> 256 (+ eltwise) -> 128");
+        if (db.n != da.n || db.h != a->oh || db.w != a->ow || db.c != da.k || (!pair2 && !trail && db.k != da.c))
             return fail(SABER_HIP_INVALID_VALUE, "chain: shapes must be C -> 4C -> C with C in {64,128,256,512} on the same pixels");
     }
     if (pair2) {
@@ -470,6 +477,14 @@
         if (d2.res_mode != SABER_HIP_RES_NONE || b2->x_dtype != DT_S8 || (d2.out_dtype != SABER_HIP_S8 && d2.out_dtype != SABER_HIP_U8) || d2.n != da.n ||
             d2.h != a->oh || d2.w != a->ow || d2.c != da.k || da.c != 64 || db.k % 32 || db.k + d2.k != 640 || d2.k <= 0)
             return fail(SABER_HIP_INVALID_VALUE, "chain: the sibling pair after a strided head: 64 -> 256 (+ eltwise) -> k_b | k_b2 with k_b + k_b2 = 640, k_b % 32 == 0, 8-bit outputs");
+    }
+    if (proj) {
+        const saber_hip_conv_desc& dp = proj->d;
+        if (!chain_1x1(proj) || dp.res_mode != SABER_HIP_RES_NONE || dp.out_dtype != SABER_HIP_S8 || dp.c != 256 || dp.k != da.k || da.c != 128 || dp.n != da.n ||
+            dp.h != da.h || dp.w != da.w || (proj->x_dtype != DT_S8 && proj->x_dtype != DT_U8) || (int)proj->wq_oihw.size() != dp.k * dp.c || !c3 ||
+            c3->d.stride_h != 1)
+            return fail(SABER_HIP_INVALID_VALUE, "chain: the projection shortcut must be a plain 1x1 / stride-1 INT8 NHWC conv 256 -> 512 (s8 out) on the pixels of a "
+                                                  "3x3-led C = 128 chain");
     }
     if (!conv1x1_chain_ok(da.c, da.k, da.c))
         return fail(SABER_HIP_INVALID_VALUE, "chain: shapes must be C -> 4C -> C with C in {64,128,256,512} on the same pixels");
@@ -487,7 +502,7 @@
     }
     saber_hip_chain* ch = new saber_hip_chain();
     const int k2 = b ? b->d.k + (pair2 ? b2->d.k : 0) : 0;
-    ch->c3 = c3; ch->a = a; ch->b = b; ch->b2 = b2; ch->c1 = da.c; ch->k1 = da.k; ch->k2 = k2;
+    ch->c3 = c3; ch->a = a; ch->b = b; ch->b2 = b2; ch->proj = proj; ch->c1 = da.c; ch->k1 = da.k; ch->k2 = k2;
     ch->scale_conv = a->out_scale;
     if (c3 && !b && da.c == 256 && strided) {
         ch->tail_w3 = c3->wq_oihw;
@@ -519,7 +534,7 @@
         if (e == hipSuccess) e = hipHostMalloc((void**)&ch->h_coop_err, sizeof(unsigned), hipHostMallocMapped);
         if (e == hipSuccess) *ch->h_coop_err = 0u;
     }
-    if (e == hipSuccess && (da.c == 128 || da.c == 64) && c3 && b && !pair2 && c3->d.stride_h == 1 && xcd_round_robin()) {
+    if (e == hipSuccess && (da.c == 128 || da.c == 64) && c3 && b && !pair2 && !proj && c3->d.stride_h == 1 && xcd_round_robin()) {
         std::vector<uint8_t> s1;
         if (da.c == 128) pack_stage1_c128_stream(c3, a, b, s1);
         else pack_stage1_c64_stream(c3->wq_oihw.data(), a->wq_oihw.data(), b->wq_oihw.data(), s1);
@@ -527,6 +542,11 @@
     }
     if (e == hipSuccess) e = ch->d_prm1.upload(p1);
     if (e == hipSuccess && b) e = ch->d_prm2.upload(p2);
+    if (e == hipSuccess && proj) {
+        std::vector<uint8_t> pp;
+        pack_chain_params(proj, (size_t)proj->d.k / 4 * 3, pp);
+        e = ch->d_prmp.upload(pp);
+    }
     if (e == hipSuccess && c3) {
         pack_chain_params(c3, ((size_t)da.c / 4 * 3 + 63) / 64 * 64 + 64, p0);
         e = ch->d_prm0.upload(p0);
@@ -557,6 +577,23 @@
                                         saber_hip_chain_t** out) {
     if (!conv3x3 || !pair_a || !pair_b) return fail(SABER_HIP_INVALID_VALUE, "null argument");
     return chain_build(conv3x3, a, pair_a, out, pair_b);
+}
+int saber_hip_conv2d_chain_create3_trail(saber_hip_conv_t* conv3x3, saber_hip_conv_t* a, saber_hip_conv_t* next, saber_hip_chain_t** out) {
+    if (!conv3x3 || !next) return fail(SABER_HIP_INVALID_VALUE, "null argument");
+    return chain_build(conv3x3, a, next, out, nullptr, true);
+}
+int saber_hip_conv2d_chain_create3_proj(saber_hip_conv_t* proj, saber_hip_conv_t* conv3x3, saber_hip_conv_t* a, saber_hip_conv_t* b, saber_hip_chain_t** out) {
+    if (!proj || !conv3x3 || !b) return fail(SABER_HIP_INVALID_VALUE, "null argument");
+    return chain_build(conv3x3, a, b, out, nullptr, false, proj);
+}
+int saber_hip_conv2d_chain_pack_weights_host(const int8_t* w_oihw, int k, int c, int acc_per_group, int waves, uint8_t* out, size_t out_bytes) {
+    if (!w_oihw || !out || k <= 0 || c <= 0 || c % 64 || (waves != 4 && waves != 8) || acc_per_group < 1 || acc_per_group > 4 || k % (waves * 16 * acc_per_group))
+        return fail(SABER_HIP_INVALID_VALUE, "chain pack: k a multiple of waves x 16 x accumulators, c of 64");
+    std::vector<uint8_t> v;
+    for (int w = 0; w < waves; ++w) pack_chain_weights(w_oihw, k, c, acc_per_group, w, v, 0, waves);
+    if (v.size() != out_bytes) return fail(SABER_HIP_INVALID_VALUE, "chain pack: the stream has k x c bytes");
+    std::memcpy(out, v.data(), v.size());
+    return SABER_HIP_OK;
 }
 void saber_hip_conv2d_chain_destroy(saber_hip_chain_t* ch) { delete ch; }
 int saber_hip_conv2d_chain_set_tile(saber_hip_chain_t* ch, int tn) {
@@ -592,6 +629,11 @@
         k.relu2 = b->d.act == SABER_HIP_ACT_RELU;
         k.out_u8_2 = b->d.out_dtype == SABER_HIP_U8;
     }
+    if (ch->proj) {
+        k.prmp = ch->d_prmp.p;
+        k.proj_in_u8 = ch->proj->x_dtype == DT_U8;
+        k.proj_relu = ch->proj->d.act == SABER_HIP_ACT_RELU;
+    }
     if (ch->b2) {
         k.y2b = y_c;
         k.k2_split = b->d.k;
diff --git a/anakin_amd/csrc/api_internal.h b/anakin_amd/csrc/api_internal.h
--- a/anakin_amd/csrc/api_internal.h
+++ b/anakin_amd/csrc/api_internal.h
@@ -200,6 +200,8 @@
     saber_hip_conv* a = nullptr;
     saber_hip_conv* b = nullptr;
     saber_hip_conv* b2 = nullptr;
+    saber_hip_conv* proj = nullptr;
+    DevBuf<uint8_t> d_prmp;
     int c1 = 0, k1 = 0, k2 = 0;
     float scale_conv = 1.f;
     std::vector<int8_t> tail_w3, tail_wa;
@@ -360,7 +362,7 @@
 
 namespace saber_api {
 enum OpKind { OP_CONV, OP_CONV_PAIR, OP_FC, OP_QUANT, OP_DEQUANT, OP_TRANSPOSE_IN, OP_ELT_I8, OP_ELT_F32, OP_POOL_I8, OP_POOL_F32, OP_POOL_F32_I8, OP_FC_Q, OP_SOFTMAX, OP_RELU_F32, OP_ACT_F32, OP_CONCAT, OP_DECONV };
-enum Launch { LAUNCH_NONE, LAUNCH_OWN, LAUNCH_CHAIN, LAUNCH_CHAIN3, LAUNCH_STAGE, LAUNCH_STEM_PAIR, LAUNCH_SEP, LAUNCH_IR, LAUNCH_FIRE };
+enum Launch { LAUNCH_NONE, LAUNCH_OWN, LAUNCH_CHAIN, LAUNCH_CHAIN3, LAUNCH_STAGE, LAUNCH_STEM_PAIR, LAUNCH_SEP, LAUNCH_IR, LAUNCH_FIRE, LAUNCH_SPLIT };
 struct NetOp {
     OpKind kind;
     std::string name;
@@ -401,6 +403,9 @@
     saber_hip_fire* fire = nullptr;
     int fire_out = -1;
     bool fire_on = false;
+    saber_hip_chain* split = nullptr;
+    int split_res = -1, split_y1 = -1, split_y2 = -1, split_b1 = -1;
+    bool split_site = false, split_on = false;
     int lane = 0;
     bool record = false;
     int p[16] = {0};
@@ -506,6 +511,7 @@
 void net_set_chain_mode(saber_hip_net* net, int ia, int mode);
 int net_chain_mode(const saber_hip_net* net, int ia);
 void net_set_stage(saber_hip_net* net, int i0, bool on);
+void net_set_split(saber_hip_net* net, int ip, bool on, int head_code = 0, int proj_code = 0);
 void net_set_head(saber_hip_net* net, int i0, bool on);
 void net_set_tail(saber_hip_net* net, int i0, bool on);
 ChainForm chain_form(const saber_hip_chain* ch, int code);
diff --git a/anakin_amd/csrc/api_net.hip b/anakin_amd/csrc/api_net.hip
--- a/anakin_amd/csrc/api_net.hip
+++ b/anakin_amd/csrc/api_net.hip
@@ -44,6 +44,7 @@
             }
             return rc;
         }
+        case LAUNCH_SPLIT: return saber_hip_conv2d_chain_run3(o.split, T(o.in), T(o.split_res), T(o.split_y1), T(o.split_y2), nullptr, s);
         case LAUNCH_CHAIN: return saber_hip_conv2d_chain_run(o.chain, T(o.in), T(o.in2), T(o.out), T(o.chain_out), s);
         case LAUNCH_SEP: return saber_hip_conv2d_sep_run(o.sep, T(o.in), nullptr, T(o.sep_out), s);
         case LAUNCH_IR: return saber_hip_conv2d_ir_run(o.ir, T(o.in), nullptr, nullptr, T(o.ir_out), s);
@@ -334,6 +335,7 @@
         if (o.stage) span(i, 3 * o.stage_n + (o.stage->tail ? 2 : 0));
         if (o.stage && o.stage->head_a && i > 0) span(i - 1, 2);
         if (o.chain3) span(i, 3);
+        if (o.split) span(i, 3);
         if (o.chain) span(i, 2);
         if (o.stem_pair) span(i, 2);
         if (o.sep) span(i, 2);
@@ -343,8 +345,8 @@
     }
     for (int i = 0; i < nops; ++i) {
         const NetOp& o = net->ops[i];
-        const int rd[] = {o.in, o.in2, o.chain3_res};
-        const int wr[] = {o.out, o.out2, o.chain_out, o.chain3_y1, o.chain3_y2, o.chain3_y3, o.stem_y1, o.stem_y2, o.sep_out, o.ir_out, o.fire_out};
+        const int rd[] = {o.in, o.in2, o.chain3_res, o.split_res};
+        const int wr[] = {o.out, o.out2, o.chain_out, o.chain3_y1, o.chain3_y2, o.chain3_y3, o.split_y1, o.split_y2, o.stem_y1, o.stem_y2, o.sep_out, o.ir_out, o.fire_out};
         auto touch = [&](int t) {
             if (t < 0 || t >= nt) return;
             first[t] = std::min(first[t], g_lo[i]);
@@ -503,7 +505,7 @@
     if (index < 0 || index >= (int)net->ops.size() || lane < 0 || lane > 1) return fail(SABER_HIP_INVALID_VALUE, "bad op index / lane");
     if (net->lanes_ready) return fail(SABER_HIP_INVALID_VALUE, "lanes are fixed after the first run");
     for (const NetOp& o : net->ops)
-        if (lane && (o.chain || o.chain3 || o.stem_pair || o.sep || o.ir || o.fire))
+        if (lane && (o.chain || o.chain3 || o.split || o.stem_pair || o.sep || o.ir || o.fire))
             return fail(SABER_HIP_INVALID_VALUE, "the net has launches that span several ops' tensors (conv1x1 chains, the stem pair, separable sites): lanes must be assigned before saber_hip_net_optimize");
     if (lane) {
         const NetOp& o = net->ops[index];
@@ -681,7 +683,8 @@
     if (net->tensor_bytes[id] == 0) return 1;
     for (const NetOp& o : net->ops) {
         const Launch by = o.skip ? net->ops[o.absorbed_by].launch : o.launch;
-        if (o.out == id && (o.launch == LAUNCH_CHAIN3 || o.launch == LAUNCH_STEM_PAIR || o.launch == LAUNCH_SEP || (o.chain3 && by == LAUNCH_STAGE))) return 1;
+        if (o.launch == LAUNCH_SPLIT && o.split_b1 == id) return 1;
+        if (o.out == id && (o.launch == LAUNCH_CHAIN3 || o.launch == LAUNCH_SPLIT || o.launch == LAUNCH_STEM_PAIR || o.launch == LAUNCH_SEP || (o.chain3 && by == LAUNCH_STAGE))) return 1;
         if (o.out == id && (o.launch == LAUNCH_IR || (o.skip && by == LAUNCH_IR && (int)(&o - net->ops.data()) == o.absorbed_by + 1))) return 1;
         if (o.out == id && o.kind == OP_CONV && (o.launch == LAUNCH_FIRE || (o.skip && by == LAUNCH_FIRE))) return 1;
         if (o.launch == LAUNCH_STAGE && o.head_on && o.chain3_res == id) return 1;
diff --git a/anakin_amd/csrc/api_net_autotune.hip b/anakin_amd/csrc/api_net_autotune.hip
--- a/anakin_amd/csrc/api_net_autotune.hip
+++ b/anakin_amd/csrc/api_net_autotune.hip
@@ -22,6 +22,8 @@
     if (o.stage && o.stage_on) choice |= 1 << 30;
     if (o.stage && o.stage_on && o.tail_on) choice |= (int)0x80000000u;
     if (o.head_of >= 0 && net->ops[o.head_of].stage_on && net->ops[o.head_of].head_on) choice |= 1 << 29;
+    if (o.split_site && o.split_on)
+        choice |= (1 << 28) | ((net->ops[index - 2].split->form.code == 2 ? 1 : 0) << 24) | ((net->ops[index + 1].split->form.code == 5 ? 1 : 0) << 25);
     return choice;
 }
 int saber_hip_net_stage_blocks(const saber_hip_net_t* net, int index) {
@@ -85,6 +87,7 @@
     if (o.stage) net_set_stage(net, index, stage_on);
     if (o.stage) net_set_tail(net, index, tail_on);
     if (o.head_of >= 0) net_set_head(net, o.head_of, (chain_bits & 32) && !net->shared_device);
+    if (o.split_site) net_set_split(net, index, (chain_bits & 16) != 0, (chain_bits & 1) ? 2 : 4, (chain_bits & 2) ? 5 : 6);
     if (sep_bits) net_set_sep(net, index, tn);
     if (ir_bits) net_set_ir(net, index, ir_tn);
     if (fire_bits) net_set_fire(net, index, ir_tn);
@@ -225,6 +228,8 @@
     };
     for (size_t i = 0; i < net->ops.size(); ++i)
         if (net->ops[i].stage) net_set_stage(net, (int)i, false);
+    for (size_t i = 0; i < net->ops.size(); ++i)
+        if (net->ops[i].split_site) net_set_split(net, (int)i, false);
     for (size_t i = 0; i < net->ops.size(); ++i) {
         NetOp& A = net->ops[i];
         const int ia = (int)i;
@@ -316,6 +321,34 @@
         rc = run_all();
         if (rc) return rc;
     }
+    for (size_t i = 2; i + 3 < net->ops.size(); ++i) {
+        NetOp& P = net->ops[i];
+        if (!P.split_site || net->shared_device || (net->ops[i + 1].stage && net->ops[i + 1].stage_on)) continue;
+        hipStream_t s = (hipStream_t)stream;
+        auto run_all = [&]() -> int {
+            int rc = 0;
+            for (size_t k = i - 2; k <= i + 3; ++k) rc |= net_launch(net, net->ops[k], s);
+            return rc;
+        };
+        auto timed = [&](float* t) { return time_enqueued(s, run_all, 20, t); };
+        float sep = 0.f, best = 0.f;
+        int best_h = 0, best_p = 0;
+        int rc = timed(&sep);
+        if (rc) return rc;
+        log_cand(P.conv, "separate", sep);
+        best = sep * 0.99f;
+        for (int hc : {4, 2})
+            for (int pc : {6, 5}) {
+                float us = -1.f;
+                net_set_split(net, (int)i, true, hc, pc);
+                const int rt = timed(&us);
+                log_cand(P.conv, net->ops[i - 2].name.substr(5) + " | " + net->ops[i + 1].name.substr(5), us);
+                if (rt == SABER_HIP_OK && us > 0.f && us < best) { best = us; best_h = hc; best_p = pc; }
+            }
+        net_set_split(net, (int)i, best_h != 0, best_h, best_p);
+        rc = run_all();
+        if (rc) return rc;
+    }
     for (size_t i = 0; i + 1 < net->ops.size(); ++i) {
         NetOp& D = net->ops[i];
         if (!D.sep) continue;
diff --git a/anakin_amd/csrc/api_net_optimize.hip b/anakin_amd/csrc/api_net_optimize.hip
--- a/anakin_amd/csrc/api_net_optimize.hip
+++ b/anakin_amd/csrc/api_net_optimize.hip
@@ -37,6 +37,14 @@
         } else if (o.stem_pair) {
             o.launch = LAUNCH_STEM_PAIR;
             absorb(i + 1, i, IN_STEM);
+        } else if (o.split && i + 5 < n && ops[i + 2].split_site && ops[i + 2].split_on && !(ops[i + 3].stage && ops[i + 3].stage_on)) {
+            o.launch = LAUNCH_SPLIT;
+            absorb(i + 1, i, IN_CHAIN);
+            absorb(i + 2, i, IN_CHAIN);
+        } else if (o.split && i >= 3 && i + 2 < n && ops[i - 1].split_site && ops[i - 3].launch == LAUNCH_SPLIT) {
+            o.launch = LAUNCH_SPLIT;
+            absorb(i + 1, i, IN_CHAIN);
+            absorb(i + 2, i, IN_CHAIN);
         } else if (o.chain3 && o.led_on) {
             o.launch = LAUNCH_CHAIN3;
             absorb(i + 1, i, IN_CHAIN);
@@ -76,6 +84,7 @@
             case LAUNCH_OWN: o.name = "conv:" + own + o.res_note; break;
             case LAUNCH_CHAIN: o.name = "conv:" + chain_form_name(o.chain); break;
             case LAUNCH_CHAIN3: o.name = "conv:" + chain_form_name(o.chain3); break;
+            case LAUNCH_SPLIT: o.name = "conv:" + chain_form_name(o.split); break;
             case LAUNCH_SEP: o.name = std::string("conv:") + saber_hip_conv2d_sep_algo(o.sep); break;
             case LAUNCH_IR: o.name = std::string("conv:") + saber_hip_conv2d_ir_algo(o.ir); break;
             case LAUNCH_FIRE: o.name = std::string("conv:") + saber_hip_conv2d_fire_algo(o.fire); break;
@@ -107,6 +116,14 @@
     H0.tail_on = on;
     net_resolve(net);
 }
+void net_set_split(saber_hip_net* net, int ip, bool on, int head_code, int proj_code) {
+    if (ip < 2 || ip + 1 >= (int)net->ops.size() || !net->ops[ip].split_site) return;
+    saber_hip_chain *hd = net->ops[ip - 2].split, *pj = net->ops[ip + 1].split;
+    if (head_code && chain_form_valid(hd, head_code)) hd->form = chain_form(hd, head_code);
+    if (proj_code && chain_form_valid(pj, proj_code)) pj->form = chain_form(pj, proj_code);
+    net->ops[ip].split_on = on && !net->shared_device;
+    net_resolve(net);
+}
 void net_set_head(saber_hip_net* net, int i0, bool on) {
     NetOp& H0 = net->ops[i0];
     if (!H0.stage || !H0.stage->head_a || i0 < 1 || net->ops[i0 - 1].head_of != i0) return;
@@ -124,6 +141,7 @@
         }
     if (on) H0.tail_on = H0.stage->tail != nullptr;
     if (!on) H0.tail_on = H0.head_on = false;
+    if (on && i0 >= 1 && net->ops[i0 - 1].split_site) net->ops[i0 - 1].split_on = false;
     H0.stage_on = on;
     net_resolve(net);
 }
@@ -544,6 +562,37 @@
             if (Hd.led_on) removed += P ? 2 : 1;
         }
     }
+    if ((flags & SABER_HIP_NET_PAIR_SPLIT) && !two_lanes && !net->shared_device) {
+        for (size_t i = 0; i + 5 < ops.size(); ++i) {
+            NetOp &Hd = ops[i], &A = ops[i + 1], &P = ops[i + 2], &H2 = ops[i + 3], &A2 = ops[i + 4], &B2 = ops[i + 5];
+            if (Hd.kind != OP_CONV || A.kind != OP_CONV || P.kind != OP_CONV_PAIR || H2.kind != OP_CONV || A2.kind != OP_CONV || B2.kind != OP_CONV) continue;
+            if (!Hd.conv || !A.conv || !P.conv || !H2.conv || !A2.conv || !B2.conv || P.split_site || Hd.split || H2.split) continue;
+            if (!P.conv->pair_src_a || !P.conv->pair_src_b || (Hd.chain3 && Hd.chain3->b2)) continue;
+            bool busy = false;
+            for (size_t j = i; j <= i + 5; ++j) busy = busy || ops[j].lane || ops[j].stem_pair || ops[j].sep || in_ir(ops[j]) || (j > 0 && ops[j - 1].stem_pair);
+            if (busy || Hd.stage || Hd.tail_of >= 0 || P.head_of >= 0) continue;
+            if (Hd.in2 >= 0 || H2.in2 >= 0 || B2.in2 >= 0 || A.in != Hd.out || A.in2 < 0 || P.in != A.out || A2.in != H2.out || B2.in != A2.out) continue;
+            const bool fwd = A2.in2 == P.out && H2.in == P.out2, rev = A2.in2 == P.out2 && H2.in == P.out;
+            if (!(fwd || rev) || P.out == P.out2) continue;
+            const int t_b1 = fwd ? P.out : P.out2, t_b2a = fwd ? P.out2 : P.out;
+            if (readers(Hd.out) != 1 || readers(A.out) != 1 || readers(t_b1) != 1 || readers(t_b2a) != 1 || readers(H2.out) != 1) continue;
+            saber_hip_conv* b1 = const_cast<saber_hip_conv*>(fwd ? P.conv->pair_src_a : P.conv->pair_src_b);
+            saber_hip_conv* b2a = const_cast<saber_hip_conv*>(fwd ? P.conv->pair_src_b : P.conv->pair_src_a);
+            saber_hip_chain *hd = nullptr, *pj = nullptr;
+            if (saber_hip_conv2d_chain_create3_trail(Hd.conv, A.conv, b2a, &hd) != SABER_HIP_OK) continue;
+            if (saber_hip_conv2d_chain_create3_proj(b1, H2.conv, A2.conv, B2.conv, &pj) != SABER_HIP_OK) {
+                saber_hip_conv2d_chain_destroy(hd);
+                continue;
+            }
+            net->owned_chains.push_back(hd);
+            net->owned_chains.push_back(pj);
+            Hd.split = hd; Hd.split_res = A.in2; Hd.split_y1 = A.out; Hd.split_y2 = t_b2a;
+            H2.split = pj; H2.split_res = A.out; H2.split_y1 = A2.out; H2.split_y2 = B2.out; H2.split_b1 = t_b1;
+            P.split_site = true;
+            P.split_on = false;
+            ++removed;
+        }
+    }
     if ((flags & 256) && (flags & 32) && !two_lanes) {
         for (size_t i = 0; i + 2 < ops.size();) {
             auto block_ok = [&](size_t j) {
diff --git a/anakin_amd/csrc/conv1x1_chain.hip b/anakin_amd/csrc/conv1x1_chain.hip
--- a/anakin_amd/csrc/conv1x1_chain.hip
+++ b/anakin_amd/csrc/conv1x1_chain.hip
@@ -3,7 +3,7 @@
 namespace saber_mi355x {
 
 
-template <int KS1, int G1, int MFG2, int G2, int TN, int R, bool C3, int SP, bool HAS2 = true, int NW = 4, int S0 = 1>
+template <int KS1, int G1, int MFG2, int G2, int TN, int R, bool C3, int SP, bool HAS2 = true, int NW = 4, int S0 = 1, bool PROJ = false>
 __global__ __launch_bounds__(64 * NW) void conv1x1_chain_kernel(const ChainKArgs a) {
     static_assert(NW == 4 || NW == 8, "4 or 8 waves");
     static_assert(S0 == 1 || (C3 && S0 == 2), "a strided head is led by its 3x3 conv");
@@ -26,6 +26,10 @@
     static_assert(SG1 % R == 0 && SG2 % R == 0, "ring depth must divide the group lengths");
     static_assert(CPR >= 16 && P1C % 64 == 0, "tile rows are swizzled on 16 chunks");
     static_assert(SP == 1 || (!C3 && (NPX * CPR / (64 * NW)) % SP == 0), "split second conv: 1x1 chains only");
+    constexpr int CP = 256, KSP = CP / 64;
+    constexpr int TP = PROJ ? KSP * 4 : 0;
+    static_assert(!PROJ || (C3 && S0 == 1 && HAS2 && SP == 1 && G1 == 1 && K1 == 64 * NW && TP % R == 0),
+                  "projection shortcut: 3x3-led, one 64-channel group per wave, ring slots of the later phases unchanged");
 
     __shared__ v4i tile[NPX * CPR];
     __shared__ v4i prm1[P1C];
@@ -95,7 +99,7 @@
             for (int i = wave; i < P0C / 64; i += NW) lds_dma16((const v4i*)a.prm0 + i * 64 + lane, prm0 + i * 64);
         }
         const char* rg = (const char*)a.res;
-        constexpr int NI = NPX * CPR / 64;
+        constexpr int NI = PROJ ? 0 : NPX * CPR / 64;
 #pragma unroll
         for (int i0 = 0; i0 < NI; i0 += NW) {
             const int i = i0 + wave;
@@ -114,12 +118,72 @@
             for (int i = wave; i < P2C / 64; i += NW) lds_dma16((const v4i*)a.prm2 + i * 64 + lane, prm2 + i * 64);
     }
     asm volatile("" ::: "memory");
-
-    const v4i* wsb = (const v4i*)a.wstream + (size_t)(half * NW + wave) * ((T0 + T1 + T2) * 64);
+    v4i bp[PROJ ? KSP : 1][TN];
+    v4i cp0[PROJ ? 4 : 1];
+    if constexpr (PROJ) {
+#pragma unroll
+        for (int j = 0; j < TN; ++j) {
+            bool ok;
+            const int p = pix(j * 16 + frow, ok);
+            const char* xp = (const char*)a.res + (size_t)p * CP + fq * 16;
+#pragma unroll
+            for (int ks = 0; ks < KSP; ++ks) bp[ks][j] = *(const v4i*)(xp + ks * 64);
+        }
+        const v4i* pg = (const v4i*)a.prmp + ((wave * 64 + fq * 16) / 4) * 3;
+#pragma unroll
+        for (int mf = 0; mf < 4; ++mf) cp0[mf] = pg[mf * 3 + 2];
+        asm volatile("" ::: "memory");
+    }
+
+    const v4i* wsb = (const v4i*)a.wstream + (size_t)(half * NW + wave) * ((TP + T0 + T1 + T2) * 64);
     v4i ring[R];
 #pragma unroll
     for (int r = 0; r < R; ++r) ring[r] = wsb[r * 64 + lane];
     wsb += R * 64;
+
+    if constexpr (PROJ) {
+        asm volatile("" ::"s"(a.prmp), "s"(a.proj_in_u8), "s"(a.proj_relu));
+        const int xmp = a.proj_in_u8 ? (int)0x80808080u : 0;
+        const int cg = wave * 64 + fq * 16;
+        const v4i* pg = (const v4i*)a.prmp + (cg / 4) * 3;
+        v4i acc[4][TN];
+        v4f scp[4], bip[4];
+#pragma unroll
+        for (int mf = 0; mf < 4; ++mf)
+#pragma unroll
+            for (int j = 0; j < TN; ++j) acc[mf][j] = cp0[mf];
+#pragma unroll
+        for (int s = 0; s < TP; ++s) {
+            const int ks = s / 4, mf = s % 4;
+#pragma unroll
+            for (int j = 0; j < TN; ++j) {
+                v4i b = bp[ks][j];
+                b.x ^= xmp; b.y ^= xmp; b.z ^= xmp; b.w ^= xmp;
+                acc[mf][j] = mma_step(ring[s % R], b, acc[mf][j]);
+            }
+            ring[s % R] = wsb[s * 64 + lane];
+            if (s == TP / 2) {
+#pragma unroll
+                for (int m = 0; m < 4; ++m) {
+                    scp[m] = __builtin_bit_cast(v4f, pg[m * 3]);
+                    bip[m] = __builtin_bit_cast(v4f, pg[m * 3 + 1]);
+                }
+                asm volatile("" ::: "memory");
+            }
+        }
+        wsb += TP * 64;
+        const float lop = a.proj_relu ? 0.f : -3.0e38f;
+#pragma unroll
+        for (int j = 0; j < TN; ++j) {
+            v4i o;
+            o.x = (int)chain_out_pack(acc[0][j], v4i{0, 0, 0, 0}, bip[0], scp[0], lop, 128.f, 0x80808080u);
+            o.y = (int)chain_out_pack(acc[1][j], v4i{0, 0, 0, 0}, bip[1], scp[1], lop, 128.f, 0x80808080u);
+            o.z = (int)chain_out_pack(acc[2][j], v4i{0, 0, 0, 0}, bip[2], scp[2], lop, 128.f, 0x80808080u);
+            o.w = (int)chain_out_pack(acc[3][j], v4i{0, 0, 0, 0}, bip[3], scp[3], lop, 128.f, 0x80808080u);
+            tile[(j * 16 + frow) * CPR + ((cg / 16) ^ frow)] = o;
+        }
+        SABER_TL(6);
+    }
 
     if constexpr (C3) {
         asm volatile("s_waitcnt vmcnt(%0)" ::"n"(R) : "memory");
@@ -300,7 +364,8 @@
     SABER_TL_FLUSH();
 }
 
-bool conv1x1_chain_ok(int c1, int k1, int k2) {
+bool conv1x1_chain_ok(int c1, int k1, int k2, int s0) {
+    if (s0 == 2 && c1 == 64 && k1 == 256 && k2 == 128) return true;
     return (c1 == 64 || c1 == 128 || c1 == 256 || c1 == 512) && k1 == 4 * c1 && k2 == c1;
 }
 
@@ -308,15 +373,20 @@
     const bool has2 = k2 != 0;
     const bool pair2 = has2 && a.k2_split > 0;
     if (pair2 && !(a.s0 == 2 && with3x3 && c1 == 64 && k1 == 256 && k2 == 640 && a.k2_split % 32 == 0 && a.k2_split < 640)) return hipErrorInvalidValue;
-    if (!conv1x1_chain_ok(c1, k1, (has2 && !pair2) ? k2 : c1) || a.M <= 0 || (!has2 && !with3x3)) return hipErrorInvalidValue;
+    const bool shead2 = has2 && !pair2 && with3x3 && a.s0 == 2;
+    const bool proj = a.prmp != nullptr;
+    if (shead2 && !(c1 == 64 && k1 == 256 && k2 == 128)) return hipErrorInvalidValue;
+    if (proj && !(with3x3 && has2 && !pair2 && !shead2 && c1 == 128 && waves == 8 && split == 1)) return hipErrorInvalidValue;
+    if (!conv1x1_chain_ok(c1, k1, (has2 && !pair2) ? k2 : c1, shead2 ? 2 : 1) || a.M <= 0 || (!has2 && !with3x3)) return hipErrorInvalidValue;
     const dim3 block(64 * waves);
     const dim3 grid((with3x3 ? a.tiles_per_img * a.N : (a.M + 16 * rows - 1) / (16 * rows)) * split);
-    enum { PLAIN, LED, HEAD, SHEAD, PAIR };
-    const int kind = pair2 ? PAIR : (!has2 ? (a.s0 == 2 ? SHEAD : HEAD) : (with3x3 ? LED : PLAIN));
+    enum { PLAIN, LED, HEAD, SHEAD, PAIR, SHEAD2, LEDP };
+    const int kind = pair2 ? PAIR : (shead2 ? SHEAD2 : (proj ? LEDP : (!has2 ? (a.s0 == 2 ? SHEAD : HEAD) : (with3x3 ? LED : PLAIN))));
 #define SABER_CHAIN(KIND, C1, ROWS, NW, SP, KS1, G1, MFG2, G2, R)                                                                   \
     case (((KIND * 1024 + C1) * 8 + ROWS) * 16 + NW) * 4 + SP:                                                                      \
-        hipLaunchKernelGGL((conv1x1_chain_kernel<KS1, G1, MFG2, G2, ROWS, R, KIND != PLAIN, SP, KIND == PLAIN || KIND == LED || KIND == PAIR, NW, \
-                                                 KIND == SHEAD || KIND == PAIR ? 2 : 1>), grid, block, 0, s, a);                   \
+        hipLaunchKernelGGL((conv1x1_chain_kernel<KS1, G1, MFG2, G2, ROWS, R, KIND != PLAIN, SP,                                     \
+                                                 KIND == PLAIN || KIND == LED || KIND == PAIR || KIND == SHEAD2 || KIND == LEDP, NW, \
+                                                 KIND == SHEAD || KIND == PAIR || KIND == SHEAD2 ? 2 : 1, KIND == LEDP>), grid, block, 0, s, a); \
         break;
 #define SABER_CHAIN_W4(KIND)                          \
     SABER_CHAIN(KIND, 64, 4, 4, 1, 1, 1, 1, 1, 4)     \
@@ -330,6 +400,9 @@
     switch ((((kind * 1024 + c1) * 8 + rows) * 16 + waves) * 4 + split) {
     SABER_CHAIN(PAIR, 64, 4, 4, 1, 1, 1, 2, 5, 4)
     SABER_CHAIN(PAIR, 64, 2, 4, 1, 1, 1, 2, 5, 4)
+    SABER_CHAIN(SHEAD2, 64, 4, 4, 1, 1, 1, 2, 1, 4)
+    SABER_CHAIN(SHEAD2, 64, 2, 4, 1, 1, 1, 2, 1, 4)
+    SABER_CHAIN_C128_W8(LEDP)
     SABER_CHAIN_W4(SHEAD)
     SABER_CHAIN(SHEAD, 256, 1, 8, 1, 4, 2, 2, 1, 16)
     SABER_CHAIN_C128_W8(SHEAD)
diff --git a/anakin_amd/csrc/kernels.h b/anakin_amd/csrc/kernels.h
--- a/anakin_amd/csrc/kernels.h
+++ b/anakin_amd/csrc/kernels.h
@@ -118,6 +118,8 @@
     int res_sub, res_H, res_W;
     void* y2b;
     int k2_split, relu2b, out_u8_2b;
+    const void* prmp;
+    int proj_in_u8, proj_relu;
 };
 struct CoopKArgs {
     ChainKArgs c;
@@ -127,7 +129,7 @@
     unsigned* coop_err;
     int n_tiles;
 };
-bool conv1x1_chain_ok(int c1, int k1, int k2);
+bool conv1x1_chain_ok(int c1, int k1, int k2, int s0 = 1);
 hipError_t launch_conv1x1_chain(const ChainKArgs& a, int c1, int k1, int k2, int rows, int waves, int split, int with3x3, hipStream_t s);
 hipError_t launch_conv_chain_coop(const CoopKArgs& a, hipStream_t s);
 
diff --git a/anakin_amd/lib.py b/anakin_amd/lib.py
--- a/anakin_amd/lib.py
+++ b/anakin_amd/lib.py
@@ -19,7 +19,7 @@
     "saber_hip_conv2d_get_tile", "saber_hip_conv2d_autotune", "saber_hip_conv2d_set_pooling",
     "saber_hip_conv2d_create_pair", "saber_hip_conv2d_run_pair", "saber_hip_conv2d_autotune_pair",
     "saber_hip_net_add_conv_pair",
-    "saber_hip_conv2d_chain_create", "saber_hip_conv2d_chain_create3", "saber_hip_conv2d_chain_create3_pair", "saber_hip_conv2d_chain_destroy", "saber_hip_conv2d_chain_run",
+    "saber_hip_conv2d_chain_create", "saber_hip_conv2d_chain_create3", "saber_hip_conv2d_chain_create3_pair", "saber_hip_conv2d_chain_create3_trail", "saber_hip_conv2d_chain_create3_proj", "saber_hip_conv2d_chain_pack_weights_host", "saber_hip_conv2d_chain_destroy", "saber_hip_conv2d_chain_run",
     "saber_hip_conv2d_chain_run3",
     "saber_hip_conv2d_chain_set_tile", "saber_hip_conv2d_chain_get_tile",
     "saber_hip_conv2d_stage_create", "saber_hip_conv2d_stage_destroy", "saber_hip_conv2d_stage_run", "saber_hip_conv2d_stage_create_tail", "saber_hip_conv2d_stage_run_tail",
@@ -126,6 +126,9 @@
     lib.saber_hip_conv2d_chain_destroy.restype = None
     lib.saber_hip_conv2d_chain_run.argtypes = [P, P, P, P, P, P]
     lib.saber_hip_conv2d_chain_create3_pair.argtypes = [P, P, P, P, C.POINTER(P)]
+    lib.saber_hip_conv2d_chain_create3_trail.argtypes = [P, P, P, C.POINTER(P)]
+    lib.saber_hip_conv2d_chain_create3_proj.argtypes = [P, P, P, P, C.POINTER(P)]
+    lib.saber_hip_conv2d_chain_pack_weights_host.argtypes = [P, C.c_int, C.c_int, C.c_int, C.c_int, P, C.c_size_t]
     lib.saber_hip_conv2d_chain_run3.argtypes = [P, P, P, P, P, P, P]
     lib.saber_hip_conv2d_chain_set_tile.argtypes = [P, I]
     lib.saber_hip_conv2d_chain_get_tile.argtypes = [P]
diff --git a/anakin_amd/saber.py b/anakin_amd/saber.py
--- a/anakin_amd/saber.py
+++ b/anakin_amd/saber.py
@@ -339,10 +339,14 @@
 
 class SaberConvChain:
 
-    def __init__(self, a, b, conv3x3=None, pair_b=None):
-        self.a, self.b, self.c3, self.b2 = a, b, conv3x3, pair_b
-        self.h = C.c_void_p()
-        if pair_b is not None:
+    def __init__(self, a, b, conv3x3=None, pair_b=None, trail=False, proj=None):
+        self.a, self.b, self.c3, self.b2, self.proj = a, b, conv3x3, pair_b, proj
+        self.h = C.c_void_p()
+        if proj is not None:
+            L.check(L.load().saber_hip_conv2d_chain_create3_proj(proj.h, conv3x3.h, a.h, b.h, C.byref(self.h)))
+        elif trail:
+            L.check(L.load().saber_hip_conv2d_chain_create3_trail(conv3x3.h, a.h, b.h, C.byref(self.h)))
+        elif pair_b is not None:
             L.check(L.load().saber_hip_conv2d_chain_create3_pair(conv3x3.h, a.h, b.h, pair_b.h, C.byref(self.h)))
         elif conv3x3 is None:
             L.check(L.load().saber_hip_conv2d_chain_create(a.h, b.h, C.byref(self.h)))
diff --git a/anakin_amd/workloads.py b/anakin_amd/workloads.py
--- a/anakin_amd/workloads.py
+++ b/anakin_amd/workloads.py
@@ -369,7 +369,7 @@
     if shared_device:
         net.optimize(2048)
         stage = False
-    net.removed = net.absorbed = net.gpooled = net.stem_paired = net.chained = net.fc_softmaxed = net.separated = net.inverted = net.fired = 0
+    net.removed = net.absorbed = net.gpooled = net.stem_paired = net.chained = net.fc_softmaxed = net.separated = net.inverted = net.fired = net.pair_split = 0
     if fuse:
         net.removed = net.optimize(15)
     if fire:
@@ -384,6 +384,7 @@
         net.stem_paired = net.optimize(512) if stem_pair else 0
         net.chained = net.optimize(16 | (32 if int(chain) >= 2 else 0) | (256 if int(chain) >= 2 and stage else 0) |
                                    (1024 if int(chain) >= 2 and head_pair else 0)) if chain else 0
+        net.pair_split = net.optimize(131072) if int(chain) >= 2 else 0
         net.fc_softmaxed = net.optimize(4096) if fc_softmax else 0
     if before_finalize is not None:
         before_finalize(net)
diff --git a/include/saber_hip.h b/include/saber_hip.h
--- a/include/saber_hip.h
+++ b/include/saber_hip.h
@@ -86,6 +86,9 @@
 int saber_hip_conv2d_chain_create3(saber_hip_conv_t* conv3x3, saber_hip_conv_t* a, saber_hip_conv_t* b, saber_hip_chain_t** out);
 int saber_hip_conv2d_chain_create3_pair(saber_hip_conv_t* conv3x3, saber_hip_conv_t* a, saber_hip_conv_t* pair_a, saber_hip_conv_t* pair_b,
                                         saber_hip_chain_t** out);
+int saber_hip_conv2d_chain_create3_trail(saber_hip_conv_t* conv3x3, saber_hip_conv_t* a, saber_hip_conv_t* next, saber_hip_chain_t** out);
+int saber_hip_conv2d_chain_create3_proj(saber_hip_conv_t* proj, saber_hip_conv_t* conv3x3, saber_hip_conv_t* a, saber_hip_conv_t* b, saber_hip_chain_t** out);
+int saber_hip_conv2d_chain_pack_weights_host(const int8_t* w_oihw, int k, int c, int acc_per_group, int waves, uint8_t* out, size_t out_bytes);
 void saber_hip_conv2d_chain_destroy(saber_hip_chain_t* chain);
 int saber_hip_conv2d_chain_run(saber_hip_chain_t* chain, const void* x, const void* res, void* y_a, void* y_b,
                                saber_hip_stream_t stream);
@@ -261,6 +264,7 @@
 #define SABER_HIP_NET_SEPARABLE 16384
 #define SABER_HIP_NET_INVERTED_RESIDUAL 32768
 #define SABER_HIP_NET_FIRE 65536
+#define SABER_HIP_NET_PAIR_SPLIT 131072
 int saber_hip_net_optimize(saber_hip_net_t* net, int flags);
 int saber_hip_net_coop_fallbacks(const saber_hip_net_t* net);
 int saber_hip_coop_fallbacks_total(void);
```

Measured after the change: 39980, median of 5. Within noise of the previous version (+0.7%).
